# rrwick/Autocycler

Hardware: AMD Instinct MI355X
Metric: Mbp/sec through compress->unitig GFA (k=51) (higher is better)
Workload: dtype u64

## Files before the change

### autocycler_amd/_capi.py

```python
import ctypes as C
import os
from pathlib import Path

_HERE = Path(__file__).resolve().parent
LIB_PATH = _HERE / "libautocycler_hip.so"


class HipLibraryMissing(RuntimeError):
    pass


class AutocyclerError(RuntimeError):
    """The text the reference would hand to quit_with_error (misc.rs:131-137)."""


class SeqView(C.Structure):
    _fields_ = [("fwd", C.c_char_p), ("length", C.c_uint32), ("id", C.c_uint16)]


class Position(C.Structure):
    _fields_ = [("pos", C.c_uint32), ("seq_id_and_strand", C.c_uint16)]


class Link(C.Structure):
    _fields_ = [("a", C.c_int32), ("b", C.c_int32)]


class Stats(C.Structure):
    _fields_ = [("unitigs", C.c_uint32), ("links_one_way", C.c_uint64), ("total_length", C.c_uint64)]


class Timings(C.Structure):
    _fields_ = [(n, C.c_double) for n in ("h2d", "pack", "insert", "collect_sort", "degree", "segment", "minkey",
                                          "rank", "paths", "links", "seqs", "d2h", "total_device", "expand",
                                          "insert_kernel_ms")] + \
               [(n, C.c_uint64) for n in ("insert_positions", "table_capacity", "n_distinct", "n_path_entries")] + \
               [("simplify_passes", C.c_uint32), ("insert_launches", C.c_uint32), ("insert_real", C.c_uint64),
                ("analysis", C.c_double), ("finalize", C.c_double), ("n_candidates", C.c_uint32), ("n_levels", C.c_uint32),
                ("fragments", C.c_double), ("union_pack", C.c_double), ("union_insert", C.c_double),
                ("n_local_distinct", C.c_uint64), ("n_fragments", C.c_uint64), ("fragment_bytes", C.c_uint64),
                ("upload_device_ms", C.c_double), ("path_runs_copied", C.c_uint64), ("path_entries_walked", C.c_uint64), ("position_retries", C.c_uint64), ("n_candidates_owned", C.c_uint32),
                ("launches", C.c_uint32), ("readbacks", C.c_uint32), ("n_degrees_open", C.c_uint64), ("sort_retries", C.c_uint64), ("insert_rest_known", C.c_double), ("insert_rest_sampled", C.c_double), ("path_stretches", C.c_uint64),
                ("expand_sparse_sweeps", C.c_uint32), ("expand_sparse_start", C.c_uint32)]

    def as_dict(self):
        return {n: getattr(self, n) for n, _ in self._fields_}


class TrimSlice(C.Structure):
    _fields_ = [(n, C.c_uint32) for n in ("status", "begin", "end", "trimmed_length")]

    def as_dict(self):
        return {n: getattr(self, n) for n, _ in self._fields_}


class TrimResult(C.Structure):
    _fields_ = [("start_end", TrimSlice), ("hairpin", TrimSlice), ("hairpin_start_trimmed", C.c_uint32), ("hairpin_end_trimmed", C.c_uint32)]

    def as_dict(self):
        return dict(start_end=self.start_end.as_dict(), hairpin=self.hairpin.as_dict(),
                    hairpin_start_trimmed=self.hairpin_start_trimmed, hairpin_end_trimmed=self.hairpin_end_trimmed)


class TrimSummary(C.Structure):
    _fields_ = [("size", C.c_uint64), ("c_se", C.c_uint32), ("c_hp", C.c_uint32), ("chosen", C.c_uint32), ("launches", C.c_uint32),
                ("cells", C.c_uint64), ("seconds_device", C.c_double)]

    def as_dict(self):
        return {n: getattr(self, n) for n, _ in self._fields_ if n != "size"}


class AlignmentPiece(C.Structure):
    _fields_ = [("a_unitig", C.c_int32), ("a_index", C.c_uint32), ("b_unitig", C.c_int32), ("b_index", C.c_uint32)]


ALIGN_GAP, ALIGN_NONE = 0, 0xFFFFFFFF


class Bridge(C.Structure):
    _fields_ = [("start", C.c_int32), ("end", C.c_int32), ("depth", C.c_uint32), ("n_distinct", C.c_uint32), ("best_off", C.c_uint64),
                ("best_total", C.c_uint64), ("first_distinct", C.c_uint64), ("best_len", C.c_uint32), ("status", C.c_uint32),
                ("conflicting", C.c_uint32), ("culled", C.c_uint32), ("cull_rank", C.c_uint32), ("reserved", C.c_uint32)]


class ResolveSummary(C.Structure):
    _fields_ = [("size", C.c_uint64), ("jobs", C.c_uint64), ("jobs_not_launched", C.c_uint64), ("cells", C.c_uint64), ("largest_job_cells", C.c_uint64),
                ("launches", C.c_uint32), ("reserved", C.c_uint32), ("seconds_device", C.c_double)]

    def as_dict(self):
        return {n: getattr(self, n) for n, _ in self._fields_ if n not in ("size", "reserved")}


class Component(C.Structure):
    _fields_ = [("first", C.c_uint32), ("unitigs", C.c_uint32), ("length", C.c_uint64), ("links_all", C.c_uint64), ("links_one_way", C.c_uint64),
                ("open_ends", C.c_uint32), ("marked", C.c_uint32), ("circular_loop", C.c_uint8)]


class ComponentsSummary(C.Structure):
    _fields_ = [(n, C.c_uint32) for n in ("size", "unitigs", "components", "topology")] + \
               [(n, C.c_uint64) for n in ("links_all", "links_one_way", "total_length")] + \
               [("launches", C.c_uint32), ("read_backs", C.c_uint32), ("seconds_device", C.c_double)]

    def as_dict(self):
        return {n: getattr(self, n) for n, _ in self._fields_ if n != "size"}


class MergeChain(C.Structure):
    _fields_ = [("number", C.c_uint32), ("members", C.c_uint32), ("length", C.c_uint64), ("member_off", C.c_uint64), ("seq_off", C.c_uint64), ("depth", C.c_double),
                ("type", C.c_uint8), ("loop", C.c_uint8)]


class MergeSummary(C.Structure):
    _fields_ = [(n, C.c_uint32) for n in ("size", "chains", "merged_unitigs", "unitigs_after")] + [("links_after", C.c_uint64), ("bases_copied", C.c_uint64)] + \
               [("launches", C.c_uint32), ("read_backs", C.c_uint32), ("seconds_device", C.c_double), ("seconds_copy", C.c_double)]

    def as_dict(self):
        return {n: getattr(self, n) for n, _ in self._fields_ if n != "size"}


class SubsetCluster(C.Structure):
    _fields_ = [("seqs", C.c_uint32), ("unitigs", C.c_uint32), ("entries", C.c_uint64), ("links", C.c_uint64), ("length", C.c_uint64)]


class SubsetsSummary(C.Structure):
    _fields_ = [(n, C.c_uint32) for n in ("size", "clusters", "sequences_kept", "n_unitigs")] + [(n, C.c_uint64) for n in ("entries_kept", "unitigs", "links")] + \
               [("launches", C.c_uint32), ("read_backs", C.c_uint32), ("seconds_device", C.c_double)]

    def as_dict(self):
        return {n: getattr(self, n) for n, _ in self._fields_ if n != "size"}


class MergedPathsSummary(C.Structure):
    _fields_ = [("size", C.c_uint32), ("sequences", C.c_uint32), ("entries_before", C.c_uint64), ("entries_after", C.c_uint64),
                ("launches", C.c_uint32), ("read_backs", C.c_uint32), ("seconds_device", C.c_double)]

    def as_dict(self):
        return {n: getattr(self, n) for n, _ in self._fields_ if n != "size"}


class FinishedUnitig(C.Structure):
    _fields_ = [("number", C.c_uint32), ("source", C.c_uint32), ("length", C.c_uint64), ("seq_off", C.c_uint64), ("depth", C.c_double), ("type", C.c_uint8)]


class FinishedSummary(C.Structure):
    _fields_ = [(n, C.c_uint32) for n in ("size", "unitigs", "renumbered", "launches", "read_backs")] + \
               [(n, C.c_uint64) for n in ("links", "path_entries", "bases", "tie_items")] + [("seconds_device", C.c_double), ("seconds_gather", C.c_double)]

    def as_dict(self):
        return {n: getattr(self, n) for n, _ in self._fields_ if n != "size"}


class AppliedSummary(C.Structure):
    _fields_ = [(n, C.c_uint32) for n in ("size", "bridges_applied", "direct_links", "launches", "launches_components", "read_backs")] + \
               [(n, C.c_uint64) for n in ("removed_no_anchor", "removed_zero_depth", "links_in", "links_out", "bases_copied")] + \
               [("seconds_device", C.c_double), ("seconds_copy", C.c_double), ("seconds_components", C.c_double)]

    def as_dict(self):
        return {n: getattr(self, n) for n, _ in self._fields_ if n != "size"}


class CleanedSummary(C.Structure):
    _fields_ = [(n, C.c_uint32) for n in ("size", "unitigs_in", "unitigs_out", "rounds", "rounds_per_batch", "launches", "read_backs", "reserved")] + \
               [(n, C.c_uint64) for n in ("kept", "removed", "duplicated", "low_depth", "kept_dead_end", "absent", "links_in", "links_out")] + [("seconds_device", C.c_double)]

    def as_dict(self):
        return {n: getattr(self, n) for n, _ in self._fields_ if n not in ("size", "reserved")}


class TrimmedRecord(C.Structure):
    _fields_ = [("begin", C.c_uint32), ("end", C.c_uint32), ("length", C.c_uint64), ("trimmed", C.c_uint32), ("excluded", C.c_uint32)]


class TrimmedSummary(C.Structure):
    _fields_ = [("size", C.c_uint32), ("chosen", C.c_uint32), ("c_se", C.c_uint32), ("c_hp", C.c_uint32), ("sequences", C.c_uint32), ("trimmed", C.c_uint32),
                ("excluded", C.c_uint32), ("rejected", C.c_uint32), ("unitigs_in", C.c_uint32), ("unitigs_alive", C.c_uint32), ("launches", C.c_uint32),
                ("read_backs", C.c_uint32), ("median", C.c_uint64), ("mad", C.c_uint64), ("min_length", C.c_uint64), ("max_length", C.c_uint64),
                ("entries_kept", C.c_uint64), ("links", C.c_uint64), ("seconds_device", C.c_double), ("align_launches", C.c_uint32), ("reserved", C.c_uint32),
                ("align_cells", C.c_uint64), ("align_seconds_device", C.c_double)]

    def as_dict(self):
        return {name: getattr(self, name) for name, _ in self._fields_ if name not in ("size", "reserved")}


class CombinedCluster(C.Structure):
    _fields_ = [("input_index", C.c_uint32), ("unitigs", C.c_uint32), ("length", C.c_uint64), ("links", C.c_uint64), ("offset", C.c_uint64), ("max_number", C.c_uint32),
                ("topology", C.c_uint32), ("has_read_depth", C.c_uint32), ("reserved", C.c_uint32), ("read_depth", C.c_double)]


class CombinedUnitig(C.Structure):
    _fields_ = [("graph", C.c_uint32), ("index", C.c_uint32), ("number", C.c_uint32), ("length", C.c_uint32), ("depth", C.c_double), ("read_depth", C.c_double),
                ("has_read_depth", C.c_uint8), ("flags", C.c_uint8), ("type", C.c_uint8), ("reserved", C.c_uint8 * 5)]


class CombinedSummary(C.Structure):
    _fields_ = [("size", C.c_uint32), ("graphs", C.c_uint32), ("bases", C.c_uint64), ("unitigs", C.c_uint64), ("links", C.c_uint64), ("fully_resolved", C.c_uint32),
                ("with_reads", C.c_uint32), ("launches", C.c_uint32), ("read_backs", C.c_uint32), ("seconds_device", C.c_double)]

    def as_dict(self):
        d = {n: getattr(self, n) for n, _ in self._fields_ if n != "size"}
        d["fully_resolved"], d["with_reads"] = bool(d["fully_resolved"]), bool(d["with_reads"])
        return d


class ClusterNode(C.Structure):
    _fields_ = [("id", C.c_uint16), ("left", C.c_int32), ("right", C.c_int32), ("distance", C.c_double)]


class ClusterMerge(C.Structure):
    _fields_ = [("a", C.c_uint16), ("b", C.c_uint16), ("distance", C.c_double)]


class ClusterSummary(C.Structure):
    _fields_ = [("n_seqs", C.c_uint32), ("launches", C.c_uint32), ("rescans", C.c_uint64), ("compares", C.c_uint64), ("seconds", C.c_double)]

    def as_dict(self):
        return {n: getattr(self, n) for n, _ in self._fields_}


class ClusterQcRecord(C.Structure):
    _fields_ = [("node", C.c_uint16), ("container", C.c_uint16), ("size", C.c_uint32), ("assembly_count", C.c_uint32), ("fail", C.c_uint32),
                ("trusted", C.c_uint32), ("reserved", C.c_uint32), ("median_length", C.c_uint64), ("cluster_dist", C.c_double)]

    def as_dict(self):
        return {n: getattr(self, n) for n, _ in self._fields_ if n != "reserved"}


class ClusteringMetrics(C.Structure):
    _fields_ = [(n, C.c_uint32) for n in ("pass_cluster_count", "fail_cluster_count", "pass_contig_count", "fail_contig_count")] + \
               [(n, C.c_double) for n in ("pass_contig_fraction", "fail_contig_fraction", "cluster_balance_score", "cluster_tightness_score",
                                          "overall_clustering_score")]

    def as_dict(self):
        return {n: getattr(self, n) for n, _ in self._fields_}


class ClusterQcSummary(C.Structure):
    _fields_ = [(n, C.c_uint32) for n in ("n_seqs", "n_clusters", "rounds", "evaluations", "pair_batches", "launches", "readbacks", "reserved")] + \
               [(n, C.c_uint64) for n in ("alternatives", "node_pairs", "bytes_read_back")] + [("seconds", C.c_double), ("start_score", C.c_double)]

    def as_dict(self):
        return {n: getattr(self, n) for n, _ in self._fields_ if n != "reserved"}


class DepthGraph(C.Structure):
    _fields_ = [("seq_bytes", C.c_void_p), ("seq_begin", C.c_void_p), ("seq_len", C.c_void_p), ("n_unitigs", C.c_uint32),
                ("links", C.c_void_p), ("n_links", C.c_uint64)]


class DepthTotals(C.Structure):
    _fields_ = [("size", C.c_uint64)] + \
               [(n, C.c_uint64) for n in ("reads", "rejected_reads", "read_bases", "span_bases", "span_kmers", "hits", "distinct_kmers", "repeat_kmers",
                                          "table_slots")] + [("batches", C.c_uint32), ("launches", C.c_uint32), ("seconds_device", C.c_double)]

    def as_dict(self):
        return {n: getattr(self, n) for n, _ in self._fields_ if n != "size"}

ALLREDUCE_FN = C.CFUNCTYPE(C.c_int, C.c_void_p, C.c_void_p, C.c_uint64, C.c_int, C.c_int)

EXPORTS = ["ac_compress_build", "ac_compress_build_multi", "ac_multi_info_get", "ac_compress_build_device", "ac_pack_text", "ac_text_size", "ac_layout_text", "ac_kmer_count",
           "ac_stats_pre", "ac_stats_post", "ac_unitig_count", "ac_unitig", "ac_unitigs_bulk", "ac_paths_bulk", "ac_unitig_positions", "ac_links",
           "ac_path", "ac_timings_get", "ac_timings_get_sized", "ac_free", "ac_gfa_string", "ac_string_free", "ac_last_error",
           "ac_device_count", "ac_max_kmer", "ac_version", "ac_abi_version", "ac_set_host_side_device", "ac_source_hash", "ac_set_stage_timing", "ac_random_access_ceilings", "ac_random_access_ceilings_at", "ac_release_memory", "ac_end_repair_device", "ac_pairwise_distances", "ac_trim_paths", "ac_trim_path_slices", "ac_overlap_alignment", "ac_trim_max_unitigs", "ac_resolve_bridges", "ac_resolve_bridge_paths", "ac_path_distances", "ac_resolve_anchors", "ac_resolve_bridge_records", "ac_resolve_best_paths", "ac_resolve_distinct_paths", "ac_resolve_summary_get_sized", "ac_resolve_max_path", "ac_resolve_free", "ac_graph_components", "ac_components_from_links", "ac_components_records", "ac_components_of_unitig", "ac_components_members", "ac_components_unitig_flags", "ac_components_summary_get_sized", "ac_topology_name", "ac_components_free", "ac_graph_merge_plan", "ac_merge_plan_from_links", "ac_merge_chains", "ac_merge_members", "ac_merge_chain_of_unitig", "ac_merge_fixed_flags", "ac_merge_sequences", "ac_merge_links", "ac_merge_summary_get_sized", "ac_merge_free", "ac_graph_subsets", "ac_subsets_from_paths", "ac_subsets_records", "ac_subsets_unitigs", "ac_subsets_links", "ac_subsets_seqs", "ac_subsets_path_ends", "ac_subsets_dense", "ac_subsets_summary_get_sized", "ac_subsets_free", "ac_subsets_components", "ac_subsets_merge_plan", "ac_subsets_merged_paths", "ac_merged_paths_get", "ac_merged_paths_summary_get_sized", "ac_merged_paths_free", "ac_merge_finish", "ac_subsets_finish", "ac_finished_unitigs", "ac_finished_sequences", "ac_finished_new_of_old", "ac_finished_links", "ac_finished_paths", "ac_finished_summary_get_sized", "ac_finished_free", "ac_finished_gfa_string", "ac_finished_to_graph", "ac_apply_bridges", "ac_graph_resolve_apply", "ac_applied_unitigs", "ac_applied_bridge_of", "ac_applied_links", "ac_applied_bridge_sequences", "ac_applied_summary_get_sized", "ac_applied_free", "ac_applied_merge_plan", "ac_applied_finish", "ac_applied_gfa_string", "ac_resolve_graphs", "ac_clean_graph", "ac_graph_clean", "ac_cleaned_unitigs", "ac_cleaned_links", "ac_cleaned_summary_get_sized", "ac_cleaned_free", "ac_cleaned_merge_plan", "ac_cleaned_finish", "ac_cleaned_gfa_string", "ac_parse_tig_numbers", "ac_gfa_segment_types", "ac_clean_gfa", "ac_clean", "ac_trim_apply", "ac_graph_trim_apply", "ac_graph_trim", "ac_trimmed_records", "ac_trimmed_summary_get_sized", "ac_trimmed_free", "ac_trimmed_subsets", "ac_trimmed_finish", "ac_trimmed_yaml_string", "ac_trim_gfa", "ac_trim_dir", "ac_resolve_dir", "ac_combine_graphs", "ac_combine_handles", "ac_combined_clusters", "ac_combined_unitigs", "ac_combined_links", "ac_combined_summary_get_sized", "ac_combined_free", "ac_combined_gfa_string", "ac_combined_fasta_string", "ac_combined_yaml_string", "ac_combined_depth_lines", "ac_combine_gfas", "ac_combine", "ac_gfa2fasta_string", "ac_gfa2fasta", "ac_cluster_tree_build", "ac_cluster_tree_from_distances", "ac_cluster_tree_from_nodes", "ac_cluster_nodes", "ac_cluster_merges", "ac_cluster_summary_get_sized", "ac_cluster_free", "ac_cluster_max_seqs", "ac_cluster_cut", "ac_cluster_assign", "ac_cluster_containment", "ac_cluster_newick", "ac_cluster_generate", "ac_cluster_qc_nodes", "ac_cluster_qc_clusters", "ac_cluster_qc_assignment", "ac_cluster_qc_records", "ac_cluster_qc_metrics", "ac_cluster_qc_trace", "ac_cluster_qc_summary_get_sized", "ac_cluster_qc_free", "ac_cluster_min_assemblies", "ac_cluster_seq_inputs", "ac_depth_begin", "ac_depth_begin_handles", "ac_depth_add_reads", "ac_depth_add_fastq", "ac_depth_totals_get", "ac_depth_kmer_counts", "ac_depth_finish", "ac_depth_free", "ac_selftest_primitives", "ac_selftest_scan", "ac_selftest_radix", "ac_selftest_segments", "ac_selftest_sort_cmp", "ac_selftest_scan_pool", "ac_selftest_wave", "ac_selftest_fills", "ac_selftest_fill_order", "ac_selftest_readback", "ac_selftest_scalar_chain", "ac_selftest_arena", "ac_selftest_launch", "ac_selftest_atomics", "ac_selftest_side_order", "ac_selftest_event_ring", "ac_verify_graph", "ac_verify_graph_device", "ac_graph_from_gfa", "ac_graph_kmer_size", "ac_graph_seq_info", "ac_decompress_seq", "ac_decompress_device", "ac_decompress",
           "ac_shard_begin", "ac_shard_fragment_sizes", "ac_shard_fragments_export", "ac_shard_build_union", "ac_shard_fragment_packed_words", "ac_shard_fragments_export_packed", "ac_shard_build_union_packed",
           "ac_shard_unitig_count", "ac_shard_table_capacity", "ac_shard_bitmap_words", "ac_shard_bitmap_export", "ac_shard_build_novel", "ac_shard_sib_words", "ac_shard_sib_export", "ac_shard_degrees",
           "ac_shard_degree_bytes", "ac_multi_info_get_sized", "ac_shard_links_export", "ac_shard_links_import",
           "ac_shard_query_count", "ac_shard_query_key_words", "ac_shard_queries_export", "ac_shard_answer", "ac_shard_walk", "ac_shard_queries_route", "ac_shard_walk_routed", "ac_shard_local_distinct", "ac_shard_set_distinct_upper_bound", "ac_shard_distinct_count", "ac_shard_degrees_export", "ac_shard_build_graph", "ac_gfa_string_parts", "ac_shard_reduce_export", "ac_shard_reduce_import", "ac_shard_finish", "ac_shard_set_allreduce", "ac_device_copy",
           "ac_shard_path_entries", "ac_shard_paths_export", "ac_shard_free", "ac_graph_set_paths", "ac_graph_seq_count", "ac_path_counts",
           "ac_seqs_load", "ac_seqs_from_raw", "ac_seqs_count", "ac_seqs_assembly_count", "ac_seqs_views", "ac_seqs_get",
           "ac_seqs_repair_seconds", "ac_seqs_metrics_yaml", "ac_seqs_free", "ac_compress_seqs", "ac_compress_dir", "ac_compress_dir_multi"]

_libs = {}


def load_library(path=None):
    path = Path(path) if path else LIB_PATH
    key = str(path)
    if key in _libs:
        return _libs[key]
    if not path.exists():
        raise HipLibraryMissing(f"{path} not found: build the HIP extension first (make -C autocycler_amd/csrc). "
                                "There is no CPU fallback.")
    try:
        if os.environ.get("AC_NO_TORCH"):
            raise ImportError
        import torch
    except ImportError:
        pass
    lib = C.CDLL(key)
    lib.ac_last_error.restype = C.c_char_p
    lib.ac_version.restype = C.c_char_p
    lib.ac_source_hash.restype = C.c_char_p
    lib.ac_kmer_count.restype = C.c_uint64
    lib.ac_kmer_count.argtypes = [C.c_void_p]
    lib.ac_stats_pre.restype = Stats
    lib.ac_stats_pre.argtypes = [C.c_void_p]
    lib.ac_stats_post.restype = Stats
    lib.ac_stats_post.argtypes = [C.c_void_p]
    lib.ac_unitig_count.restype = C.c_uint32
    lib.ac_unitig_count.argtypes = [C.c_void_p]
    lib.ac_max_kmer.restype = C.c_uint32
    lib.ac_text_size.restype = C.c_uint64
    lib.ac_free.argtypes = [C.c_void_p]
    lib.ac_string_free.argtypes = [C.c_void_p]
    lib.ac_unitig.argtypes = [C.c_void_p, C.c_uint32, C.POINTER(C.c_void_p), C.POINTER(C.c_uint32), C.POINTER(C.c_double)]
    lib.ac_unitig_positions.argtypes = [C.c_void_p, C.c_uint32, C.c_int, C.POINTER(C.POINTER(Position)), C.POINTER(C.c_uint32)]
    lib.ac_links.argtypes = [C.c_void_p, C.POINTER(C.POINTER(Link)), C.POINTER(C.c_uint64)]
    lib.ac_path.argtypes = [C.c_void_p, C.c_uint32, C.POINTER(C.POINTER(C.c_int32)), C.POINTER(C.c_uint32)]
    lib.ac_timings_get.argtypes = [C.c_void_p, C.POINTER(Timings)]
    lib.ac_shard_unitig_count.restype = C.c_uint32
    lib.ac_shard_unitig_count.argtypes = [C.c_void_p]
    lib.ac_shard_fragment_packed_words.restype = C.c_uint64
    lib.ac_shard_fragment_packed_words.argtypes = [C.c_void_p, C.c_uint64]
    lib.ac_shard_local_distinct.restype = C.c_uint64
    lib.ac_shard_local_distinct.argtypes = [C.c_void_p]
    lib.ac_shard_set_distinct_upper_bound.argtypes = [C.c_void_p, C.c_uint64]
    lib.ac_shard_set_distinct_upper_bound.restype = None
    lib.ac_shard_distinct_count.restype = C.c_uint64
    lib.ac_shard_distinct_count.argtypes = [C.c_void_p]
    lib.ac_shard_path_entries.restype = C.c_uint64
    lib.ac_shard_path_entries.argtypes = [C.c_void_p]
    lib.ac_shard_free.argtypes = [C.c_void_p]
    for name in ("ac_shard_table_capacity", "ac_shard_bitmap_words", "ac_shard_query_count", "ac_shard_sib_words", "ac_shard_degree_bytes"):
        getattr(lib, name).restype = C.c_uint64
        getattr(lib, name).argtypes = [C.c_void_p]
    lib.ac_shard_query_key_words.restype = C.c_uint32
    lib.ac_shard_query_key_words.argtypes = [C.c_void_p]
    lib.ac_graph_seq_count.restype = C.c_uint32
    lib.ac_graph_seq_count.argtypes = [C.c_void_p]
    lib.ac_trim_max_unitigs.restype = C.c_uint32
    lib.ac_trim_max_unitigs.argtypes = []
    lib.ac_trim_paths.argtypes = [C.c_void_p, C.c_double, C.c_uint32, C.c_int, C.POINTER(TrimResult), C.POINTER(TrimSummary)]
    lib.ac_trim_path_slices.argtypes = [C.c_void_p, C.c_void_p, C.c_uint32, C.c_void_p, C.c_uint32, C.c_double, C.c_uint32, C.c_int,
                                        C.POINTER(TrimResult), C.POINTER(TrimSummary)]
    lib.ac_overlap_alignment.argtypes = [C.c_void_p, C.c_void_p, C.c_uint32, C.c_void_p, C.c_uint32, C.c_double, C.c_uint32, C.c_int, C.c_int,
                                         C.POINTER(AlignmentPiece), C.POINTER(C.c_uint32)]
    lib.ac_resolve_max_path.restype = C.c_uint32
    lib.ac_resolve_max_path.argtypes = []
    lib.ac_resolve_bridges.argtypes = [C.c_void_p, C.c_int, C.POINTER(C.c_void_p)]
    lib.ac_resolve_bridge_paths.argtypes = [C.c_void_p, C.c_void_p, C.c_uint32, C.c_void_p, C.c_void_p, C.c_uint32, C.c_int, C.POINTER(C.c_void_p)]
    lib.ac_path_distances.argtypes = [C.c_void_p, C.c_void_p, C.c_uint32, C.c_void_p, C.c_void_p, C.c_uint64, C.c_void_p, C.c_uint32, C.c_int, C.c_void_p, C.c_void_p]
    lib.ac_resolve_anchors.argtypes = [C.c_void_p, C.POINTER(C.POINTER(C.c_uint32)), C.POINTER(C.c_uint32)]
    lib.ac_resolve_bridge_records.argtypes = [C.c_void_p, C.POINTER(C.POINTER(Bridge)), C.POINTER(C.c_uint32)]
    lib.ac_resolve_best_paths.argtypes = [C.c_void_p, C.POINTER(C.POINTER(C.c_int32)), C.POINTER(C.c_uint64)]
    lib.ac_resolve_distinct_paths.argtypes = [C.c_void_p, C.POINTER(C.POINTER(C.c_int32)), C.POINTER(C.POINTER(C.c_uint64)), C.POINTER(C.POINTER(C.c_uint32)),
                                              C.POINTER(C.c_uint64)]
    lib.ac_resolve_summary_get_sized.restype = C.c_size_t
# ... 2095 lines not shown
```

### autocycler_amd/csrc/capi.cpp

```cpp
#include <algorithm>
#include <cstring>
#include <memory>

#include "capi_common.hpp"
#include "gfa_writer.hpp"

using namespace ac;
using namespace ac::abi;

static void select_device(int device, bool refresh_tuning = true) {
    if (refresh_tuning) tuning_refresh();
#ifndef AC_EMU
    int n = 0;
    hipError_t e = hipGetDeviceCount(&n);
    if (e != hipSuccess || n == 0)
        throw DeviceError("no HIP device available: the MI355X backend has no CPU fallback");
    if (device < 0 || device >= n) throw DeviceError("invalid HIP device ordinal " + std::to_string(device));
    AC_HIP_CHECK(hipSetDevice(device));
    hipDeviceProp_t prop;
    AC_HIP_CHECK(hipGetDeviceProperties(&prop, device));
    if (std::string(prop.gcnArchName).rfind("gfx950", 0) != 0)
        throw DeviceError(std::string("device is ") + prop.gcnArchName + "; this library is built for gfx950 only");
#endif
    int& arena_device = device_ctx().arena_device;
// ... 5 lines not shown
            Mailbox::get().release();
#endif
        }
        arena_device = device;
    }
}

namespace ac {
void select_device_checked(int device) { select_device(device, false); }

namespace abi __attribute__((visibility("hidden"))) {

std::string& last_error() { static thread_local std::string err; return err; }
std::mutex g_build_mutex;
int g_live_shards = 0;
std::atomic<int> g_host_side_device{0};

DeviceCall::DeviceCall(int device, Kind kind) : lock(g_build_mutex) {
    if (g_live_shards && kind != SHARD_PHASE)
        throw DeviceError(kind == SHARD_BEGIN ? "another sharded build is in flight in this process" : "a sharded build is in flight in this process");
    if (kind == ALL_DEVICES) tuning_refresh();
    else select_device(device);
}

void validate(uint32_t k, const ac_seq_view* seqs, uint32_t n_seqs) {
    if (!seqs || n_seqs == 0) throw DeviceError("no sequences found in input assemblies");
    if (k % 2 == 0) throw DeviceError("--kmer must be odd");
    if (n_seqs > 32767) throw DeviceError("no more than 32767 input sequences are allowed");
    for (uint32_t i = 0; i < n_seqs; i++) {
        if (!seqs[i].fwd) throw DeviceError("null sequence pointer");
        if (seqs[i].length < k) throw DeviceError("sequence shorter than k");
    }
}

void validate_layout(uint32_t k, uint64_t n_text, const uint64_t* off, const uint32_t* len, const uint16_t* d1, const uint16_t* d2,
                     uint32_t n_seqs) {
    if (k < 1 || k % 2 == 0) throw DeviceError("--kmer must be odd");
    if (!off || !len || !d1 || !d2) throw DeviceError("null sequence table");
    uint64_t prev_end = 0;
    for (uint32_t i = 0; i < n_seqs; i++) {
        if (len[i] < k) throw DeviceError("sequence " + std::to_string(i + 1) + " is shorter than k");
        const uint64_t plen = (uint64_t)len[i] + k - 1;
        if (off[i] != prev_end + 1) throw DeviceError("sequence table: sequence " + std::to_string(i + 1) + " does not start right behind the separator of the previous one");
        if (off[i] + plen + 1 > n_text) throw DeviceError("sequence table: sequence " + std::to_string(i + 1) + " runs past the end of the text");
        if (d1[i] > k - 1 || d2[i] > k - 1 || (uint32_t)d1[i] + d2[i] > k - 1) throw DeviceError("sequence table: more padding dots than k - 1 on sequence " + std::to_string(i + 1));
        prev_end = off[i] + plen;
    }
    if (n_seqs && prev_end + 1 != n_text) throw DeviceError("sequence table: the text does not end with the separator of the last sequence");
}

std::vector<SeqView> seq_views(const ac_seq_view* seqs, uint32_t n_seqs, std::vector<uint16_t>* seq_ids, std::vector<uint32_t>* seq_lens) {
    std::vector<SeqView> v(n_seqs);
    for (uint32_t i = 0; i < n_seqs; i++) {
        v[i] = SeqView{seqs[i].fwd, seqs[i].length};
        seq_ids->push_back(seqs[i].id);
        seq_lens->push_back(seqs[i].length);
    }
    return v;
}

void set_device_text(GraphBuilder& b, const void* d_text, uint64_t n_text, const uint64_t* seq_off, const uint32_t* seq_len,
                     const uint16_t* ids, const uint16_t* seq_d1, const uint16_t* seq_d2, uint32_t n_seqs,
                     std::vector<uint16_t>* seq_ids, std::vector<uint32_t>* seq_lens) {
    std::vector<uint64_t> off(seq_off, seq_off + n_seqs);
    std::vector<uint32_t> len(seq_len, seq_len + n_seqs);
    std::vector<uint16_t> d1(seq_d1, seq_d1 + n_seqs), d2(seq_d2, seq_d2 + n_seqs);
    seq_ids->assign(ids, ids + n_seqs);
    *seq_lens = len;
    b.set_text_device((const uint8_t*)d_text, n_text, off, len, d1, d2);
}

}
}

static void build_graph(GraphBuilder& b, uint32_t assembly_count, ac_graph* h) {
    b.build(assembly_count, &h->g);
    h->tm = b.timings();
}

template <class T> static size_t copy_sized(const T& full, T* out, size_t out_size) {
    memcpy(out, &full, std::min(out_size, sizeof full));
    return sizeof full;
}

extern "C" {

const char* ac_last_error(void) { return last_error().c_str(); }
const char* ac_version(void) {
#ifdef AC_EMU
    return "autocycler_amd 0.1 (CPU emulation, tests only)";
#else
    return "autocycler_amd 0.1 (gfx950)";
#endif
}
int ac_abi_version(void) { return AC_ABI_VERSION; }
int ac_set_host_side_device(int device) { if (device < 0) return fail("invalid HIP device ordinal"); g_host_side_device.store(device); return 0; }
void ac_set_stage_timing(int on) { set_stage_timing(on != 0); }
int ac_release_memory(void) {
    return guarded([&] {
        std::lock_guard<std::mutex> lock(g_build_mutex);
        if (g_live_shards) throw DeviceError("a sharded build is in flight in this process");
        Arena::device().release_all();
        release_multi_contexts();
        PinnedPool::get().trim();
        release_host_stager();
        scan_pool().release();
#ifndef AC_EMU
        Mailbox::get().release();
#endif
    });
}
uint32_t ac_max_kmer(void) { int m = max_supported_k(); return (uint32_t)(m % 2 ? m : m - 1); }
int ac_device_count(void) {
#ifndef AC_EMU
    int n = 0;
    if (hipGetDeviceCount(&n) != hipSuccess) return 0;
    return n;
#else
    return 0;
#endif
}

uint64_t ac_text_size(uint32_t k, const ac_seq_view* seqs, uint32_t n_seqs) {
    uint64_t n = 1;
    for (uint32_t i = 0; i < n_seqs; i++) n += (uint64_t)seqs[i].length + k - 1 + 1;
    return n;
}
int ac_layout_text(uint32_t k, const ac_seq_view* seqs, uint32_t n_seqs, uint8_t* text, uint64_t* seq_off,
                   uint16_t* seq_d1, uint16_t* seq_d2) {
    return guarded([&] {
        std::vector<SeqView> v(n_seqs);
        for (uint32_t i = 0; i < n_seqs; i++) v[i] = SeqView{seqs[i].fwd, seqs[i].length};
        std::vector<uint64_t> off; std::vector<uint32_t> len; std::vector<uint16_t> d1, d2;
        std::vector<uint8_t> t = layout_text(v, k, &off, &len, &d1, &d2);
        memcpy(text, t.data(), t.size());
        for (uint32_t i = 0; i < n_seqs; i++) { seq_off[i] = off[i]; seq_d1[i] = d1[i]; seq_d2[i] = d2[i]; }
    });
}

int ac_pack_text(const uint8_t* text, uint64_t n_text, uint64_t* bits, uint32_t* mask32, int force_scalar) {
    return guarded([&] {
        if (!text || !bits || !mask32) throw DeviceError("null pointer");
        pack_text_host(text, n_text, bits, mask32, force_scalar != 0);
    });
}

int ac_compress_build(uint32_t k, uint32_t assembly_count, const ac_seq_view* seqs, uint32_t n_seqs, int device,
                      ac_graph** out) {
    return guarded([&] {
        validate(k, seqs, n_seqs);
        DeviceCall call(device);
        auto h = std::make_unique<ac_graph>();
        const std::vector<SeqView> v = seq_views(seqs, n_seqs, &h->seq_ids, &h->seq_lens);
        GraphBuilder b(k);
        b.set_sequences_host(v);
        build_graph(b, assembly_count, h.get());
        *out = h.release();
    });
}

int ac_compress_build_multi(uint32_t k, uint32_t assembly_count, const ac_seq_view* seqs, uint32_t n_seqs, const int* devices, int n_devices,
                            ac_graph** out) {
    return guarded([&] {
        validate(k, seqs, n_seqs);
        if (!devices || n_devices < 1) throw DeviceError("ac_compress_build_multi: no devices");
        if (n_devices > 64) throw DeviceError("ac_compress_build_multi: more than 64 devices");
        DeviceCall call(-1, DeviceCall::ALL_DEVICES);
        auto h = std::make_unique<ac_graph>();
        const std::vector<SeqView> v = seq_views(seqs, n_seqs, &h->seq_ids, &h->seq_lens);
        int transport = MULTI_AUTO;
        if (const int e = tuning_multi_transport()) transport = e == 1 ? MULTI_HOST_STAGED : MULTI_RCCL;
        build_multi(k, assembly_count, v, std::vector<int>(devices, devices + n_devices), transport, &h->g, &h->tm, &h->multi);
        *out = h.release();
    });
}
int ac_multi_info_get(const ac_graph* g, ac_multi_info* o) {
    if (!g || !o) return fail("null pointer");
    const MultiStats& m = g->multi;
    memset(o, 0, sizeof *o);
    o->n_ranks = m.n_ranks; o->transport = m.transport;
    o->bytes_fragments = m.bytes_fragments; o->bytes_bitmap = m.bytes_bitmap; o->bytes_degrees = m.bytes_degrees; o->bytes_links = m.bytes_links;
    o->bytes_queries = m.bytes_queries; o->bytes_answers = m.bytes_answers; o->bytes_reduce = m.bytes_reduce;
    o->queries_total = m.queries_total; o->queries_sent_away = m.queries_sent_away;
    o->table_capacity_max = m.table_capacity_max; o->table_capacity_sum = m.table_capacity_sum;
    o->union_text_bytes = m.union_text_bytes; o->fragments = m.fragments; o->distinct = m.distinct;
    o->seconds_total = m.seconds_total; o->seconds_exchange_max = m.seconds_exchange_max;
    o->candidates_total = m.candidates_total; o->candidates_owned_max = m.candidates_owned_max;
    o->bytes_sibling = m.bytes_sibling; o->bytes_tail = m.bytes_tail; o->degrees_open = m.degrees_open; o->bytes_received_max = m.bytes_received_max;
    o->path_runs_copied = m.path_runs_copied;
    return 0;
}
size_t ac_multi_info_get_sized(const ac_graph* g, ac_multi_info* out, size_t out_size) {
    ac_multi_info t;
    if (!g || !out) { fail("null pointer"); return sizeof t; }
    ac_multi_info_get(g, &t);
    return copy_sized(t, out, out_size);
}

int ac_compress_build_device(uint32_t k, uint32_t assembly_count, const void* d_text, uint64_t n_text,
                             const uint64_t* seq_off, const uint32_t* seq_len, const uint16_t* seq_ids,
                             const uint16_t* seq_d1, const uint16_t* seq_d2, uint32_t n_seqs, int device,
                             ac_graph** out) {
    return guarded([&] {
        if (!d_text || n_seqs == 0) throw DeviceError("no sequences found in input assemblies");
        if (n_seqs > 32767) throw DeviceError("no more than 32767 input sequences are allowed");
        validate_layout(k, n_text, seq_off, seq_len, seq_d1, seq_d2, n_seqs);
        DeviceCall call(device);
        auto h = std::make_unique<ac_graph>();
        GraphBuilder b(k);
        set_device_text(b, d_text, n_text, seq_off, seq_len, seq_ids, seq_d1, seq_d2, n_seqs, &h->seq_ids, &h->seq_lens);
        build_graph(b, assembly_count, h.get());
        *out = h.release();
    });
}

uint32_t ac_graph_seq_count(const ac_graph* g) { return (uint32_t)g->seq_ids.size(); }
int ac_path_counts(const ac_graph* g, uint64_t* counts) {
    for (size_t s = 0; s + 1 < g->g.path_off.size(); s++) counts[s] = g->g.path_off[s + 1] - g->g.path_off[s];
    return 0;
}

uint32_t ac_graph_kmer_size(const ac_graph* g) { return g->g.k; }
int ac_graph_seq_info(const ac_graph* g, uint32_t i, uint16_t* id, uint32_t* length, const char** filename, const char** header) {
    if (i >= g->seq_ids.size()) return fail("sequence index out of range");
    if (id) *id = g->seq_ids[i];
    if (length) *length = g->seq_lens[i];
    if (filename) *filename = i < g->filenames.size() ? g->filenames[i].c_str() : nullptr;
    if (header) *header = i < g->headers.size() ? g->headers[i].c_str() : nullptr;
    return 0;
}

uint64_t ac_kmer_count(const ac_graph* g) { return g->g.n_kmers; }
ac_stats ac_stats_pre(const ac_graph* g) { return ac_stats{g->g.pre.unitigs, g->g.pre.links_one_way, g->g.pre.total_length}; }
ac_stats ac_stats_post(const ac_graph* g) { return ac_stats{g->g.post.unitigs, g->g.post.links_one_way, g->g.post.total_length}; }
uint32_t ac_unitig_count(const ac_graph* g) { return g->g.n_unitigs; }

int ac_unitig(const ac_graph* g, uint32_t idx, const uint8_t** seq, uint32_t* len, double* depth) {
    if (idx >= g->g.n_unitigs) return fail("unitig index out of range");
    if (!g->host_arrays) return fail("this rank kept no host arrays (sharded build, not the writing rank)");
    if (seq) *seq = (const uint8_t*)g->g.seq(idx);
    if (len) *len = g->g.seq_len[idx];
    if (depth) *depth = g->g.depth[idx];
    return 0;
}
int ac_unitig_positions(ac_graph* g, uint32_t idx, int forward, const ac_position** positions, uint32_t* n) {
    if (idx >= g->g.n_unitigs) return fail("unitig index out of range");
    return guarded([&] {
        if (!g->host_arrays || !g->host_paths) throw DeviceError("this rank kept no host arrays (sharded build, not the writing rank)");
        if (!g->positions_built) { build_positions(&g->g, g->seq_ids, g->seq_lens); g->positions_built = true; }
        auto& v = forward ? g->g.fwd_positions[idx] : g->g.rev_positions[idx];
        static_assert(sizeof(ac_position) == sizeof(Position), "layout");
        *positions = (const ac_position*)v.data();
        *n = (uint32_t)v.size();
    });
}
int ac_links(const ac_graph* g, const ac_link** links, uint64_t* n) {
    static_assert(sizeof(ac_link) == sizeof(Link), "layout");
    if (!g->host_arrays) return fail("this rank kept no host arrays (sharded build, not the writing rank)");
    *links = (const ac_link*)g->g.links;
    *n = g->g.n_links;
    return 0;
}
int ac_path(const ac_graph* g, uint32_t seq_index, const int32_t** signed_unitigs, uint32_t* n) {
    if ((size_t)seq_index + 1 >= g->g.path_off.size()) return fail("sequence index out of range");
    if (!g->host_paths) return fail("this rank kept no paths on the host (sharded build)");
    uint64_t b = g->g.path_off[seq_index], e = g->g.path_off[seq_index + 1];
    *signed_unitigs = g->g.path + b;
    *n = (uint32_t)(e - b);
    return 0;
}
int ac_unitigs_bulk(const ac_graph* g, const uint8_t** seq_bytes, const uint64_t** seq_begin, const uint32_t** seq_len, const double** depth) {
    if (!g->host_arrays) return fail("this rank kept no host arrays (sharded build, not the writing rank)");
    if (seq_bytes) *seq_bytes = (const uint8_t*)g->g.seq_block.p;
    if (seq_begin) *seq_begin = g->g.seq_begin;
    if (seq_len) *seq_len = g->g.seq_len;
    if (depth) *depth = g->g.depth;
    return 0;
}
int ac_paths_bulk(const ac_graph* g, const int32_t** path_entries, const uint64_t** path_off, uint64_t* n_entries) {
    if (!g->host_paths) return fail("this rank kept no paths on the host (sharded build)");
    if (path_entries) *path_entries = g->g.path;
    if (path_off) *path_off = g->g.path_off.data();
    if (n_entries) *n_entries = g->g.n_path;
    return 0;
}
int ac_timings_get(const ac_graph* g, ac_timings* o) {
    const BuildTimings& t = g->tm;
    o->h2d = t.h2d; o->pack = t.pack; o->insert = t.insert; o->collect_sort = t.collect_sort; o->degree = t.degree;
    o->segment = t.segment; o->minkey = t.minkey; o->rank = t.rank; o->paths = t.paths; o->links = t.links; o->seqs = t.seqs;
    o->d2h = t.d2h; o->total_device = t.total_device; o->expand = t.expand;
    o->insert_kernel_ms = t.insert_kernel_ms; o->insert_positions = t.insert_positions;
    o->table_capacity = t.table_capacity; o->n_distinct = t.n_distinct; o->n_path_entries = t.n_path_entries;
    o->simplify_passes = t.simplify_passes; o->n_candidates = t.n_candidates; o->n_levels = t.n_levels;
    o->insert_launches = t.insert_launches; o->insert_real = t.insert_real;
    o->analysis = t.analysis; o->finalize = t.finalize;
    o->fragments = t.fragments; o->union_pack = t.union_pack; o->union_insert = t.union_insert;
    o->n_local_distinct = t.n_local_distinct; o->n_fragments = t.n_fragments; o->fragment_bytes = t.fragment_bytes;
    o->upload_device_ms = t.upload_device_ms;
    o->path_runs_copied = t.path_runs_copied; o->path_entries_walked = t.path_entries_walked; o->position_retries = t.position_retries;
    o->n_candidates_owned = t.n_candidates_owned;
    o->launches = t.launches; o->readbacks = t.readbacks; o->n_degrees_open = t.n_degrees_open; o->sort_retries = t.sort_retries;
    o->insert_rest_known = t.insert_rest_known; o->insert_rest_sampled = t.insert_rest_sampled; o->path_stretches = t.path_stretches;
    o->expand_sparse_sweeps = t.expand_sparse_sweeps; o->expand_sparse_start = t.expand_sparse_start;
    return 0;
}
size_t ac_timings_get_sized(const ac_graph* g, ac_timings* out, size_t out_size) {
    ac_timings t;
    memset(&t, 0, sizeof t);
    ac_timings_get(g, &t);
    return out ? copy_sized(t, out, out_size) : sizeof t;
}
void ac_free(ac_graph* g) { delete g; }

static int gfa_parts_impl(const ac_graph* g, int parts, const char* const* filenames, const char* const* headers, char** out,
                          uint64_t* out_len) {
    return guarded([&] {
        if ((parts & 1) && !g->host_arrays) throw DeviceError("this rank kept no unitigs / links on the host (sharded build)");
        if ((parts & 2) && !g->host_paths) throw DeviceError("this rank kept no paths on the host (sharded build)");
        std::vector<SeqMeta> meta(g->seq_ids.size());
        for (size_t i = 0; i < meta.size(); i++) meta[i] = SeqMeta{g->seq_ids[i], g->seq_lens[i], filenames[i], headers[i]};
        std::string s = gfa_string(g->g, meta, parts);
        char* p = (char*)malloc(s.size() + 1);
        if (!p) throw DeviceError("out of memory");
        memcpy(p, s.data(), s.size()); p[s.size()] = 0;
        *out = p;
        if (out_len) *out_len = s.size();
    });
}
int ac_gfa_string(const ac_graph* g, const char* const* filenames, const char* const* headers, char** out, uint64_t* out_len) {
    return gfa_parts_impl(g, 3, filenames, headers, out, out_len);
}
int ac_gfa_string_parts(const ac_graph* g, int parts, const char* const* filenames, const char* const* headers, char** out,
                        uint64_t* out_len) {
    return gfa_parts_impl(g, parts, filenames, headers, out, out_len);
}
void ac_string_free(char* p) { free(p); }

}
```

### autocycler_amd/csrc/graph_build.hpp

```cpp
#pragma once
#include <cstdint>
#include <functional>
#include <string>
#include <vector>

#include "graph_types.hpp"
#include "trim_host.hpp"
#include "resolve_host.hpp"
#include "components_host.hpp"
#include "merge_host.hpp"
#include "subset_host.hpp"
#include "trim_apply_host.hpp"
#include "finish_host.hpp"
#include "apply_host.hpp"
#include "clean_host.hpp"
#include "combine_host.hpp"
#include "cluster_host.hpp"
#include "cluster_qc_host.hpp"

namespace ac {

struct SeqView {
    const uint8_t* fwd;
    uint32_t length;
};

struct BuildTimings {
    double h2d = 0, pack = 0, insert = 0, collect_sort = 0, degree = 0, segment = 0, minkey = 0, rank = 0,
           paths = 0, links = 0, seqs = 0, d2h = 0, total_device = 0;
    double expand = 0;
    double analysis = 0;
    double finalize = 0;
    double insert_kernel_ms = 0;
    uint64_t insert_positions = 0;
    uint64_t table_capacity = 0;
    uint64_t n_distinct = 0;
    uint64_t n_path_entries = 0;
    uint32_t insert_launches = 0;
    uint64_t insert_real = 0;
    uint32_t simplify_passes = 0, n_candidates = 0, n_levels = 0;
    uint32_t n_candidates_owned = 0;
    uint32_t local_hint = 0, graph_hint = 0;
    double fragments = 0;
    double union_pack = 0, union_insert = 0;
    uint64_t n_local_distinct = 0, n_fragments = 0, fragment_bytes = 0;
    double upload_device_ms = 0;
    double insert_rest_known = 0;
    uint64_t path_stretches = 0;
    uint32_t expand_sparse_sweeps = 0;
    uint32_t expand_sparse_start = 0;
    double insert_rest_sampled = 0;
    uint32_t sort_retries = 0;
    uint32_t position_retries = 0;
    uint32_t launches = 0, readbacks = 0;
    uint64_t n_degrees_open = 0;
    uint64_t path_runs_copied = 0, path_entries_walked = 0;
};

struct RepairTimings { double total = 0, scan_ms = 0; uint64_t hits = 0, matches = 0; uint32_t patterns = 0; };

class GraphBuilder {
  public:
    explicit GraphBuilder(uint32_t k);
    ~GraphBuilder();
    void set_sequences_host(const std::vector<SeqView>& seqs, bool pack_now = true);
    void repair_ends(RepairTimings* tm);
    void set_text_device(const uint8_t* d_text, uint64_t n_text, const std::vector<uint64_t>& off,
                         const std::vector<uint32_t>& len, const std::vector<uint16_t>& d1,
                         const std::vector<uint16_t>& d2);
    void build(uint32_t assembly_count_hint, FinalGraph* out);

    void shard_begin(uint32_t local_assembly_hint);
    uint64_t local_distinct_count() const;
    void set_distinct_upper_bound(uint64_t n);
    uint64_t fragment_text_bytes() const;
    uint64_t fragment_count() const;
    void fragments_export(void* d_text_out, void* d_meta_out);
    uint64_t fragment_packed_words(uint64_t union_off) const;
    void fragments_export_packed(uint64_t union_off, void* d_words_out, void* d_meta_out);
    void shard_build_union_packed(uint32_t rank, uint32_t n_shards, const void* d_staged_words, const uint64_t* first_word, const uint64_t* n_words,
                                  uint64_t n_union_text, const void* d_meta, uint64_t n_frags_total);
    void shard_build_union(uint32_t rank, uint32_t n_shards, const uint8_t* d_union_text, uint64_t n_union_text,
                           const void* d_meta, uint64_t n_frags_total);
    uint64_t bitmap_words() const;
    void bitmap_export(void* d_out);
    void shard_build_novel(const void* d_bitmap_sum);
    uint64_t sib_words() const;
    void sib_export(void* d_out);
    void shard_degrees(const void* d_sib_sum);
    uint64_t degree_bytes() const;
    uint64_t distinct_count() const;
    void degrees_export(void* d_out);
    void shard_build_graph(const void* d_kinfo_sum);
    uint32_t unitig_count() const;
    void links_export(void* d_links_i32, void* d_wlinks_i64);
    void links_import(const void* d_links_i32, const void* d_wlinks_i64);
    uint64_t query_count() const;
    uint32_t query_key_words() const;
    void queries_export(void* d_out);
    void answer_queries(const void* d_keys, uint64_t n, void* d_out);
    void shard_walk(const void* d_answers_mine);
    void queries_route(uint32_t n_shards, void* d_routed_keys, uint64_t* counts_host);
    void shard_walk_routed(const void* d_routed_answers);
    void reduce_export(int32_t* d_sum, int32_t* d_min);
    void reduce_import(const int32_t* d_sum, const int32_t* d_min);
    void set_tail_exchange(std::function<void(void*, uint64_t, int, int)> all_reduce);
    void shard_finish(FinalGraph* out, bool want_graph, bool want_paths);
    uint64_t path_entry_count() const;
    void paths_export(void* d_out);
    const BuildTimings& timings() const { return tm_; }
    void set_sequence_index_base(uint64_t n);
    static void set_upload_threads_cap(int n);
    uint64_t n_text() const;
    uint64_t n_bases() const;

    struct Impl;

  private:
    void build_union_impl(uint32_t rank, uint32_t n_shards, const uint8_t* d_union_text, const void* d_staged_words, const uint64_t* first_word,
                          const uint64_t* n_words, uint64_t n_union_text, const void* d_meta, uint64_t n_frags_total);
    void upload_packed(const std::vector<SeqView>& seqs, const std::vector<uint64_t>& off);
    Impl* impl_;
    BuildTimings tm_;
};

std::vector<uint8_t> layout_text(const std::vector<SeqView>& seqs, uint32_t k, std::vector<uint64_t>* off,
                                 std::vector<uint32_t>* len, std::vector<uint16_t>* d1, std::vector<uint16_t>* d2);

void end_repair_device(uint32_t k, uint8_t* d_text, uint64_t n_text, const std::vector<uint64_t>& off, const std::vector<uint32_t>& len,
                       std::vector<uint16_t>* d1, std::vector<uint16_t>* d2, RepairTimings* tm, bool reset_arena = true);

void pairwise_distances_device(const FinalGraph& g, uint32_t n_seqs, double* out);

struct VerifyReport {
    uint32_t failed = 0;
    uint64_t first_bad_unitig = ~0ULL, first_bad_link = ~0ULL, first_bad_path_entry = ~0ULL, first_bad_sequence = ~0ULL, first_bad_base = ~0ULL;
    uint64_t unitigs = 0, links = 0, path_entries = 0, bases_checked = 0, self_mirror_links = 0;
    double seconds = 0;
    uint32_t checks = 0;
    uint64_t first_bad_junction = ~0ULL;
};
void verify_graph_device(const FinalGraph& g, const uint8_t* d_text, uint64_t n_text, const std::vector<uint64_t>& off,
                         const std::vector<uint32_t>& len, VerifyReport* rep);

void decompress_device(const FinalGraph& g, const std::vector<uint32_t>& seq_len, uint8_t* out_host);
struct TrimDeviceStats { double seconds_device = 0; uint64_t cells = 0; uint32_t jobs = 0, launches = 0; };
void overlap_alignment_batch(const std::vector<AlignJob>& jobs, const uint32_t* weights, uint32_t max_unitigs, std::vector<AlignOut>* outs,
                             TrimDeviceStats* st);
uint32_t trim_max_unitigs();
struct ResolveDeviceStats { double seconds_device = 0; uint64_t cells = 0, jobs = 0, largest_job_cells = 0; uint32_t launches = 0; };
void path_distance_batch(const PathPool& pool, const std::vector<PathPair>& pairs, const uint32_t* weights, std::vector<uint32_t>* dist,
                         ResolveDeviceStats* st);
uint32_t resolve_max_path();
struct ClusterDeviceStats { double seconds = 0; uint64_t rescans = 0, compares = 0; uint32_t launches = 0; };
void cluster_merges_device(const double* asym, uint32_t n, std::vector<ClusterRowMerge>* merges, ClusterDeviceStats* st);
void cluster_merges_graph_device(const FinalGraph& g, uint32_t n_seqs, double* asym_out, std::vector<ClusterRowMerge>* merges, ClusterDeviceStats* st);
uint32_t cluster_max_seqs();
struct ClusterQcDeviceStats {
    double seconds = 0;
    uint32_t launches = 0, readbacks = 0, evaluations = 0, pair_batches = 0;
    uint64_t alternatives = 0, pairs_counted = 0, bytes_read_back = 0;
};
void cluster_qc_device(const double* asym, uint32_t n, const uint32_t* dfs_tip, double cutoff, const std::function<void(const ClusterQcEvaluate&)>& body,
                       ClusterQcDeviceStats* st);
void components_device(uint32_t n_unitigs, const Link* links, uint64_t n_links, const uint32_t* unitig_len, const uint8_t* alive, const uint8_t* marked,
                       ComponentsResult* out);
struct MergePlanInput {
    uint32_t n_unitigs = 0; const Link* links = nullptr; uint64_t n_links = 0; const uint32_t* unitig_len = nullptr; const uint8_t* alive = nullptr;
    const uint8_t* seed_fixed = nullptr; const int32_t* path = nullptr; uint64_t n_path = 0;
    const uint8_t* seq_bytes = nullptr; const uint64_t* seq_begin = nullptr; uint64_t seq_total = 0;
};
void merge_plan_device(const MergePlanInput& in, MergeResult* out);
struct SubsetInput {
    uint32_t n_unitigs = 0; const Link* links = nullptr; uint64_t n_links = 0; const uint32_t* unitig_len = nullptr; const uint8_t* alive = nullptr;
    const int32_t* path = nullptr; const uint64_t* path_off = nullptr; uint32_t n_clusters = 0; const SubsetPlan* plan = nullptr;
};
void subsets_device(const SubsetInput& in, SubsetResult* out);
struct MergedPathsInput {
    uint32_t n_unitigs = 0; const uint32_t* unitig_len = nullptr; const int32_t* path = nullptr; const uint64_t* path_off = nullptr;
    const SubsetPlan* plan = nullptr; size_t kept_first = 0, kept_count = 0; const MergeResult* merge = nullptr;
};
void merged_paths_device(const MergedPathsInput& in, MergedPathsResult* out);
struct TrimApplyInput {
    uint32_t n_unitigs = 0; const Link* links = nullptr; uint64_t n_links = 0; const uint32_t* unitig_len = nullptr; const uint8_t* alive = nullptr;
    const int32_t* path = nullptr; const uint64_t* path_off = nullptr; double mad = 0;
};
void trim_apply_device(const TrimApplyInput& in, TrimApplyPlan* tp, SubsetPlan* plan, SubsetResult* out);
struct FinishInput {
    uint32_t n_unitigs = 0; const Link* links = nullptr; uint64_t n_links = 0; const uint32_t* unitig_len = nullptr; const uint8_t* alive = nullptr;
    const double* depth = nullptr; const uint8_t* type = nullptr; const uint8_t* seq_bytes = nullptr; const uint64_t* seq_begin = nullptr; uint64_t seq_total = 0;
    const MergeResult* plan = nullptr; const int32_t* path = nullptr; uint64_t n_path = 0; bool renumber = false; uint64_t unitigs_after = 0;
};
void merge_finish_device(const FinishInput& in, FinishResult* out);
void apply_bridges_device(const ApplyInput& in, const ApplyPlan& plan, ApplyResult* out);
void clean_device(const CleanInput& in, CleanResult* out);
void combine_device(const CombineInput& in, CombineResult* out);
void primitives_selftest(uint64_t n, uint64_t seed, int end_bit, int key_kind);
void selftest_scan(int kind, const void* in, uint64_t n, bool in_place, int misalign_in, int misalign_out, void* out);
void selftest_radix(const uint64_t* keys, const void* vals, uint64_t n, int begin_bit, int end_bit, int val_kind, uint64_t prep_n, int prep_bits, bool prep_reuse,
                    uint64_t* keys_out, void* vals_out);
void selftest_segments(int op, const uint32_t* seg, const uint64_t* vals, uint64_t n, uint64_t n_segments, bool deferred_err, void* out, uint32_t* err_out);
void selftest_sort_cmp(int form, const uint64_t* a, const uint32_t* b, const uint32_t* vals, uint64_t n, uint64_t* a_out, uint32_t* b_out, uint32_t* vals_out);
void selftest_scan_pool(int op, uint64_t value, uint64_t* out);
void selftest_wave(int program, const uint64_t* in_u64, const int32_t* aux_i32, const uint64_t* live_mask, uint64_t* out_u64);
void selftest_fills(const uint64_t* regions, uint64_t n_regions, int trigger, int mode, uint8_t* span, uint64_t span_bytes, uint32_t* launches_out);
void selftest_fill_order(uint64_t n, int byte1, uint64_t w_lo, uint64_t w_hi, int w_val, uint64_t from2, int byte2, uint64_t upto3, int byte3, uint8_t* out);
void selftest_readback(const uint8_t* data, uint64_t n_data, int path, const uint64_t* items, uint64_t n_items, uint8_t* out, uint32_t* counters_out);
void selftest_scalar_chain(const uint64_t* values, uint64_t n, uint64_t* out, uint32_t* counters_out);
void selftest_arena(const uint64_t* ops, uint64_t n_ops, uint64_t* totals_out, uint64_t* allocs_out, const uint8_t* live, uint64_t* wrong_out);
void selftest_launch(int which, uint64_t n, uint64_t* slots_out, uint32_t* info_out);
void selftest_atomics(int op, uint64_t init, uint64_t expected, const uint64_t* operand, const uint32_t* target, uint32_t n_words, uint64_t* words_out, uint64_t* returns_out);
void selftest_side_order(int mode, int which, uint32_t seed, uint64_t n_words, uint32_t* out_words);
void selftest_event_ring(int op, const uint8_t* kinds, uint32_t n_more, uint64_t* out);

void random_access_ceilings(double* cas_gops, double* read_gops, uint64_t table_slots = (uint64_t)1 << 24);

void device_warmup(int device, uint32_t k = 0, uint64_t text_bytes_estimate = 0);

void pack_text_host(const uint8_t* text, uint64_t n_text, uint64_t* bits, uint32_t* mask32, bool force_scalar);

void release_host_stager();

int max_supported_k();
void tuning_refresh();
int tuning_multi_transport();
bool tuning_multi_fragments_as_bytes();
bool tuning_multi_tail_replicated();
void set_stage_timing(bool on);
bool stage_timing();

}
```

### autocycler_amd/csrc/graph_impl.hpp

```cpp
#pragma once
#include "graph_build.hpp"

#include <chrono>
#include <cmath>
#include <map>
#include <string>
#include <algorithm>
#include <atomic>
#include <thread>
#include <functional>
#include <condition_variable>
#include <mutex>
#include <fcntl.h>
#include <unistd.h>
#if defined(__x86_64__)
#include <immintrin.h>
#endif

#include "device_rt.hpp"

namespace ac {

static double now_s() {
    return std::chrono::duration<double>(std::chrono::steady_clock::now().time_since_epoch()).count();
}



static const int MAX_PROBES = 1 << 14;
static const int MAX_PROBES_INSERT = 1 << 10;
#ifndef AC_W_ONLY
#define AC_W_ONLY 0
#endif
extern bool g_stage_timing;

static const u32 KI_OUT_MASK = 7u, KI_IN_SHIFT = 3, KI_FIRST_T = 1u << 6, KI_FIRST_RCT = 1u << 7;

struct TextCtx {
    const u64* bits;
    const u64* mask;
    u64 n_text;
    int k;
    const u64* seq_off;
    const u32* seq_len;
    const u16* seq_d1;
    const u16* seq_d2;
    u32 n_seqs;
};

struct Table {
    u64* slots;
    u64 cap_mask;
    const u64* occ;
    u64* novel;
    u32 n_owners;
    u32 my_owner;
    u64* sflags;
    u64* full_at;
    u64* runs; u32* run_count; u64 run_row0;
};
static const u64 RUN_MIN = 128;
static const u32 RUN_ROW = 128;
AC_D void run_note(const Table& tb, u64 wave, u32& noted, u64 pj, u64 qj, bool same, u64 n) {
    if (!tb.runs || n < RUN_MIN || noted >= RUN_ROW) return;
    u64* rec = tb.runs + 3 * ((tb.run_row0 + wave) * RUN_ROW + noted);
    noted++;
    const bool with_anchor = ((tb.novel[qj >> 6] >> (qj & 63)) & 1) != 0;
    if (with_anchor) { rec[0] = pj; rec[1] = n + 1; rec[2] = qj | ((u64)(same ? 1 : 0) << 63); }
    else { rec[0] = pj + 1; rec[1] = n; rec[2] = (same ? qj + 1 : qj - 1) | ((u64)(same ? 1 : 0) << 63); }
}
AC_D void run_note_done(const Table& tb, u64 wave, u32 noted) { if (tb.runs) tb.run_count[tb.run_row0 + wave] = noted; }
AC_D void sib_note(const Table& tb, u64 s, u32 fl) { if (fl) atomic_or64(&tb.sflags[s >> 5], (u64)fl << (2 * (s & 31))); }
AC_HD u32 sib_bits(u64 v, u64 mine) {
    const u64 d = v ^ mine;
    if ((d >> TAG_MFP_SHIFT) != 0 || slot_isdot(v) || (d >> 41) == 0) return 0;
    return (((d >> TAG_X_SHIFT) & 3) == 0 ? 1u : 0u) | (((d >> TAG_Y_SHIFT) & 3) == 0 ? 2u : 0u);
}
AC_HD bool table_owns(const Table& tb, u64 home_hash) { return tb.n_owners <= 1 || (u32)((home_hash >> 40) % tb.n_owners) == tb.my_owner; }

AC_HD bool locate(const TextCtx& t, u64 p, u32* s_out, u32* f_out) {
    if (t.n_seqs == 0 || p < t.seq_off[0]) return false;
    u32 lo = 0, hi = t.n_seqs;
    while (hi - lo > 1) {
        u32 mid = lo + ((hi - lo) >> 1);
        if (t.seq_off[mid] <= p) lo = mid; else hi = mid;
    }
    u64 f = p - t.seq_off[lo];
    if (f >= (u64)t.seq_len[lo]) return false;
    *s_out = lo; *f_out = (u32)f;
    return true;
}

template <int W> AC_HD bool xkmer_at(const TextCtx& t, u64 p, XKmer<W>* x) {
    u32 s, f;
    if (!locate(t, p, &s, &f)) return false;
    int k = t.k;
    int plen = (int)t.seq_len[s] + k - 1;
    int ld = (int)t.seq_d1[s] - (int)f;
    int td = (int)f + k - (plen - (int)t.seq_d2[s]);
    x->ld = ld > 0 ? ld : 0;
    x->td = td > 0 ? td : 0;
    x->fwd = text_extract<W>(t.bits, p, k);
    return true;
}

template <int W> AC_HD int claimant_match(const TextCtx& t, u64 v, const Key<W>& ukey) {
    XKmer<W> y;
    if (!slot_isdot(v)) {
        y.fwd = text_extract<W>(t.bits, slot_pos(v), t.k);
        y.ld = 0; y.td = 0;
    } else {
        if (!xkmer_at<W>(t, slot_pos(v), &y)) return 0;
    }
    bool yf;
    Key<W> yk = xk_canonical<W>(y, t.k, &yf);
    if (!key_eq<W>(yk, ukey)) return 0;
    return yf ? 2 : 1;
}

struct FindResult { u64 pos; int claimant_flipped; bool found; };

template <int W> AC_HD FindResult table_find(const TextCtx& t, const Table& tb, const Key<W>& ukey, bool isdot) {
    const KeyPlace pl = key_place<W>(ukey, t.k, isdot, key_hash<W>(ukey));
    u64 tag = slot_make(pl.tag, isdot, 0);
    const u64 hh = pl.home;
    u64 s = hh & tb.cap_mask;
    FindResult r; r.found = false; r.pos = 0; r.claimant_flipped = 0;
    if (!table_owns(tb, hh)) return r;
    if (tb.occ && !((tb.occ[s >> 6] >> (s & 63)) & 1)) return r;
    for (int probes = 0; probes < MAX_PROBES; probes++) {
        u64 v = tb.slots[s];
        if (v == SLOT_EMPTY) return r;
        if (slot_tag_eq(v, tag)) {
            int m = claimant_match<W>(t, v, ukey);
            if (m) { r.found = true; r.pos = slot_pos(v); r.claimant_flipped = (m == 2); return r; }
        }
        s = (s + 1) & tb.cap_mask;
    }
    return r;
}

template <int W> AC_HD bool find_xk(const TextCtx& t, const Table& tb, const XKmer<W>& x, u64* pos, bool* rel_same) {
    bool flipped;
    Key<W> uk = xk_canonical<W>(x, t.k, &flipped);
    FindResult r = table_find<W>(t, tb, uk, x.ld > 0 || x.td > 0);
    if (!r.found) return false;
    *pos = r.pos;
    *rel_same = ((r.claimant_flipped != 0) == flipped);
    return true;
}

template <int W> AC_HD bool owns_xk(const TextCtx& t, const Table& tb, const XKmer<W>& x) {
    if (tb.n_owners <= 1) return true;
    bool flipped;
    Key<W> uk = xk_canonical<W>(x, t.k, &flipped);
    return table_owns(tb, key_home<W>(uk, t.k, x.ld > 0 || x.td > 0, key_hash<W>(uk)));
}

struct Novel {
    const u64* bm;
    const u32* wprefix;
};
AC_HD int popc64(u64 x) {
#ifdef AC_EMU
    return __builtin_popcountll(x);
#else
    return __popcll(x);
#endif
}
AC_HD u32 novel_rank(const Novel& nv, u64 pos) {
    u64 w = pos >> 6;
    int b = (int)(pos & 63);
    u64 below = b ? (nv.bm[w] & ((1ULL << b) - 1)) : 0;
    return nv.wprefix[w] + (u32)popc64(below);
}

static const u64 NOREF = ~0ULL;

template <int W> AC_D u64 table_insert(const TextCtx& t, const Table& tb, const Key<W>& ukey, bool isdot, bool flipped, u64 p,
                                       u32* claimed, u32* err, bool* same, bool* mine_now) {
    const KeyPlace pl = key_place<W>(ukey, t.k, isdot, key_hash<W>(ukey));
    u64 mine = slot_make(pl.tag, isdot, p);
    const u64 hh = pl.home;
    u64 s = hh & tb.cap_mask;
    *mine_now = false;
    if (!table_owns(tb, hh)) return NOREF;
    const bool note = tb.sflags != nullptr && !isdot;
    u32 my_fl = 0;
    for (int probes = 0; probes < MAX_PROBES_INSERT; probes++) {
        u64 v = tb.slots[s];
        if (v == SLOT_EMPTY) {
            u64 old = atomic_cas64(&tb.slots[s], SLOT_EMPTY, mine);
            if (old == SLOT_EMPTY) { (*claimed)++; *mine_now = true; if (note) sib_note(tb, s, my_fl); return NOREF; }
            v = old;
        }
        if (slot_tag_eq(v, mine)) {
            if (slot_pos(v) == p) { if (note) sib_note(tb, s, my_fl); return NOREF; }
            int m = claimant_match<W>(t, v, ukey);
            if (m) {
                if (note) sib_note(tb, s, my_fl);
                if (slot_pos(v) > p) {
                    u64 old = atomic_min64(&tb.slots[s], mine);
                    if (old > mine) {
                        *mine_now = true;
                        u64 q = slot_pos(old);
                        atomic_xor64(&tb.novel[q >> 6], 1ULL << (q & 63));
                    }
                    return NOREF;
                }
                *same = ((m == 2) == flipped);
                return slot_pos(v);
            }
        } else if (note) {
            const u32 fl = sib_bits(v, mine);
            if (fl) { sib_note(tb, s, fl); my_fl |= fl; }
        }
        s = (s + 1) & tb.cap_mask;
    }
    atomic_or32(err, 1u);
    if (tb.full_at) atomic_max64(tb.full_at, ~p);
    return NOREF;
}

struct alignas(16) V16 { u32 a, b, c, d; };

#include "kernels_table.inc"
#include "kernels_unitigs.inc"
#include "kernels_paths.inc"
#include "kernels_tail.inc"
#include "kernels_shard.inc"
struct PathRemapJob {
    int32_t* path = nullptr; u64 n_ent = 0;
    const int32_t* rec_val = nullptr; const u32* rec_pos = nullptr; u64 n_rec = 0;
    const u32* number = nullptr; u32 n_unitigs = 0;
    u64 ent_limit = ~0ULL;
    void* landed = nullptr; SideStream* side = nullptr;
    int dev = 0;
    std::atomic<u64> next{0}; std::atomic<int> ready{0};
    std::atomic<u32> bad{0};
    u64 ticket = 0; bool started = false;
    std::atomic<double> t_ready{0}, t_last{0};
};
void path_remap_range(int32_t* p, u64 n, const u32* number, u32 n_unitigs, std::atomic<u32>* bad);
void path_stretch_range(const PathRemapJob& j, u64 s0, u64 s1, std::atomic<u32>* bad);
bool path_remap_is_wide();
void path_remap_start(PathRemapJob& j, int threads);
void path_remap_finish(PathRemapJob& j) noexcept;
struct SeqExpandJob {
    const u64* words = nullptr; u8* out = nullptr; u64 total = 0;
    void* landed = nullptr; SideStream* side = nullptr; int dev = 0;
    std::atomic<u64> next{0}; std::atomic<int> ready{0};
    u64 ticket = 0; bool started = false;
    std::atomic<double> t_start{0}, t_ready{0}, t_last{0};
};
void seq_expand_range(const u64* words, u8* out, u64 b, u64 e);
void seq_expand_start(SeqExpandJob& j, int threads);
void seq_expand_finish(SeqExpandJob& j) noexcept;
[[maybe_unused]] static int key_words(int k) { int w = words_for_k(k); return w <= 4 ? w : (w <= 8 ? 8 : 16); }
[[maybe_unused]] static u64 next_pow2(u64 x) { u64 p = 1; while (p < x) p <<= 1; return p; }
[[maybe_unused]] static size_t arena_estimate(u64 n_text, bool owns_text) { return (size_t)n_text * (owns_text ? 8 : 7) + ((size_t)768 << 20); }
struct Knobs {
    int minkey_variant;
    int path_copy;
    u64 run_piece;
    u32 pos_cap;
    bool path_filter;
    int host_remap_mode;
    u32 remap_block;
    int minkey_prefix_bases;
    bool seed_prefix_sort;
    u32 seed_max_group;
    int seed_prefix_bits;
    u32 degree_region_cap;
    int upload_direct_mode;
    int upload_slots;
    int degree_flags;
    int table_shift;
    u64 wave_chunk_max;
    u64 insert_chunk_rest_env;
    bool host_pack;
    u32 expand_level_table;
    bool shard_path_copy;
    bool expand_rewrite_always;
    u32 expand_sparse_max, expand_sparse_list, expand_sparse_batch;
    u32 stretch_device_share;
    int seq_codes_transfer;
    int late_copies;
    bool seq_writer_plain;
    bool seq_writer_forced;
    u64 seed_radix_limit;
    bool upload_overlap;
    bool sort_checks_deferrable;
    bool shard_host_remap;
    bool shard_degree_flags;
    bool insert_adaptive;
    u64 insert_growth;
    u64 insert_waves_target;
    bool renum_two_pass;
    u32 renum_max_group;
    u32 path_chunk_env;
    long upload_threads_env;
    bool debug_arena;
    bool degree_diag;
    int multi_transport;
    int multi_fragments;
    int multi_tail;
    u64 trim_batch_bytes;
    u64 resolve_batch_bytes;
    static Knobs read() {
        Knobs k;
        k.minkey_variant = [&]() -> int { const char* e = getenv("AC_MINKEY_VARIANT"); return e ? atoi(e) : -1; }();
        k.path_copy = [&]() -> int { const char* e = getenv("AC_PATH_COPY"); return e ? (atoi(e) != 0 ? 1 : 0) : 2; }();
        k.run_piece = [&]() -> u64 { const char* e = getenv("AC_RUN_PIECE"); const long v = e ? atol(e) : 0; return v > 0 ? (u64)v : 4096; }();
        k.pos_cap = [&]() -> u32 { const char* e = getenv("AC_POS_CAP"); const long v = e ? atol(e) : 65536; return v < 0 ? 0u : (u32)std::min<long>(v, 0x3FFFFFFF); }();
        k.path_filter = [&]() -> bool { const char* e = getenv("AC_PATH_FILTER"); return e ? atoi(e) != 0 : true; }();
        k.host_remap_mode = [&]() -> int { const char* e = getenv("AC_HOST_REMAP"); return e ? (atoi(e) == 2 ? 2 : (atoi(e) != 0 ? 1 : 0)) : -1; }();
        k.remap_block = [&]() -> u32 { const char* e = getenv("AC_REMAP_BLOCK"); int v = e ? atoi(e) : 4096; v = v < 64 ? 64 : (v > 65536 ? 65536 : v); return (u32)(v & ~63); }();
        k.minkey_prefix_bases = [&]() -> int { const char* e = getenv("AC_MINKEY_PREFIX_BASES"); int v = e ? atoi(e) : 31; return v < 1 ? 1 : (v > 31 ? 31 : v); }();
        k.seed_prefix_sort = [&]() -> bool { const char* e = getenv("AC_SEED_PREFIX_SORT"); return e ? atoi(e) != 0 : true; }();
        k.seed_max_group = [&]() -> u32 { const char* e = getenv("AC_SEED_MAX_GROUP"); int v = e ? atoi(e) : 1024; return (u32)(v < 1 ? 1 : v); }();
        k.seed_prefix_bits = [&]() -> int { const char* e = getenv("AC_SEED_PREFIX_BITS"); if (!e) return 0; int v = atoi(e); return v < 1 ? 1 : (v > 64 ? 64 : v); }();
        k.degree_region_cap = [&]() -> u32 { const char* e = getenv("AC_DEGREE_REGION_CAP"); int v = e ? atoi(e) : 0; return (u32)(v < 0 ? 0 : v); }();
        k.upload_direct_mode = [&]() -> int { const char* e = getenv("AC_UPLOAD_DIRECT"); return e ? (atoi(e) != 0 ? 1 : 0) : -1; }();
        k.upload_slots = [&]() -> int { const char* e = getenv("AC_UPLOAD_SLOTS"); int v = e ? atoi(e) : 1 << 20; return v < 1 ? 1 : v; }();
        k.degree_flags = [&]() -> int { const char* e = getenv("AC_DEGREE_FLAGS"); return e ? (atoi(e) != 0 ? 1 : 0) : 1; }();
        k.table_shift = [&]() -> int { const char* e = getenv("AC_TABLE_SHIFT"); if (!e) return -1; int v = atoi(e); return v < 0 ? 0 : (v > 3 ? 3 : v); }();
        k.wave_chunk_max = [&]() -> u64 { const char* e = getenv("AC_INSERT_CHUNK"); u64 x = e ? (u64)atoll(e) : 8192; return (std::max<u64>(x, 256) + 63) & ~63ULL; }();
        k.insert_chunk_rest_env = [&]() -> u64 { const char* e = getenv("AC_INSERT_CHUNK_REST"); if (!e) return 0; return (std::max<u64>((u64)atoll(e), 256) + 63) & ~63ULL; }();
        k.host_pack = [&]() -> bool { const char* e = getenv("AC_HOST_PACK"); return e ? atoi(e) != 0 : true; }();
        k.expand_level_table = [&]() -> u32 { const char* e = getenv("AC_EXPAND_LEVEL_TABLE"); int v = e ? atoi(e) : 1024; return (u32)(v < 1 ? 1 : v); }();
        k.shard_path_copy = [&]() -> bool { const char* e = getenv("AC_SHARD_PATH_COPY"); return !(e && atoi(e) == 0); }();
        k.expand_rewrite_always = [&]() -> bool { return getenv("AC_EXPAND_REWRITE_ALWAYS") != nullptr; }();
        k.expand_sparse_max = [&]() -> u32 { const char* e = getenv("AC_EXPAND_SPARSE_MAX"); int v = e ? atoi(e) : 256; return (u32)(v < 0 ? 0 : v); }();
        k.late_copies = [&]() -> int { const char* e = getenv("AC_LATE_COPIES"); return e ? atoi(e) : 1; }();
        k.seq_codes_transfer = [&]() -> int { const char* e = getenv("AC_SEQ_CODES"); return e ? atoi(e) : 1; }();
        k.stretch_device_share = [&]() -> u32 { const char* e = getenv("AC_STRETCH_DEVICE_SHARE"); int v = e ? atoi(e) : 30; return (u32)(v < 0 ? 0 : v); }();
        k.expand_sparse_list = [&]() -> u32 { const char* e = getenv("AC_EXPAND_SPARSE_LIST"); int v = e ? atoi(e) : 0; return (u32)(v < 0 ? 0 : v); }();
        k.expand_sparse_batch = [&]() -> u32 { const char* e = getenv("AC_EXPAND_SPARSE_BATCH"); int v = e ? atoi(e) : 4096; return (u32)(v < 1 ? 1 : v); }();
        k.seq_writer_plain = [&]() -> bool { const char* e = getenv("AC_SEQ_WRITER"); return e && atoi(e) == 0; }();
        k.seq_writer_forced = [&]() -> bool { const char* e = getenv("AC_SEQ_WRITER"); return e && atoi(e) == 1; }();
        k.seed_radix_limit = [&]() -> u64 { const char* e = getenv("AC_SEED_RADIX_LIMIT"); return e ? (u64)atoll(e) : (1u << 19); }();
        k.upload_overlap = [&]() -> bool { const char* e = getenv("AC_UPLOAD_OVERLAP"); return e ? atoi(e) != 0 : true; }();
        k.sort_checks_deferrable = [&]() -> bool { const char* e = getenv("AC_SORT_CHECKS"); return !(e && atoi(e) == 1); }();
        k.shard_host_remap = [&]() -> bool { const char* e = getenv("AC_SHARD_HOST_REMAP"); return e ? atoi(e) != 0 : true; }();
        k.shard_degree_flags = [&]() -> bool { const char* e = getenv("AC_SHARD_DEGREE_FLAGS"); return e ? atoi(e) != 0 : true; }();
        k.insert_adaptive = [&]() -> bool { const char* e = getenv("AC_INSERT_ADAPT"); return e ? atoi(e) != 0 : true; }();
        k.insert_growth = [&]() -> u64 { const char* e = getenv("AC_INSERT_GROWTH"); long x = e ? atol(e) : 2; return (u64)(x < 2 ? 2 : x); }();
        k.insert_waves_target = [&]() -> u64 { const char* e = getenv("AC_INSERT_WAVES"); long x = e ? atol(e) : 16384; return (u64)(x < 1024 ? 1024 : x); }();
        k.renum_two_pass = [&]() -> bool { const char* e = getenv("AC_RENUM_TWO_PASS"); return e && atoi(e) != 0; }();
        k.renum_max_group = [&]() -> u32 { const char* e = getenv("AC_RENUM_MAX_GROUP"); int v = e ? atoi(e) : 64; return (u32)(v < 1 ? 1 : (v > 64 ? 64 : v)); }();
        k.path_chunk_env = [&]() -> u32 { const char* e = getenv("AC_PATH_CHUNK"); if (!e) return 0; int v = atoi(e); return (u32)(v < 64 ? 64 : (v > 4096 ? 4096 : v)); }();
        k.upload_threads_env = [&]() -> long { const char* e = getenv("AC_UPLOAD_THREADS"); return e ? atol(e) : 24; }();
        k.debug_arena = [&]() -> bool { return getenv("AC_DEBUG_ARENA") != nullptr; }();
        k.degree_diag = [&]() -> bool { return getenv("AC_DEGREE_DIAG") != nullptr; }();
        k.multi_transport = [&]() -> int { const char* e = getenv("AC_MULTI_TRANSPORT"); return !e ? 0 : (!strcmp(e, "host") ? 1 : (!strcmp(e, "rccl") ? 2 : 0)); }();
        k.multi_fragments = [&]() -> int { const char* e = getenv("AC_MULTI_FRAGMENTS"); return e && !strcmp(e, "bytes") ? 1 : 0; }();
        k.multi_tail = [&]() -> int { const char* e = getenv("AC_MULTI_TAIL"); return e && !strcmp(e, "replicated") ? 1 : 0; }();
        k.trim_batch_bytes = [&]() -> u64 { const char* e = getenv("AC_TRIM_BATCH_BYTES"); const long long v = e ? atoll(e) : 0; return v > 0 ? (u64)v : (u64)4 << 30; }();
        k.resolve_batch_bytes = [&]() -> u64 { const char* e = getenv("AC_RESOLVE_BATCH_BYTES"); const long long v = e ? atoll(e) : 0; return v > 0 ? (u64)v : (u64)1 << 30; }();
        return k;
    }
};
const Knobs& knobs();
void knobs_refresh();

[[maybe_unused]] static int minkey_variant() { return knobs().minkey_variant; }
[[maybe_unused]] static int path_copy() { return knobs().path_copy; }
[[maybe_unused]] static bool path_copy_pays(u64 n_text, u32 assemblies, u32 k, double r2) {
    const double A = (double)std::max<u32>(assemblies, 1);
    const double entries = (double)n_text * std::min(1.0, 2.0 * A * r2 / (double)k);
    const double saving = entries * 53e-12 * std::max(0.0, 1.0 - 2.0 / A), cost = 0.25e-3 + 0.3e-12 * (double)n_text;
    return saving > 1.5 * cost;
}
[[maybe_unused]] static u64 run_piece() { return knobs().run_piece; }
[[maybe_unused]] static u32 pos_cap() { return knobs().pos_cap; }
[[maybe_unused]] static bool path_filter() { return knobs().path_filter; }
#ifdef AC_MEASUREMENT_KNOBS
[[maybe_unused]] static int path_diag() { const char* e = getenv("AC_PATH_DIAG"); return e ? (atoi(e) & 3) : 0; }
#else
[[maybe_unused]] static int path_diag() { return 0; }
#endif
[[maybe_unused]] static u32 path_chunk(u64 n_kmers, u32 n_unitigs) {
    if (knobs().path_chunk_env) return knobs().path_chunk_env;
    const u64 want = 5 * n_kmers / std::max<u32>(n_unitigs, 1);
    u32 pc = 64;
    while (pc < 2048 && (u64)pc * 3 / 2 < want) pc *= 2;
    return pc;
}
[[maybe_unused]] static int host_remap_mode() { return knobs().host_remap_mode; }
[[maybe_unused]] static u32 remap_block() { return knobs().remap_block; }
[[maybe_unused]] static int minkey_prefix_bases() { return knobs().minkey_prefix_bases; }
[[maybe_unused]] static bool seed_prefix_sort() { return knobs().seed_prefix_sort; }
[[maybe_unused]] static u32 seed_max_group() { return knobs().seed_max_group; }
[[maybe_unused]] static int seed_prefix_bits() { return knobs().seed_prefix_bits; }
[[maybe_unused]] static u32 degree_region_cap() { return knobs().degree_region_cap; }
[[maybe_unused]] static u64 upload_chunk_bytes() { return (u64)64 << 20; }
[[maybe_unused]] static int upload_direct_mode() { return knobs().upload_direct_mode; }
[[maybe_unused]] static int upload_slots() { return knobs().upload_slots; }
[[maybe_unused]] static int degree_flags() { return knobs().degree_flags; }
[[maybe_unused]] static int table_shift() { return knobs().table_shift; }
[[maybe_unused]] static u64 wave_chunk_max() { return knobs().wave_chunk_max; }
[[maybe_unused]] static u64 wave_chunk_rest() { return 16384; }
[[maybe_unused]] static u64 insert_chunk_rest_env() { return knobs().insert_chunk_rest_env; }
static thread_local int tl_upload_threads_cap = 0;
[[maybe_unused]] static u64 upload_threads() {

    long x = knobs().upload_threads_env;
    if (tl_upload_threads_cap > 0 && x > tl_upload_threads_cap) x = tl_upload_threads_cap;
    return (u64)(x < 1 ? 1 : (x > 128 ? 128 : x));
}
[[maybe_unused]] static bool host_pack() { return knobs().host_pack; }
[[maybe_unused]] static bool insert_profile() { static const bool v = getenv("AC_INSERT_PROFILE") != nullptr; return v; }
[[maybe_unused]] static u32 expand_level_table() { return knobs().expand_level_table; }
[[maybe_unused]] static bool shard_path_copy() { return knobs().shard_path_copy; }
[[maybe_unused]] static u32 expand_sparse_max() { return knobs().expand_sparse_max; }
[[maybe_unused]] static int late_copies() { return knobs().late_copies; }
[[maybe_unused]] static int seq_codes_transfer() { return knobs().seq_codes_transfer; }
[[maybe_unused]] static u32 stretch_device_share() { return knobs().stretch_device_share; }
[[maybe_unused]] static u32 expand_sparse_list() { return knobs().expand_sparse_list; }
[[maybe_unused]] static u32 expand_sparse_batch() { return knobs().expand_sparse_batch; }
[[maybe_unused]] static bool expand_rewrite_always() { return knobs().expand_rewrite_always; }
[[maybe_unused]] static bool seq_writer_plain() { return knobs().seq_writer_plain; }
[[maybe_unused]] static bool seq_writer_forced() { return knobs().seq_writer_forced; }
[[maybe_unused]] static u64 seed_radix_limit() { return knobs().seed_radix_limit; }
[[maybe_unused]] static bool upload_overlap() { return knobs().upload_overlap; }
[[maybe_unused]] static bool sort_checks_deferrable() { return knobs().sort_checks_deferrable; }
[[maybe_unused]] static bool shard_host_remap() { return knobs().shard_host_remap; }
[[maybe_unused]] static bool shard_degree_flags() { return knobs().shard_degree_flags; }
[[maybe_unused]] static bool insert_adaptive() { return knobs().insert_adaptive; }
[[maybe_unused]] static u64 insert_growth() { return knobs().insert_growth; }
[[maybe_unused]] static u64 insert_waves_target() { return knobs().insert_waves_target; }

struct PackedText {
    const u8* d_text = nullptr;
    u64 n_text = 0, n_bases = 0;
    u32 n_seqs = 0;
    int any_dots = 0; u64 n_dotted = 0;
    DBuf<u64> seq_off; DBuf<u32> seq_len; DBuf<u16> seq_d1, seq_d2; DBuf<u8> seq_flags;
    bool has_flags = false;
    DBuf<u64> bits, mask;
    DBuf<u32> pack_bad; bool check_alphabet = false; int k = 0; u64 expected_nonbase = 0;
    u64 index_base = 0;
    PackCheck chk() const { return PackCheck{seq_off.ptr(), seq_len.ptr(), seq_d1.ptr(), seq_d2.ptr(), n_seqs, k, check_alphabet ? const_cast<u32*>(pack_bad.ptr()) : nullptr}; }
    std::vector<u64> h_off; std::vector<u32> h_len;
    void set_table(const std::vector<uint64_t>& off, const std::vector<uint32_t>& len, const std::vector<uint16_t>& d1,
                   const std::vector<uint16_t>& d2, const std::vector<uint8_t>* flags = nullptr) {
        n_seqs = (u32)off.size();
        h_off = off; h_len = len;
        seq_off.alloc(n_seqs); seq_len.alloc(n_seqs); seq_d1.alloc(n_seqs); seq_d2.alloc(n_seqs);
        copy_h2d(seq_off.ptr(), off.data(), (size_t)n_seqs * 8);
        copy_h2d(seq_len.ptr(), len.data(), (size_t)n_seqs * 4);
        copy_h2d(seq_d1.ptr(), d1.data(), (size_t)n_seqs * 2);
        copy_h2d(seq_d2.ptr(), d2.data(), (size_t)n_seqs * 2);
        has_flags = flags != nullptr;
        if (flags) { seq_flags.alloc(n_seqs); copy_h2d(seq_flags.ptr(), flags->data(), n_seqs); }
        n_bases = 0; any_dots = 0; n_dotted = 0; expected_nonbase = (u64)n_seqs + 1;
        for (u32 i = 0; i < n_seqs; i++) { n_bases += len[i]; if (d1[i] || d2[i]) { any_dots = 1; n_dotted++; } expected_nonbase += (u64)d1[i] + d2[i]; }
        stream_sync();
    }
    void alloc_table(u32 n) { n_seqs = n; h_off.clear(); h_len.clear(); seq_off.alloc(n); seq_len.alloc(n); seq_d1.alloc(n); seq_d2.alloc(n); seq_flags.alloc(n); has_flags = true; }
    void set_sums(u64 bases, u64 dotted, u64 dots) { n_bases = bases; n_dotted = dotted; any_dots = dotted ? 1 : 0; expected_nonbase = (u64)n_seqs + 1 + dots; }
    TextCtx ctx(int k) const { return TextCtx{bits.ptr(), mask.ptr(), n_text, k, seq_off.ptr(), seq_len.ptr(), seq_d1.ptr(), seq_d2.ptr(), n_seqs}; }
    bool packed = false;
    void pack_alloc(stream_t s = 0) {
        u64 n_bits_words = n_text / 32 + 24, n_mask_words = n_text / 64 + 12;
        bits.alloc(n_bits_words); mask.alloc(n_mask_words);
        const u64 groups = (n_text + 31) / 32;
        bits.fill_bytes_from(groups * 8, 0, s);
        mask.fill_bytes_from(groups * 4, 0xFF, s);
        if (check_alphabet) { pack_bad.alloc(2); pack_bad.fill_bytes(0xFF, s); }
    }
    void verify_alphabet(const u32* bad) const {
        if (!check_alphabet) return;
        if (bad[0] != 0xFFFFFFFFu) throw DeviceError("input sequence " + std::to_string(index_base + bad[0]) + " contains non-ACGT characters");
        const u64 found = (u64)(u32)(bad[1] + 1u);
        if (found != (expected_nonbase & 0xFFFFFFFFULL))
            throw DeviceError("the text does not match its sequence table: " + std::to_string(expected_nonbase) + " padding dots and separators expected, " +
                              std::to_string(found) + " non-ACGT characters found");
    }
    void pack() {
        if (packed) return;
        pack_alloc();
        launch((n_text + 31) / 32, PackFunctor{d_text, n_text, bits.ptr(), (u32*)mask.ptr(), 0, chk()});
        packed = true;
    }
};

struct GraphBuilder::Impl {
    u32 k = 0;
    DBuf<u8> text_owned;
    PackedText loc;
    PackedText uni;
    PackedText* G = &loc;
    BuildTimings* tm = nullptr;
    double t0 = 0, t_begin = 0;
    void lap(double* acc) { if (!g_stage_timing) return; stream_sync(); double t = now_s(); *acc += t - t0; t0 = t; }

    DBuf<u32> counters;
    DBuf<u64> slots; u64 cap = 0; u64 N = 0;
    DBuf<u64> bm; DBuf<u32> wprefix; DBuf<u64> npos;
    u32 U = 0;
    DBuf<u32> kinfo, head, scan, ustart, order, rank, ulen;
    DBuf<u64> ustartpos, useq_off; DBuf<u8> uorient;
    DBuf<int32_t> links; DBuf<u64> wlinks;
    DBuf<u32> depth, minpos_fwd, minpos_rev; DBuf<u64> path_off; DBuf<int32_t> ent_val; u64 n_ent = 0;
    DBuf<u64> wl_text; DBuf<u32> depth_u, minpos_fwd_u, minpos_rev_u, run_start, run_end;
    void walk_arrays();
    void walk_tables(bool filter);
    void walk_to_seed_order();
    bool walked_plain = false;
    DBuf<u8> fs0, fe0;
    u32 pos_cap_now = 0xFFFFFFFFu; bool exact_positions = false;
    bool host_remap_allowed = false;
    bool paths_in_seed_numbers = false;
    bool checked_sorts = false; DBuf<u32> sort_flags;
    bool deferred_sort_checks() const { return host_remap_allowed_build && !checked_sorts && sort_checks_deferrable(); }
    bool host_remap_allowed_build = false;
    DBuf<u8> maybe_dest; bool maybe_dest_valid = false;
    DBuf<u8> frag_text; DBuf<u64> frag_meta, frag_fpos, frag_boff; u64 frag_bytes = 0, n_frags = 0;
    u64 distinct_upper = 0;

    void begin(BuildTimings* t) {
        tm = t; t_begin = t0 = now_s();
        rt_counters() = RtCounters();
        host_remap_allowed = false;
        counters.alloc(8); counters.fill_bytes(0);
        sort_flags.alloc(2); sort_flags.fill_bytes(0);
    }
    void check_sizes(const PackedText& t) const {
        if (t.n_text >= POS_MASK) throw DeviceError("input too large for 40-bit text positions");
        if (t.n_seqs == 0 || t.n_text < (u64)k + 2) throw DeviceError("no sequences");
    }
    template <int W> void insert(const PackedText& t, u32 hint, DBuf<u64>* slots_out, u64* cap_out, u64* n_distinct_out, DBuf<u64>* bm_out, bool want_sib = false);
    DBuf<u64> sflags;
    DBuf<u64> runs; DBuf<u32> run_count; u64 run_rows = 0, run_rows_cap = 0;
    DBuf<u64> loc_bm; DBuf<u32> loc_wprefix; bool local_insert_of_shard = false;
    struct CopyPlan { bool ok = false; u64 R = 0, NW = 0, Rb = 0; DBuf<RunRec> rr; DBuf<u32> rseq; DBuf<u64> wfirst, w_begin, w_end; DBuf<u32> w_gap; } cplan;
    void occupancy_bitmap(const DBuf<u64>& sl, u64 c, DBuf<u64>* occ_out, const u64* sflags_in, u64* sib_out, stream_t s = 0);
    DBuf<u64> occ;
    DBuf<u64> sib;
    DBuf<u64> sibn; bool sib_pending = false;
    DBuf<u32> kcontrib, pend, pidx; u64 n_pending = 0, n_first = 0;
    DBuf<u64> endset, endset_bloom; u64 endset_mask = 0;
    u32 n_owners = 1, my_owner = 0;
    void* upload_done = nullptr; u64 upload_avail = 0; bool upload_pending = false;
    struct UploadJob {
#ifndef AC_EMU
        const std::vector<SeqView>* seqs = nullptr;
        std::vector<uint64_t> off;
        uint32_t k = 0; u64 n = 0, CH = 0, SUB = 0, n_chunks = 0, slot_bytes = 0; int NSLOT = 0, dev = 0;
        hipStream_t up = nullptr, pk = nullptr;
        u64* d_bits = nullptr;
        bool direct = false;
        double t_start = 0; std::atomic<u64> chunks_issued{0}; std::atomic<double> t_last{0};
        hipEvent_t fills_done = nullptr;
        std::atomic<u64> next{0}, nonbase{0}, bar_sink{0}; u64 expected_nonbase = 0;
        std::vector<std::atomic<u32>> done, slot_state, issued;
        std::vector<hipEvent_t> landed;
        std::mutex hip_mu; std::string fail; std::atomic<bool> stop{false};
        u64 ticket = 0;
        void* stager = nullptr;
        u64 next_wait = 0;
        void run();
#endif
    };
    UploadJob* job = nullptr;
    u64 upload_rest_limit(u64 pb) const;
    void need_text(u64 upto);
    void finish_upload();
    ~Impl();
    void pack_overlapped(u32 hint) {
        PackedText& pt = loc;
        if (pt.packed) return;
#ifndef AC_EMU
        const u64 p_end_all = pt.n_text - (u64)k + 1;
        const u64 first = std::max<u64>(p_end_all / std::max<u32>(hint, 1), 1u << 16);
        const u64 H = (first + (u64)k + 8192 + 4095) & ~4095ULL;
        const u64 cap_est = next_pow2(std::max<u64>(1024, pt.n_bases / std::max<u32>(hint, 1) * 3 + 4096));
        if (cap_est <= (1ULL << 25) && H + (1u << 22) < pt.n_text) {
            pt.pack_alloc();
            launch(H / 32, PackFunctor{pt.d_text, pt.n_text, pt.bits.ptr(), (u32*)pt.mask.ptr(), 0, pt.chk()});
            SideStream& side = SideStream::get();
            side.after_main();
            launch((pt.n_text + 31) / 32 - H / 32, PackFunctor{pt.d_text, pt.n_text, pt.bits.ptr(), (u32*)pt.mask.ptr(), H / 32, pt.chk()}, side.stream());
            upload_done = side.mark(); upload_avail = H; upload_pending = true;
            pt.packed = true;
            return;
        }
#endif
        pt.pack();
    }
    Table graph_table() const { return Table{const_cast<u64*>(slots.ptr()), cap - 1, occ.ptr(), nullptr, n_owners, my_owner, nullptr, nullptr, nullptr, nullptr, 0}; }
    template <int W> void fragments();
    template <int W> void table();
    void novel_list(u64 known_n);
    template <int W> void degrees();
    template <int W> void walk_queries();
    template <int W> void answer_queries(const u64* d_keys, u64 n, u64* d_out);
    DBuf<u64> qkeys; u64 n_queries = 0;
    DBuf<u32> qidx;
    DBuf<u64> qanswers;
    template <int W> void route_queries(u32 n_shards, u64* d_routed_keys, u64* counts_host);
    const u64* walk_answers = nullptr;
    template <int W> void unitigs();
    template <int W> void walk();
    template <int W> bool walk_copy_prepare(u32 PC, const Novel& nv_text);
    template <int W> void walk_copy_finish(u32 PC);
    void tail(FinalGraph* out, bool want_graph, bool want_paths);
    std::function<void(void*, uint64_t, int, int)> tail_xchg;
};

inline void GraphBuilder::Impl::occupancy_bitmap(const DBuf<u64>& sl, u64 c, DBuf<u64>* occ_out, const u64* sflags_in, u64* sib_out, stream_t s) {
    occ_out->alloc((c + 63) / 64);
#ifdef AC_EMU
    occ_out->fill_bytes(0);
#endif
    launch_full(c, MarkFunctor{sl.ptr(), occ_out->ptr(), sflags_in, sib_out}, s);
}
inline void GraphBuilder::Impl::novel_list(u64 known_n) {
    PackedText& g = *G;
    u64 n_bm_words = g.n_text / 64 + 1;
    DBuf<u32> wcnt(n_bm_words + 1);
    wprefix.alloc(n_bm_words + 1);
    launch(n_bm_words + 1, PopcFunctor{bm.ptr(), wcnt.ptr(), n_bm_words});
    exclusive_scan_u32(wcnt.ptr(), wprefix.ptr(), n_bm_words + 1);
    if (known_n) N = known_n;
    else {
        N = read_scalar(wprefix.ptr() + n_bm_words);
        if (N == 0) throw DeviceError("internal error: no k-mers in the union of the shards");
        tm->n_distinct = N;
    }
    npos.alloc(N);
    launch_wave_kernel(fill_novel_wave_kernel<0>, (n_bm_words + 255) / 256, 0, (const u64*)bm.ptr(), (const u32*)wprefix.ptr(), npos.ptr(), n_bm_words);
    kinfo.alloc(N, true);
    head.alloc(N + 1); scan.alloc(N + 1);
    head.fill_bytes_from(N * 4, 0); scan.fill_bytes_from(N * 4, 0);
    lap(&tm->collect_sort);
}

inline void GraphBuilder::Impl::walk_arrays() {
    wl_text.alloc((u64)U * 10);
    depth_u.alloc(U, true); minpos_fwd_u.alloc(U); minpos_rev_u.alloc(U);
    run_start.alloc((u64)U + 1, true); run_end.alloc((u64)U + 1, true);
}
inline void GraphBuilder::Impl::walk_tables(bool filter) {
    launch((u64)U * 10, WlinkFlagFunctor{filter ? maybe_dest.ptr() : nullptr, wlinks.ptr(), counters.ptr() + 4});
    const u32 pos_init = pos_cap_now == 0xFFFFFFFFu ? 0xFFFFFFFFu : ((pos_cap_now + 1) | POS_BOUND);
    launch((u64)U * 10, WlinkTextOrderFunctor{wlinks.ptr(), rank.ptr(), order.ptr(), uorient.ptr(), wl_text.ptr(), minpos_fwd_u.ptr(), minpos_rev_u.ptr(), pos_init});
}
inline void GraphBuilder::Impl::walk_to_seed_order() {
    depth.alloc(U); minpos_fwd.alloc(U); minpos_rev.alloc(U);
    DBuf<u32> started, ended;
    if (walked_plain) {
        started.alloc((u64)U + 1); ended.alloc((u64)U + 1);
        inclusive_scan_u32(run_start.ptr(), started.ptr(), (u64)U + 1);
        exclusive_scan_u32(run_end.ptr(), ended.ptr(), (u64)U + 1);
    }
    launch(U, WalkToSeedOrderFunctor{order.ptr(), depth_u.ptr(), walked_plain ? started.ptr() : nullptr, walked_plain ? ended.ptr() : nullptr,
                                     minpos_fwd_u.ptr(), minpos_rev_u.ptr(), depth.ptr(), minpos_fwd.ptr(), minpos_rev.ptr()});
}

template <int W> struct Stages {
    static void table(GraphBuilder::Impl& m);
    static void degrees(GraphBuilder::Impl& m);
    static void walk_queries(GraphBuilder::Impl& m);
    static void answer_queries(GraphBuilder::Impl& m, const u64* d_keys, u64 n, u64* d_out);
    static void route_queries(GraphBuilder::Impl& m, u32 n_shards, u64* d_routed_keys, u64* counts_host);
    static void unitigs(GraphBuilder::Impl& m);
    static void walk(GraphBuilder::Impl& m);
    static void fragments(GraphBuilder::Impl& m);
    static void warm();
};

void tail_warm();

#define AC_DISPATCH_W(NAME, ARGS)                                        \
    switch (key_words((int)impl_->k)) {                                  \
        case 1: Stages<1>::NAME ARGS; break;                             \
        case 2: Stages<2>::NAME ARGS; break;                             \
        case 3: Stages<3>::NAME ARGS; break;                             \
        case 4: Stages<4>::NAME ARGS; break;                             \
        case 8: Stages<8>::NAME ARGS; break;                             \
        case 16: Stages<16>::NAME ARGS; break;                           \
        default: throw DeviceError("unsupported k");                     \
    }

}
```

### autocycler_amd/csrc/graph_stages.hip

```cpp
#include "graph_impl.hpp"

namespace ac {

template <int W>
void GraphBuilder::Impl::insert(const PackedText& pt, u32 hint, DBuf<u64>* slots_out, u64* cap_out, u64* n_distinct_out, DBuf<u64>* bm_out, bool want_sib) {
    TextCtx t = pt.ctx((int)k);
    const u64 p_end_all = pt.n_text - (u64)k + 1;
    if (hint == 0) hint = 1;
    u64 est = pt.n_bases / hint;
    u64 c = next_pow2(std::max<u64>(1024, est * 3 + 4096));
    if (&pt == &uni && distinct_upper) {
        const u64 mine = distinct_upper / std::max<u32>(n_owners, 1) + distinct_upper / (8 * (u64)std::max<u32>(n_owners, 1)) + 4096;
        c = next_pow2(std::max<u64>(1024, mine * 10 / 7));
    }
    if (c > next_pow2(pt.n_bases * 2 + 1024)) c = next_pow2(pt.n_bases * 2 + 1024);
    const int shift = table_shift() >= 0 ? table_shift() : (c > (1ULL << 25) ? 0 : 1);
    c <<= shift;
    struct CapMemo { u64 n_text = 0, cap = 0; u32 k = 0; int shift = -2; u32 owners = 0; };
    static thread_local CapMemo memo[4]; static thread_local unsigned memo_next = 0;
    const u32 memo_owners = (&pt == &uni) ? n_owners : 1u;
    for (const CapMemo& m : memo)
        if (pt.n_text == m.n_text && k == m.k && m.shift == table_shift() && m.owners == memo_owners && m.cap > c) c = m.cap;
    const int copy_mode = (&pt == &loc && (want_sib || (local_insert_of_shard && shard_path_copy()))) ? path_copy() : 0;
    bool want_runs = false;
    DBuf<InsertStats> istats(257);
    DBuf<u64> sl;
    DBuf<u64> nbm(pt.n_text / 64 + 2);
    u64 n_distinct = 0;
    const Arena::Mark retry_mark = Arena::device().mark();
    std::vector<u64> phase_end;
    for (;;) {
        sl.alloc(c);
        sl.fill_bytes(0xFF);
        nbm.fill_bytes(0);
        counters.fill_bytes(0);
        istats.fill_bytes(0);
        if (want_sib) { sflags.alloc(c / 32 + 1); sflags.fill_bytes(0); }
        else sflags = DBuf<u64>();
        u32* ierr = (u32*)&istats.ptr()[256].real;
        Table tb{sl.ptr(), c - 1, nullptr, nbm.ptr(), (&pt == &uni) ? n_owners : 1u, (&pt == &uni) ? my_owner : 0u, want_sib ? sflags.ptr() : nullptr,
                 &istats.ptr()[256].claimed, nullptr, nullptr, 0};
        if (&pt == &loc) { runs = DBuf<u64>(); run_count = DBuf<u32>(); run_rows = run_rows_cap = 0; cplan = CopyPlan(); }
        phase_end.clear();
        stream_sync();
#ifndef AC_EMU
        std::vector<hipEvent_t> evs;
        flush_fills();
#endif
        u32 launches = 0;
        u64 rest_chunk = wave_chunk_rest();
        u64 first = std::max<u64>(p_end_all / hint, 1u << 16);
        u64 pb = 0;
        bool rest_at_once = false;
        while (pb < p_end_all) {
            const bool diverse = launches >= 2 && !rest_at_once && insert_adaptive();
            u64 pe = (pb == 0) ? first : pb * (diverse ? std::max<u64>(insert_growth(), 4) : insert_growth());
            if (rest_at_once || pe > p_end_all || p_end_all - pe < (1u << 16)) pe = p_end_all;
#ifndef AC_EMU
            if (upload_pending && &pt == &loc && pe + (u64)k + 8192 > upload_avail) {
                flush_fills();
                SideStream::get().consumed(upload_done);
                AC_HIP_CHECK(hipStreamWaitEvent(0, (hipEvent_t)upload_done, 0));
                upload_pending = false;
            }
            if (job && &pt == &loc) {
                if (rest_at_once) pe = std::min<u64>(pe, upload_rest_limit(pb));
                need_text(pe + (u64)k + 8192);
            }
#endif
            const u64 len = pe - pb;
            {
                u64 c = (len / (diverse ? std::max<u64>(insert_waves_target(), 65536) : insert_waves_target()) + 63) & ~63ULL;
                u32 chunk = (u32)std::min<u64>(std::max<u64>(c, 256), rest_at_once ? rest_chunk : wave_chunk_max());
                u64 n_waves = (len + chunk - 1) / chunk;
                if (want_runs && rest_at_once) {
                    if (!run_rows_cap) {
                        run_rows_cap = 2 * ((p_end_all - pb) / chunk + 1) + n_waves + 64;
                        run_rows_cap = std::min<u64>(run_rows_cap, 4 * (pt.n_text / rest_chunk + 1) + n_waves + 1024);
                        runs.alloc(3 * run_rows_cap * RUN_ROW); run_count.alloc(run_rows_cap + 1);
                        run_count.fill_bytes(0);
                    }
                    if (run_rows + n_waves <= run_rows_cap) { tb.runs = runs.ptr(); tb.run_count = run_count.ptr(); tb.run_row0 = run_rows; run_rows += n_waves; }
                    else tb.runs = nullptr;
                }
                const u64 blocks = (n_waves + 3) / 4;
#ifndef AC_EMU
                if (insert_profile()) {
                    DBuf<u64> prof(16);
                    prof.fill_bytes(0);
                    launch_wave_kernel(insert_wave_kernel<W, true>, blocks, 0, t, tb, pb, pe, chunk, istats.ptr(), ierr, prof.ptr());
                    std::vector<u64> h = to_host(prof, 16);
                    fprintf(stderr, "insert launch %u: positions %llu chunk %u waves %llu | opener %llu steps avg %.0f cy | wide %llu steps avg %.0f cy | follow %llu runs avg %.0f cy | "
                            "wave avg %.0f cy, longest %llu cy\n", launches, (unsigned long long)len, chunk, (unsigned long long)h[7],
                            (unsigned long long)h[1], h[1] ? (double)h[0] / h[1] : 0.0, (unsigned long long)h[3], h[3] ? (double)h[2] / h[3] : 0.0,
                            (unsigned long long)h[5], h[5] ? (double)h[4] / h[5] : 0.0, h[7] ? (double)h[6] / h[7] : 0.0, (unsigned long long)h[8]);
                } else {
                    hipEvent_t ea, eb;
                    AC_HIP_CHECK(hipEventCreate(&ea)); AC_HIP_CHECK(hipEventCreate(&eb));
                    evs.push_back(ea); evs.push_back(eb);
                    flush_fills();
                    AC_HIP_CHECK(hipEventRecord(ea, 0));
                    launch_wave_kernel(insert_wave_kernel<W, false>, blocks, 0, t, tb, pb, pe, chunk, istats.ptr(), ierr, (u64*)nullptr);
                    AC_HIP_CHECK(hipEventRecord(eb, 0));
                }
#else
                launch_wave_kernel(insert_wave_kernel<W, false>, blocks, 0, t, tb, pb, pe, chunk, istats.ptr(), ierr, (u64*)nullptr);
#endif
            }
            launches++;
            pb = pe;
            phase_end.push_back(pe);
            if (launches == 2 && insert_adaptive() && pb < p_end_all && (p_end_all - pb) > 4 * first) {
                u64 probe_end = p_end_all;
#ifndef AC_EMU
                if (&pt == &loc) {
                    if (job) {
                        need_text(std::min<u64>(p_end_all, pb + (1u << 20)) + (u64)k + 8192);
                        const u64 avail = job ? std::min<u64>(job->n, job->next_wait * job->CH) : pt.n_text;
                        probe_end = std::min<u64>(p_end_all, avail > (u64)k + 64 ? avail - (u64)k - 64 : 0);
                    } else if (upload_pending) probe_end = std::min<u64>(p_end_all, upload_avail > (u64)k + 64 ? upload_avail - (u64)k - 64 : 0);
                }
#endif
                if (probe_end < pb) probe_end = pb;
                DBuf<u32> probe(2);
                probe.fill_bytes(0);
                const u64 n_probe = std::min<u64>(32768, (probe_end - pb) / 4096 + 1);
                if (probe_end > pb) launch(n_probe, RestProbeFunctor<W>{t, tb, pb, probe_end, (probe_end - pb) / n_probe, probe.ptr()});
                tm->insert_rest_sampled = (double)(probe_end - pb) / (double)(p_end_all - pb);
                std::vector<InsertStats> st2(257); u32 h_probe[2] = {0, 0};
                { ReadBatch rb; rb.add(st2.data(), istats.ptr(), 257 * sizeof(InsertStats)); rb.add(h_probe, probe.ptr(), 8); rb.run(); }
                u64 claimed = 0;
                for (size_t q = 0; q < 256; q++) claimed += st2[q].claimed;
                if (st2[256].real == 0 && claimed * 4 <= first * 5) rest_at_once = true;
                const double known = h_probe[0] ? (double)h_probe[1] / (double)h_probe[0] : 1.0;
                rest_chunk = insert_chunk_rest_env() ? insert_chunk_rest_env() : (known >= 0.9 ? 16384 : known >= 0.6 ? 8192 : known >= 0.3 ? 4096 : 2048);
                tm->insert_rest_known = known;
                const double r2 = claimed > first ? (double)(claimed - first) / (double)first : 0.0;
                want_runs = rest_at_once && (copy_mode == 1 || (copy_mode == 2 && path_copy_pays(pt.n_text, hint, k, r2)));
                if (knobs().debug_arena) fprintf(stderr, "insert: second stretch %.4f new, one-launch rest %d, copying walk %d (mode %d)\n", r2, (int)rest_at_once, (int)want_runs, copy_mode);
            }
        }
#ifndef AC_EMU
        flush_fills();
        if (!evs.empty()) AC_HIP_CHECK(hipEventSynchronize(evs.back()));
        for (size_t i = 0; i + 1 < evs.size(); i += 2) {
            float ms = 0; AC_HIP_CHECK(hipEventElapsedTime(&ms, evs[i], evs[i + 1]));
            tm->insert_kernel_ms += ms;
        }
        for (hipEvent_t e : evs) (void)hipEventDestroy(e);
#endif
        tm->insert_launches += launches;
        std::vector<InsertStats> st = to_host(istats, 257);
        const bool ins_err = st[256].real != 0;
        const u64 full_at = ~st[256].claimed;
        st.pop_back();
        n_distinct = 0;
        u64 real = 0;
        for (auto& x : st) { n_distinct += x.claimed; real += x.real; }
        bool overflow = ins_err || (n_distinct * 10 > c * 7);
        if (!overflow) { tm->insert_real += real; tm->insert_positions += pt.n_text; break; }
        const u64 c_max = next_pow2(pt.n_bases * 4 + 1024);
        if (c >= c_max) throw DeviceError("k-mer table overflow");
        u64 want = c * 4;
        if (!ins_err) want = std::max(want, next_pow2(n_distinct * 2));
        else {
            u64 pb_full = 0, pe_full = p_end_all;
            for (u64 e : phase_end) { if (full_at < e) { pe_full = e; break; } pb_full = e; }
            const double done = std::sqrt((double)std::max<u64>(pb_full, pe_full / 4) * (double)pe_full);
            const double need = (double)c * 0.7 * (double)p_end_all / std::max(done, 1.0);
            want = std::max(want, next_pow2((u64)std::min(need * 2.0, 9.0e18)));
        }
        c = std::min(want, c_max);
        tm->insert_kernel_ms = 0; tm->insert_launches = 0;
        stream_sync();
        sl = DBuf<u64>(); sflags = DBuf<u64>();
        Arena::device().rewind(retry_mark);
    }
    if (n_distinct >= 0xFFFFFFF0ULL) throw DeviceError("too many distinct k-mers for 32-bit novel indices");
    {
        CapMemo* slot = nullptr;
        for (CapMemo& m : memo) if (m.n_text == pt.n_text && m.k == k && m.owners == memo_owners) slot = &m;
        if (!slot) slot = &memo[memo_next++ % 4];
        slot->n_text = pt.n_text; slot->k = k; slot->shift = table_shift(); slot->owners = memo_owners;
        slot->cap = (n_distinct * 2 > c && c * 2 <= next_pow2(pt.n_bases * 4 + 1024)) ? c * 2 : c;
    }
    *slots_out = std::move(sl);
    *cap_out = c;
    *n_distinct_out = n_distinct;
    *bm_out = std::move(nbm);
}

template <int W> void GraphBuilder::Impl::fragments() {
    DBuf<u64> lslots; DBuf<u64>& lbm = loc_bm; u64 lcap = 0, ln = 0;
    local_insert_of_shard = true;
    insert<W>(loc, tm->local_hint, &lslots, &lcap, &ln, &lbm);
    local_insert_of_shard = false;
    tm->n_local_distinct = ln;
    lap(&tm->insert);
    u64 nw = loc.n_text / 64 + 1;
    DBuf<u32> ns(nw + 1), ne(nw + 1), so(nw + 1), eo(nw + 1);
    ns.fill_bytes(0); ne.fill_bytes(0);
    launch(nw, RunEdgeCountFunctor{lbm.ptr(), nw, ns.ptr(), ne.ptr()});
    exclusive_scan_u32(ns.ptr(), so.ptr(), nw + 1);
    exclusive_scan_u32(ne.ptr(), eo.ptr(), nw + 1);
    u64 n_runs = read_scalar(so.ptr() + nw);
    if (n_runs != (u64)read_scalar(eo.ptr() + nw)) throw DeviceError("internal error: unbalanced novel runs");
    DBuf<u64> run_start(n_runs), run_end(n_runs);
    launch(nw, RunEdgeFillFunctor{lbm.ptr(), nw, so.ptr(), eo.ptr(), run_start.ptr(), run_end.ptr()});
    n_frags = n_runs + 2 * (u64)loc.n_seqs;
    DBuf<u64> blen(n_frags + 1);
    DBuf<u64>& fpos = frag_fpos; DBuf<u64>& boff = frag_boff;
    fpos.alloc(n_frags); boff.alloc(n_frags + 1);
    frag_meta.alloc(n_frags);
    launch(n_frags + 1, FragMetaFunctor{loc.ctx((int)k), run_start.ptr(), run_end.ptr(), n_runs, n_frags, fpos.ptr(), frag_meta.ptr(),
                                        blen.ptr(), counters.ptr() + 6});
    exclusive_scan_u64(blen.ptr(), boff.ptr(), n_frags + 1);
    frag_bytes = read_scalar(boff.ptr() + n_frags);
    {
        u32 frag_err = 0, pack_bad[2] = {0xFFFFFFFFu, 0xFFFFFFFFu};
        ReadBatch rb;
        rb.add(&frag_err, counters.ptr() + 6, 4);
        if (loc.check_alphabet && loc.pack_bad.size()) rb.add(pack_bad, loc.pack_bad.ptr(), 8);
        rb.run();
        if (loc.pack_bad.size()) loc.verify_alphabet(pack_bad);
        if (frag_err) throw DeviceError("internal error: novel run outside a sequence");
    }
    tm->n_fragments = n_frags; tm->fragment_bytes = frag_bytes;
    lap(&tm->fragments);
}

template <int W> void GraphBuilder::Impl::table() {
    PackedText& g = *G;
    check_sizes(g);
    const bool want_sib = k >= 3 && degree_flags() && (n_owners <= 1 || shard_degree_flags());
    insert<W>(g, tm->graph_hint, &slots, &cap, &N, &bm, want_sib);
    tm->table_capacity = cap;
    tm->n_distinct = N;
    lap(G == &loc ? &tm->insert : &tm->union_insert);
    const bool sib_by_pos = want_sib && n_owners <= 1;
    if (sib_by_pos) { sib.alloc(2 * (g.n_text / 64 + 2)); sib.fill_bytes(0); }
    else sib = DBuf<u64>();
    sibn = DBuf<u64>(); sib_pending = false;
    occupancy_bitmap(slots, cap, &occ, sib_by_pos ? sflags.ptr() : nullptr, sib_by_pos ? sib.ptr() : nullptr);
    if (n_owners <= 1) novel_list(N);
}

template <int W> void GraphBuilder::Impl::degrees() {
    PackedText& g = *G;
    Table tb = graph_table();
    Novel nv{bm.ptr(), wprefix.ptr()};
    kcontrib = DBuf<u32>(); pend = DBuf<u32>(); pidx = DBuf<u32>(); n_pending = n_first = 0;
    u32* kout = kinfo.ptr();
    const bool by_index = n_owners > 1 && sibn.size() != 0;
    const u64* sib_ptr = by_index ? sibn.ptr() : (sib.size() ? sib.ptr() : nullptr);
    EndSet es{nullptr, 0, nullptr, nullptr};
    if (sib_ptr && g.any_dots) {
        endset_mask = next_pow2(4 * (g.has_flags ? g.n_dotted : (u64)g.n_seqs) + 16) - 1;
        endset.alloc((endset_mask + 1) * W);
        endset.fill_bytes(0xFF);
        endset_bloom.alloc(2 * ENDSET_BLOOM_WORDS);
        endset_bloom.fill_bytes(0);
        es = EndSet{endset.ptr(), endset_mask, endset_bloom.ptr(), endset_bloom.ptr() + ENDSET_BLOOM_WORDS};
    }
    auto fill_end_set = [&] { if (es.keys) launch(2 * (u64)g.n_seqs, EndSetFunctor<W>{g.ctx((int)k), es}); };
    const u8* fflags = g.has_flags ? g.seq_flags.ptr() : nullptr;
    if (sib_ptr && degree_flags() == 1 && (!g.any_dots || es.keys)) {
        DBuf<u32> fslot;
        if (by_index) {
            pend.alloc(N + 1); pidx.alloc(N + 1);
            pend.fill_bytes_from(N * 4, 0);
            fslot.alloc((u64)g.n_seqs + 1);
            DBuf<u32> fcnt((u64)g.n_seqs + 1);
            fill_end_set();
            launch((u64)g.n_seqs + 1, FirstSlotCountFunctor{fflags, g.n_seqs, fcnt.ptr()});
            exclusive_scan_u32(fcnt.ptr(), fslot.ptr(), (u64)g.n_seqs + 1);
        }
        const Arena::Mark deg_mark = Arena::device().mark();
        DegWork wk;
        const u64 max_generic = std::min<u64>(N, 2 * ((u64)k - 1) * g.n_seqs);
        wk.rcap[0] = (u32)(N / DEG_REGIONS + N / (4 * DEG_REGIONS) + 64 * DEG_BATCH); wk.ocap[0] = N;
        wk.rcap[1] = (u32)(max_generic / DEG_REGIONS + 64 * DEG_BATCH); wk.ocap[1] = max_generic;
        if (degree_region_cap()) { wk.rcap[0] = std::min(wk.rcap[0], degree_region_cap()); wk.rcap[1] = std::min(wk.rcap[1], degree_region_cap()); }
        DBuf<u64> items(wk.words()); DBuf<u32> counts(DEG_LISTS * (DEG_REGIONS + 1));
        counts.fill_bytes(0);
        wk.items = items.ptr(); wk.counts = counts.ptr();
        if (!by_index) fill_end_set();
        const u64 n_thr = (((N + DEG_BATCH - 1) / DEG_BATCH) + 63) & ~63ULL;
        launch_full(n_thr, DegreeLightFunctor<W>{g.ctx((int)k), npos.ptr(), kinfo.ptr(), g.any_dots, bm.ptr(), sib_ptr, es, wk, N, n_thr, by_index ? 1 : 0,
                                                 by_index ? pend.ptr() : nullptr});
        DBuf<u32> kc_tmp;
        if (by_index) {
            exclusive_scan_u32(pend.ptr(), pidx.ptr(), N + 1);
            u32 hp[2];
            { ReadBatch rb; rb.add(&hp[0], pidx.ptr() + N, 4); rb.add(&hp[1], fslot.ptr() + g.n_seqs, 4); rb.run(); }
            n_pending = hp[0]; n_first = hp[1];
            kc_tmp.alloc(n_pending + n_first + 1); kc_tmp.fill_bytes(0);
            kout = kc_tmp.ptr();
        }
        launch((u64)DEG_LISTS * DEG_REGIONS * DEG_PROBE_THREADS, DegreeProbeFunctor<W>{g.ctx((int)k), tb, npos.ptr(), kout, g.any_dots, wk, es, by_index ? pidx.ptr() : nullptr});
#ifdef AC_EMU
        if (knobs().degree_diag) {
            u64 c0 = 0, c1 = 0;
            for (u32 r = 0; r <= DEG_REGIONS; r++) { c0 += wk.count(0)[r]; c1 += wk.count(1)[r]; }
            fprintf(stderr, "degree diag: N %llu, queued real %llu, generic %llu, left open %llu, any_dots %d\n", (unsigned long long)N,
                    (unsigned long long)c0, (unsigned long long)c1, (unsigned long long)n_pending, (int)g.any_dots);
        }
#endif
        if (by_index) launch(g.n_seqs, FirstFunctor<W>{g.ctx((int)k), tb, nv, kinfo.ptr(), fflags, fslot.ptr(), kc_tmp.ptr() + n_pending});
        items = DBuf<u64>(); counts = DBuf<u32>();
        const u32* kc_src = kc_tmp.ptr();
        kc_tmp = DBuf<u32>();
        Arena::device().rewind(deg_mark);
        if (by_index) {
            kcontrib.alloc(n_pending + n_first + 1);
            const u64 kc_bytes = (n_pending + n_first + 1) * 4;
            if (kcontrib.ptr() != kc_src) {
                const u8* dst_b = (const u8*)kcontrib.ptr(); const u8* src_b = (const u8*)kc_src;
                if (dst_b + kc_bytes <= src_b || src_b + kc_bytes <= dst_b) { Arena::keep_readable(kc_src, kc_bytes); copy_d2d(kcontrib.ptr(), kc_src, kc_bytes); }
                else {
                    const Arena::Mark bounce_mark = Arena::device().mark();
                    DBuf<u32> pad((u64)(src_b + kc_bytes - dst_b) / 4 + 1), bounce(n_pending + n_first + 1);
                    Arena::keep_readable(kc_src, kc_bytes);
                    copy_d2d(bounce.ptr(), kc_src, kc_bytes);
                    copy_d2d(kcontrib.ptr(), bounce.ptr(), kc_bytes);
                    stream_sync();
                    pad = DBuf<u32>(); bounce = DBuf<u32>();
                    Arena::device().rewind(bounce_mark);
                }
            }
            tm->n_degrees_open = n_pending;
            lap(&tm->degree);
            return;
        }
    } else {
        fill_end_set();
        launch(N, DegreeFunctor<W>{g.ctx((int)k), tb, npos.ptr(), kinfo.ptr(), g.any_dots, 0, bm.ptr(), sib.size() && n_owners <= 1 ? sib.ptr() : nullptr, es});
    }
    launch(g.n_seqs, FirstFunctor<W>{g.ctx((int)k), tb, nv, kout, fflags, nullptr, nullptr});
    lap(&tm->degree);
}

template <int W> void GraphBuilder::Impl::unitigs() {
    PackedText& g = *G;
    TextCtx t = g.ctx((int)k);
    Table tb = graph_table();
    Novel nv{bm.ptr(), wprefix.ptr()};
    launch(N, HeadFunctor{npos.ptr(), kinfo.ptr(), head.ptr(), N});
    inclusive_scan_u32(head.ptr(), scan.ptr(), N);
    U = read_scalar(scan.ptr() + (N - 1));
    ustart.alloc((u64)U + 1);
    int seed_keep = seed_prefix_bits();
    if (seed_keep <= 0) { int lg = 1; while ((1ULL << lg) < (u64)U) lg++; seed_keep = std::min(64, ((2 * lg + 8 + 7) / 8) * 8); }
    RadixScratch seed_rs; DBuf<u32> seed_big(1, true);
    if (seed_prefix_sort()) seed_rs.prepare(U, seed_keep);
    launch(N, UnitigStartFunctor{head.ptr(), scan.ptr(), ustart.ptr(), N});
    lap(&tm->segment);

    DBuf<MinVal<W>> umin(U);
    const int mk = minkey_variant() >= 0 ? minkey_variant() : ((W > 4 || (W >= 3 && N >= 32 * (u64)U)) ? 2 : 1);
    if (mk == 2) {
        const u64 n_waves = (N + 63) / 64;
        DBuf<MinPre> upre(U), wfirst(n_waves), wlast(n_waves);
        MinPreArgs a{t, npos.ptr(), scan.ptr(), N, upre.ptr(), wfirst.ptr(), wlast.ptr(), minkey_prefix_bases()};
        launch_wave_kernel(minpre_wave_kernel<W>, (N + 255) / 256, 0, a);
        launch(U, MinFinishFunctor<W>{t, npos.ptr(), ustart.ptr(), U, N, upre.ptr(), wfirst.ptr(), wlast.ptr(), umin.ptr()});
    } else if constexpr (W <= 4) {
        if (mk == 1) {
            const u64 n_waves = (N + 63) / 64;
            DBuf<MinVal<W>> wfirst(n_waves), wlast(n_waves);
            MinWaveArgs<W> a{t, npos.ptr(), scan.ptr(), N, umin.ptr(), wfirst.ptr(), wlast.ptr()};
            launch_wave_kernel(minkey_wave_kernel<W>, (N + 255) / 256, 0, a);
            launch(U, MinJoinFunctor<W>{ustart.ptr(), U, N, wfirst.ptr(), wlast.ptr(), umin.ptr()});
        } else {
            DBuf<MinVal<W>> vals(N); DBuf<u32> seg(N);
            launch(N, CKeyFunctor<W>{t, npos.ptr(), scan.ptr(), vals.ptr(), seg.ptr()});
            reduce_by_segment(seg.ptr(), vals.ptr(), N, umin.ptr(), U, MinOp<W>(), counters.ptr() + 3);
        }
    } else {
        DBuf<u32> umin_idx(U);
        segment_argmin(scan.ptr(), N, umin_idx.ptr(), U, MinIdxOp<W>{t, npos.ptr()}, counters.ptr() + 3);
        launch(U, UnitigMinFunctor<W>{t, npos.ptr(), umin_idx.ptr(), umin.ptr()});
    }
    lap(&tm->minkey);

    order.alloc(U);
    bool seeds_ordered = false;
    if (seed_prefix_sort()) {
        DBuf<u64> wkey(U);
        const int keep = seed_keep;
        DBuf<u32> by_prefix(U);
        launch(U, SeedPrefixFunctor<W>{umin.ptr(), (int)k, wkey.ptr(), keep, by_prefix.ptr()});
        sort_pairs_u64_u32(wkey, by_prefix, U, 64, 0, 64 - keep, &seed_rs);
        DBuf<u32> settled(U); DBuf<u32>& big = seed_big;
        const bool defer = deferred_sort_checks();
        launch(U, SeedTieFunctor<W>{by_prefix.ptr(), wkey.ptr(), U, umin.ptr(), settled.ptr(), seed_max_group(), defer ? sort_flags.ptr() : big.ptr()});
        if (defer || read_scalar(big.ptr()) == 0) {
            order = std::move(settled);
            DBuf<MinVal<W>> sorted(U);
            launch(U, GatherMinFunctor<W>{order.ptr(), umin.ptr(), sorted.ptr()});
            umin = std::move(sorted);
            seeds_ordered = true;
        }
    }
    if (!seeds_ordered) launch(U, IotaFunctor{order.ptr()});
    if (seeds_ordered) {
    } else if constexpr (W <= 4) {
        if ((u64)U >= seed_radix_limit() || seed_prefix_sort()) {
            DBuf<u64> wkey(U);
            for (int word = W - 1; word >= 0; word--) {
                launch(U, MinWordFunctor<W>{order.ptr(), umin.ptr(), word, wkey.ptr()});
                sort_pairs_u64_u32(wkey, order, U, 64);
            }
            DBuf<MinVal<W>> sorted(U);
            launch(U, GatherMinFunctor<W>{order.ptr(), umin.ptr(), sorted.ptr()});
            umin = std::move(sorted);
        } else {
            sort_by_key_cmp(umin, order, U, MinValLess<W>());
        }
    } else {
        sort_keys_cmp(order, U, MinValIdxLess<W>{umin.ptr()});
        DBuf<MinVal<W>> sorted(U);
        launch(U, GatherMinFunctor<W>{order.ptr(), umin.ptr(), sorted.ptr()});
        umin = std::move(sorted);
    }
    rank.alloc(U); ulen.alloc(U); ustartpos.alloc(U); useq_off.alloc((u64)U + 1); uorient.alloc(U);
    DBuf<u64> ulen64((u64)U + 1);
    launch((u64)U + 1, UnitigMetaFunctor<W>{order.ptr(), ustart.ptr(), npos.ptr(), umin.ptr(), U, N, rank.ptr(), ulen.ptr(),
                                            ulen64.ptr(), ustartpos.ptr(), uorient.ptr()});
    exclusive_scan_u64(ulen64.ptr(), useq_off.ptr(), (u64)U + 1);
    UnitigCtx uc{head.ptr(), scan.ptr(), rank.ptr(), uorient.ptr(), ustart.ptr(), ulen.ptr(), U, N};
    lap(&tm->rank);

    links.alloc((u64)U * 10); wlinks.alloc((u64)U * 10);
    DBuf<V16> ui(U);
    launch(U, WalkInfoFunctor{uc, nullptr, ui.ptr()});
    launch((u64)U * 2, LinksFunctor<W>{t, tb, nv, uc, order.ptr(), npos.ptr(), g.any_dots, links.ptr(), wlinks.ptr(), counters.ptr() + 3, ui.ptr()});
    lap(&tm->links);
}

template <int W> void GraphBuilder::Impl::walk_queries() {
    const u32 PC = path_chunk(N, U);
    u64 n_walkers = (loc.n_text + PC - 1) / PC;
    cplan = CopyPlan();
    if (run_rows && loc_bm.size() && PC <= 65535) {
        const u64 nw = loc.n_text / 64 + 1;
        DBuf<u32> wcnt(nw + 1);
        loc_wprefix.alloc(nw + 1);
        launch(nw + 1, PopcFunctor{loc_bm.ptr(), wcnt.ptr(), nw});
        exclusive_scan_u32(wcnt.ptr(), loc_wprefix.ptr(), nw + 1);
        if (walk_copy_prepare<W>(PC, Novel{loc_bm.ptr(), loc_wprefix.ptr()})) n_walkers = cplan.NW;
    }
    n_queries = n_walkers + loc.n_seqs;
    qkeys.alloc(n_queries * W);
    launch(n_queries, WalkQueryFunctor<W>{loc.ctx((int)k), PC, n_walkers, qkeys.ptr(), cplan.ok ? cplan.w_begin.ptr() : nullptr});
}
template <int W> void GraphBuilder::Impl::route_queries(u32 n_shards, u64* d_routed_keys, u64* counts_host) {
    DBuf<u64> owner64(n_queries), first(n_shards);
    qidx.alloc(n_queries);
    first.fill_bytes(0xFF);
    launch(n_queries, QueryOwnerFunctor<W>{qkeys.ptr(), (int)k, n_shards, my_owner, owner64.ptr(), qidx.ptr()});
    int bits = 1;
    while ((1u << bits) < n_shards) bits++;
    sort_pairs_u64_u32(owner64, qidx, n_queries, bits);
    launch(n_queries, OwnerBoundsFunctor{owner64.ptr(), first.ptr()});
    launch(n_queries, QueryGatherFunctor<W>{qkeys.ptr(), qidx.ptr(), d_routed_keys});
    std::vector<u64> h_first = to_host(first, n_shards);
    u64 end = n_queries;
    for (u32 o = n_shards; o-- > 0;) {
        if (h_first[o] == ~0ULL) { counts_host[o] = 0; continue; }
        counts_host[o] = end - h_first[o];
        end = h_first[o];
    }
}
template <int W> void GraphBuilder::Impl::answer_queries(const u64* d_keys, u64 n, u64* d_out) {
    launch(n, AnswerFunctor<W>{G->ctx((int)k), graph_table(), d_keys, d_out});
}

template <int W> bool GraphBuilder::Impl::walk_copy_prepare(u32 PC, const Novel& nv_text) {
    TextCtx t = loc.ctx((int)k);
    cplan = CopyPlan();
    const Arena::Mark mk = Arena::device().mark();
    DBuf<u32> rfirst(run_rows + 1);
    exclusive_scan_u32(run_count.ptr(), rfirst.ptr(), run_rows + 1);
    const u64 R0 = read_scalar(rfirst.ptr() + run_rows);
    if (R0 == 0 || R0 >= 0xFFFFFFF0ULL) { Arena::device().rewind(mk); return false; }
    DBuf<RunRec> sorted(R0);
    launch(run_rows * RUN_ROW, RunGatherFunctor{runs.ptr(), run_count.ptr(), rfirst.ptr(), sorted.ptr()});
    DBuf<u32> ok(R0 + 1), at(R0 + 1); DBuf<u64> covered(1, true); DBuf<u32> overlap(1, true);
    ok.fill_bytes(0);
    DBuf<RunRec> fixed(R0); DBuf<u32> fseq(R0);
    launch(R0, RunFilterFunctor{sorted.ptr(), fixed.ptr(), R0, nv_text, loc.n_text, ok.ptr(), covered.ptr(), t, overlap.ptr(), run_piece(), fseq.ptr()});
    exclusive_scan_u32(ok.ptr(), at.ptr(), R0 + 1);
    const u64 Rb = R0 + loc.n_text / run_piece() + 1;
    CopyPlan& c = cplan;
    c.rr.alloc(Rb); c.rseq.alloc(Rb);
    launch(R0, RunCompactFunctor{fixed.ptr(), ok.ptr(), at.ptr(), c.rr.ptr(), run_piece(), fseq.ptr(), c.rseq.ptr(), nv_text, loc.n_text});
    DBuf<u64> gw(Rb + 2);
    c.wfirst.alloc(Rb + 2);
    launch(Rb + 2, GapWalkersFunctor{c.rr.ptr(), at.ptr() + R0, loc.n_text, PC, gw.ptr()});
    exclusive_scan_u64(gw.ptr(), c.wfirst.ptr(), Rb + 2);
    u64 h_cov = 0, NW = 0; u32 h_R = 0, h_overlap = 0;
    { ReadBatch rb; rb.add(&h_cov, covered.ptr(), 8); rb.add(&h_R, at.ptr() + R0, 4); rb.add(&h_overlap, overlap.ptr(), 4); rb.add(&NW, c.wfirst.ptr() + (Rb + 1), 8); rb.run(); }
    const u64 R = h_R;
    if (knobs().debug_arena) fprintf(stderr, "path copy: %llu runs on the list, %llu pieces usable, covering %llu of %llu positions, %llu walkers\n", (unsigned long long)R0, (unsigned long long)R, (unsigned long long)h_cov, (unsigned long long)loc.n_text, (unsigned long long)NW);
    if (R == 0 || h_overlap || h_cov * 2 < loc.n_text || NW == 0 || NW >= 0xFFFFFFF0ULL) {
        cplan = CopyPlan();
        Arena::device().rewind(mk);
        return false;
    }
    c.w_begin.alloc(NW); c.w_end.alloc(NW); c.w_gap.alloc(NW);
    launch(NW, WalkerRangeFunctor{c.rr.ptr(), R, loc.n_text, PC, c.wfirst.ptr(), c.w_begin.ptr(), c.w_end.ptr(), c.w_gap.ptr()});
    c.R = R; c.NW = NW; c.Rb = Rb; c.ok = true;
    return true;
}
template <int W> void GraphBuilder::Impl::walk_copy_finish(u32 PC) {
    TextCtx t = loc.ctx((int)k), g = G->ctx((int)k);
    Table tb = graph_table();
    Novel nv{bm.ptr(), wprefix.ptr()};
    UnitigCtx uc{head.ptr(), scan.ptr(), rank.ptr(), uorient.ptr(), ustart.ptr(), ulen.ptr(), U, N};
    CopyPlan& c = cplan;
    const u64 R = c.R, NW = c.NW;
    DBuf<u64> wcount(NW + 1), woff(NW + 1);
    const u64 n_slots = ((NW + 63) / 64) * 64 * PC;
    DBuf<int32_t> stage(n_slots); DBuf<u16> stage_off(n_slots);
    DBuf<u32> seq_tid(loc.n_seqs), seq_j(loc.n_seqs);
    wcount.fill_bytes(0);
    const bool filter = maybe_dest_valid;
    walk_tables(filter);
    walked_plain = false;
    DBuf<V16> uinfo(U);
    launch(U, WalkInfoFunctor{uc, filter ? maybe_dest.ptr() : nullptr, uinfo.ptr()});
    launch(NW, PathWalkFunctor<W>{t, g, tb, nv, uc, uinfo.ptr(), wl_text.ptr(), PC, stage.ptr(), wcount.ptr(), seq_tid.ptr(), seq_j.ptr(),
                                 depth_u.ptr(), minpos_fwd_u.ptr(), minpos_rev_u.ptr(), counters.ptr() + 4, filter ? maybe_dest.ptr() : nullptr,
                                 pos_cap_now, 0, walk_answers, NW, c.w_begin.ptr(), c.w_end.ptr(), stage_off.ptr(), nullptr, nullptr});
    exclusive_scan_u64(wcount.ptr(), woff.ptr(), NW + 1);
    const u64 NE = read_scalar(woff.ptr() + NW);
    DBuf<int32_t> ent(NE); DBuf<u64> ent_pos(NE), ent_end(NE); DBuf<u8> ent_want(NE); DBuf<u32> ent_gap(NE);
    launch_full(NW, WalkCompactFunctor{stage.ptr(), stage_off.ptr(), wcount.ptr(), woff.ptr(), c.w_begin.ptr(), c.w_gap.ptr(), PC, NW, uinfo.ptr(),
                                       ent.ptr(), ent_pos.ptr(), ent_end.ptr(), ent_want.ptr(), ent_gap.ptr()});
    DBuf<u64> ra(R), rcnt(R + 1), seg(2 * R + 2), segoff(2 * R + 2); DBuf<u32> cov(NE + 1), copies(NE + 1);
    cov.fill_bytes(0);
    launch(R, RunRangeFunctor{c.rr.ptr(), ent_pos.ptr(), ent_end.ptr(), NE, ra.ptr(), rcnt.ptr(), cov.ptr()});
    launch(2 * R + 2, SegCountFunctor{c.wfirst.ptr(), woff.ptr(), rcnt.ptr(), R, seg.ptr()});
    exclusive_scan_u64(seg.ptr(), segoff.ptr(), 2 * R + 2);
    inclusive_scan_u32(cov.ptr(), copies.ptr(), NE + 1);
    n_ent = read_scalar(segoff.ptr() + (2 * R + 1));
// ... 95 lines not shown
```

### autocycler_amd/csrc/graph_tail.hip

```cpp
#include "graph_impl.hpp"

namespace ac {

[[maybe_unused]] static bool renum_two_pass() { return knobs().renum_two_pass; }
[[maybe_unused]] static u32 renum_max_group() { return knobs().renum_max_group; }
[[maybe_unused]] static void renumber_sort(DBuf<u32>& order, u32 U, const u32* len, const u64* off, const u8* seq, const u32* depth, u32* flag, bool deferred = false,
                                           RadixScratch* sc = nullptr, int len_bits = 32, bool order_is_identity = false) {
    if (U <= 1) return;
    DBuf<u32> backup(deferred && !renum_two_pass() ? 0 : U);
    if (backup.size()) copy_d2d(backup.ptr(), order.ptr(), (size_t)U * 4);
    DBuf<u64> prefix(U), key(U);
    UnitigLess less{len, off, seq, depth};
    u32 zero = 0;
    if (!renum_two_pass()) {
        if (order_is_identity) launch(U, RenumKeyPassFunctor{RenumKeyFunctor{len, off, seq, prefix.ptr()}, RenumPassFunctor{order.ptr(), len, depth, prefix.ptr(), 2, key.ptr()}});
        else {
            launch(U, RenumKeyFunctor{len, off, seq, prefix.ptr()});
            launch(U, RenumPassFunctor{order.ptr(), len, depth, prefix.ptr(), 2, key.ptr()});
        }
        sort_pairs_u64_u32(key, order, U, 32 + std::min(std::max(len_bits, 1), 32), 0, 0, sc);
        launch(U, RenumTieFunctor{order.ptr(), U, len, depth, prefix.ptr(), less, flag, 0, renum_max_group()});
#ifdef AC_EMU
        if (knobs().degree_diag) {
            u64 groups = 0, members = 0, biggest = 0, cur = 1, longest = 0;
// ... 250 lines not shown
        launch(C, LevelPredsFunctor{L, cand.ptr(), clist.ptr(), prio.ptr(), C, preds.ptr(), npred.ptr(), touch.ptr()});
        if (partitioned) {
            DBuf<u32> parent(C);
            jowner.alloc(C); owned_count.alloc(1); owned_count.fill_bytes(0);
            launch(C, UfInitFunctor{parent.ptr()});
            launch(C, UfUnionFunctor{preds.ptr(), npred.ptr(), C, parent.ptr()});
            launch(C, UfOwnerFunctor{parent.ptr(), m.n_owners, jowner.ptr()});
            launch_full((J + 63) & ~63ULL, OwnedDirtyFunctor{cand.ptr(), prio.ptr(), jowner.ptr(), m.my_owner, dirty.ptr(), owned_count.ptr(), J});
            gpre.alloc(U, true); gpost.alloc(U, true);
        }
        u32 max_level = 1;
        for (int round = 0;; round++) {
            if (round) changed.fill_bytes(0);
            for (int it = 0; it < 8; it++)
                launch(C, LevelRelaxFunctor{preds.ptr(), npred.ptr(), C, level.ptr(), changed.ptr() + it, it ? changed.ptr() + it - 1 : nullptr, changed.ptr() + 8});
            const std::vector<u32> hc = to_host(changed, 9);
            max_level = std::max(max_level, hc[8]);
            if (hc[7] == 0) break;
        }
        lkey.alloc(C);
        launch(C, LevelKeyFunctor{level.ptr(), lkey.ptr()});
        int level_bits = 1;
        while (level_bits < 32 && (max_level >> level_bits)) level_bits++;
        sort_pairs_u64_u32(lkey, clist, C, level_bits, 0, 0, &sort_lv);
        const u32 LV_TABLE = expand_level_table();
        DBuf<u32> bstart((u64)LV_TABLE + 2);
        launch(C, LevelBoundsFunctor{lkey.ptr(), C, bstart.ptr(), LV_TABLE});
        hb = to_host(bstart, (u64)LV_TABLE + 2);
        n_levels = hb[0];
        if (n_levels > LV_TABLE) {
            DBuf<u32> big((u64)n_levels + 2);
            launch(C, LevelBoundsFunctor{lkey.ptr(), C, big.ptr(), n_levels});
            hb = to_host(big, (u64)n_levels + 2);
        }
        hb.resize((size_t)n_levels + 2);
        hb[n_levels + 1] = (u32)C;
        e = ExpState{cur, ev.ptr(), pool.ptr(), pool_used.ptr(), m.minpos_fwd.ptr(), m.minpos_rev.ptr(), dirty.ptr(), cand.ptr(), L, shifted.ptr(), touch.ptr()};
    }

    void rewrite(bool last) {
        const u32 U = m.U;
        if (partitioned) launch(U, ExpFoldFunctor{e, gpre.ptr(), gpost.ptr()});
        launch((u64)U + 1, ExpLenFunctor{e, len64.ptr(), U});
        exclusive_scan_u64(len64.ptr(), noff.ptr(), (u64)U + 1);
        const bool defer_total = last && !partitioned && (seq_writer_plain() || (final_total < ((u64)16 << 20) && !seq_writer_forced()));
        if (defer_total) { write_seqs(1, &e, noff.ptr(), final_total, alt, true); final_total_pending = true; }
        else { final_total = read_scalar(noff.ptr() + U); write_seqs(1, &e, noff.ptr(), final_total, alt); }
        launch(U, ExpResetFunctor{e, noff.ptr(), coff.ptr(), clen.ptr()});
        std::swap(cur, alt);
        e.cur = cur;
        if (!last) pool_used.fill_bytes(0);
        moved_since_rewrite = 0;
    }

    void run_level(u32 lv) {
        const u64 cnt = (u64)(hb[lv + 1] - hb[lv]);
        if (cnt) launch_wave_kernel(expand_wave_kernel<16>, (cnt * 16 + 255) / 256, 0, e, (const u32*)clist.ptr(), (u64)hb[lv], cnt, (u32)pool.size(), m.counters.ptr() + 7);
    }

    void run_passes() {
        const u32 sparse_max = expand_sparse_max();
        const u32 sub_limit = (u32)(pool.size() / 2 / EXP_SUBPOOLS / 2);
        for (u32 check = 0;; check++) {
            u64* const sh_words = shifted2.ptr() + 2 * (u64)(check % SHIFT_CHECKS);
            if (check && check % SHIFT_CHECKS == 0) shifted2.fill_bytes(0);
            for (int half = 0; half < 2; half++) {
                e.shifted = sh_words + half;
                for (u32 lv = 1; lv <= n_levels; lv++) run_level(lv);
            }
            if (sparse_max) {
                launch_full((C + 63) & ~63ULL, MopCompactFunctor{clist.ptr(), lkey.ptr(), dirty.ptr(), (u64*)preds.ptr(), changed.ptr() + 9, C});
                const MopState ms{(u64*)preds.ptr(), changed.ptr() + 9, prio.ptr(), level.ptr(), sh_words, changed.ptr() + 10, sparse_max, expand_sparse_list() ? expand_sparse_list() : 8 * sparse_max, sub_limit, std::min(MOP_BATCH, expand_sparse_batch())};
                launch_wave_kernel_sized(expand_mopup_kernel<0>, 1, MOP_THREADS, 0, e, ms, (u32)pool.size(), m.counters.ptr() + 7);
            }
            u64 sh[2]; u32 used = 0; u32 mop[3] = {0, 0, 0};
            {
                std::vector<u32> pu(EXP_SUBPOOLS + 1);
                ReadBatch rb;
                rb.add(sh, sh_words, 16);
                rb.add(pu.data(), pool_used.ptr(), (EXP_SUBPOOLS + 1) * 4);
                if (sparse_max) rb.add(mop, changed.ptr() + 10, 12);
                rb.run();
                for (u32 q = 0; q < EXP_SUBPOOLS; q++) used = std::max(used, pu[q]);
                if (pu[EXP_SUBPOOLS]) used = 0xFFFFFFFFu;
            }
            moved_since_rewrite += sh[0] + sh[1];
            if (sh[0] == 0) { passes += 1; break; }
            passes += 2;
            if (sh[1] == 0) break;
            if (mop[0]) {
                passes += (int)mop[1];
                sparse_sweeps += mop[1]; sparse_start = mop[2];
                if (mop[0] == 1) break;
            }
            if (used > sub_limit || expand_rewrite_always()) rewrite(false);
        }
    }

    void merge_ranks() {
        const u32 U = m.U;
        DBuf<u8> fown((u64)U * 3); DBuf<int32_t> lens3((u64)U * 3 + 1);
        launch(U, FieldOwnerFunctor{L, cand.ptr(), prio.ptr(), jowner.ptr(), m.n_owners, fown.ptr()});
        launch(U, OwnedLensFunctor{e, fown.ptr(), gpre.ptr(), gpost.ptr(), m.my_owner, lens3.ptr()});
        const int32_t neg_passes = -(int32_t)passes;
        copy_h2d(lens3.ptr() + (u64)U * 3, &neg_passes, 4);
        stream_sync();
        m.tail_xchg(lens3.ptr(), (u64)U * 3, 1, 0);
        m.tail_xchg(lens3.ptr() + (u64)U * 3, 1, 1, 1);
        launch((u64)U + 1, Lens3SumFunctor{lens3.ptr(), len64.ptr(), U});
        exclusive_scan_u64(len64.ptr(), noff.ptr(), (u64)U + 1);
        int32_t min_neg = 0;
        {
            ReadBatch rb;
            rb.add(&final_total, noff.ptr() + U, 8);
            rb.add(&min_neg, lens3.ptr() + (u64)U * 3, 4);
            rb.add(&n_cand_owned, owned_count.ptr(), 4);
            rb.run();
        }
        passes = -min_neg;
        if (final_total > seq_alt.size()) throw DeviceError("internal error: merged sequences longer than before expand_repeats");
        const u32 per = 16;
        launch((final_total + per - 1) / per, MergeSeqFunctor{e, fown.ptr(), gpre.ptr(), gpost.ptr(), m.my_owner, lens3.ptr(), noff.ptr(), U, final_total, alt, per});
        stream_sync();
        m.tail_xchg(alt, final_total, 0, 0);
        launch(U, ExpResetFunctor{e, noff.ptr(), coff.ptr(), clen.ptr()});
        std::swap(cur, alt);
        e.cur = cur;
    }

    void send_sequences() {
        if (!want_graph) return;
        const u32 U = m.U;
        out->seq_block = PinnedPool::get().alloc(final_total + 64);
        const u64 other_late = (u64)U * 28 + n_links * sizeof(Link);
        if (seq_codes_transfer() == 2 || (seq_codes_transfer() == 1 && final_total >= ((u64)32 << 20) && final_total > 2 * other_late)) {
            const u64 nw = (final_total + 31) / 32;
            seq_words.alloc(nw); seq_bad.alloc(1); seq_bad.fill_bytes(0);
            launch(nw, SeqPack2Functor{cur, final_total, seq_words.ptr(), seq_bad.ptr()});
            seq_words_block = PinnedPool::get().alloc(nw * 8);
            side.after_main();
            copy_d2h_async(seq_words_block.p, seq_words.ptr(), nw * 8, side.stream());
            seq_job.words = (const u64*)seq_words_block.p; seq_job.out = (u8*)out->seq_block.p; seq_job.total = final_total;
            seq_job.landed = side.mark(); seq_job.side = &side;
#ifndef AC_EMU
            AC_HIP_CHECK(hipGetDevice(&seq_job.dev));
            seq_expand_start(seq_job, 12);
#endif
            seq_as_codes = true;
        } else {
            side.after_main();
            copy_d2h_async(out->seq_block.p, cur, final_total, side.stream());
        }
    }

    void finalise_records() {
        const u32 U = m.U;
        order2.alloc(U);
        copy_d2d(order2.ptr(), order1.ptr(), (size_t)U * 4);
        renumber_sort(order2, U, clen.ptr(), coff.ptr(), cur, m.depth.ptr(), defer_sorts ? m.sort_flags.ptr() + 1 : renum_flag.ptr(), defer_sorts, &sort2, len_bits);
        number_len.alloc(U); number_len_text.alloc(U); loff.alloc((u64)U + 1);
        number_only.alloc(host_numbers ? U : 0);
        meta.alloc((size_t)U * 24);
        u64* d_seq_begin = (u64*)meta.ptr();
        double* d_depth = (double*)(meta.ptr() + (size_t)U * 8);
        u32* d_seq_len = (u32*)(meta.ptr() + (size_t)U * 16);
        u32* d_seed_index = (u32*)(meta.ptr() + (size_t)U * 20);
        out->k = m.k;
        out->n_kmers = 2 * (u64)m.N;
        out->n_unitigs = U;
        late_by_host = late_copies() == 2 || (late_copies() == 1 && final_total + (u64)U * 28 + n_links * sizeof(Link) >= ((u64)256 << 20));
        launch(U, FinalMetaFunctor{order2.ptr(), coff.ptr(), clen.ptr(), m.depth.ptr(), lcnt.ptr(), number_len.ptr(), d_seq_begin, d_depth,
                                   d_seq_len, lcount.ptr(), host_numbers ? number_only.ptr() : nullptr, d_seed_index, m.order.ptr(), number_len_text.ptr(), m.uorient.ptr()});
        if (host_numbers) {
            number_block = PinnedPool::get().alloc((size_t)U * 4);
            remap_job.path = (int32_t*)out->path_block.p; remap_job.n_ent = m.n_ent;
            if (host_stretch) { remap_job.rec_val = (const int32_t*)rec_val_block.p; remap_job.rec_pos = (const u32*)rec_pos_block.p; remap_job.n_rec = n_stretch; }
            remap_job.number = (const u32*)number_block.p; remap_job.n_unitigs = U;
            remap_job.ent_limit = host_stretch ? (u64)stretch_split_wave * remap_block() : ~0ULL;
            const u32* d_number_only = number_only.ptr();
            const int remap_threads = (int)(host_stretch ? 2 * upload_threads() : upload_threads());
            late_copy([this, U, d_number_only, remap_threads]() {
                copy_d2h_async(number_block.p, d_number_only, (size_t)U * 4, side.stream());
                remap_job.landed = side.mark(); remap_job.side = &side;
#ifndef AC_EMU
                AC_HIP_CHECK(hipGetDevice(&remap_job.dev));
                path_remap_start(remap_job, remap_threads);
#endif
            });
        }
        if (want_graph) {
            out->meta_block = PinnedPool::get().alloc((size_t)U * 24);
            const u8* d_meta = meta.ptr();
            late_copy([this, U, d_meta]() { copy_d2h_async(out->meta_block.p, d_meta, (size_t)U * 24, side.stream()); });
        }
        exclusive_scan_u64(lcount.ptr(), loff.ptr(), (u64)U + 1);
        links_out.alloc(n_links);
        launch(U, LinkOutFunctor{order2.ptr(), L, number_len.ptr(), loff.ptr(), links_out.ptr()});
        if (want_graph) {
            out->links_block = PinnedPool::get().alloc(n_links * sizeof(Link));
            const Link* d_links_out = links_out.ptr();
            late_copy([this, d_links_out]() { copy_d2h_async(out->links_block.p, d_links_out, n_links * sizeof(Link), side.stream()); });
        }
    }

    void finalise_paths() {
        const u64 n_ent = m.n_ent;
        if (host_numbers) {
            const u64 RB = remap_block();
            const u64 n_waves = (n_ent + RB - 1) / RB;
            const u64 w_split = host_stretch ? std::min<u64>(stretch_split_wave, n_waves) : n_waves;
            if (w_split) launch_full(w_split * 64, RemapFunctor{m.ent_val.ptr(), number_len_text.ptr(), m.path_off.ptr(), n_seqs, n_ent, sums.ptr(), 0, (u32)RB, nullptr, false});
            if (w_split < n_waves) {
                const u64 n_chunks = 4, per_chunk = std::max<u64>((n_waves - w_split + n_chunks - 1) / n_chunks, 64);
                for (u64 w = w_split; w < n_waves; w += per_chunk) {
                    const u64 cnt = std::min<u64>(per_chunk, n_waves - w);
                    launch_full(cnt * 64, RemapFunctor{m.ent_val.ptr(), number_len_text.ptr(), m.path_off.ptr(), n_seqs, n_ent, sums.ptr(), w, (u32)RB, nullptr, true});
                    const u64 b = w * RB, e2 = std::min<u64>((w + cnt) * RB, n_ent);
                    const int32_t* d_ent = m.ent_val.ptr();
                    late_copy([this, d_ent, b, e2]() { copy_d2h_async((int32_t*)out->path_block.p + b, d_ent + b, (e2 - b) * 4, side.stream()); });
                }
            }
        } else {
            if (want_paths) out->path_block = PinnedPool::get().alloc(n_ent * 4);
            const u64 RB = remap_block();
            const u64 n_waves = (n_ent + RB - 1) / RB;
            const u64 n_chunks = n_ent * 4 >= ((u64)256 << 20) ? 8 : 4;
            const u64 per_chunk = std::max<u64>((n_waves + n_chunks - 1) / n_chunks, 64);
            int turn = 0;
            for (u64 w = 0; w < n_waves; w += per_chunk) {
                u64 cnt = std::min<u64>(per_chunk, n_waves - w);
                launch_full(cnt * 64, RemapFunctor{m.ent_val.ptr(), number_len_text.ptr(), m.path_off.ptr(), n_seqs, n_ent, sums.ptr(), w, (u32)RB, nullptr, true});
                if (want_paths) {
                    u64 b = w * RB, e2 = std::min<u64>((w + cnt) * RB, n_ent);
                    const int which = n_chunks == 8 ? (turn++ & 1) : 0;
                    side.after_main(which);
                    copy_d2h_async((int32_t*)out->path_block.p + b, m.ent_val.ptr() + b, (e2 - b) * 4, side.stream(which));
                }
            }
        }
        issue_late_copies();
        m.lap(&m.tm->finalize);
    }

    void collect_and_check() {
        const u32 U = m.U; const u64 n_ent = m.n_ent;
        PackedText& loc = m.loc;
        std::vector<u64> h_sums(n_seqs);
        out->path_off.resize((size_t)n_seqs + 1);
        std::vector<u32> errs(8);
        u32 pack_bad[2] = {0xFFFFFFFFu, 0xFFFFFFFFu};
        u32 h_sort_flags[2] = {0, 0};
        u64 n_links_check = 0, final_total_read = 0; u32 h_seq_bad = 0;
        {
            ReadBatch rb;
            rb.add(h_sums.data(), sums.ptr(), (size_t)n_seqs * 8);
            rb.add(out->path_off.data(), m.path_off.ptr(), ((size_t)n_seqs + 1) * 8);
            rb.add(errs.data(), m.counters.ptr(), 8 * 4);
            rb.add(h_sort_flags, m.sort_flags.ptr(), 8);
            rb.add(&n_links_check, loff.ptr() + U, 8);
            if (final_total_pending) rb.add(&final_total_read, noff.ptr() + U, 8);
            if (loc.check_alphabet && loc.pack_bad.size()) rb.add(pack_bad, loc.pack_bad.ptr(), 8);
            if (seq_as_codes) rb.add(&h_seq_bad, seq_bad.ptr(), 4);
            rb.run();
        }
        const double t_main_done = now_s();
        side.sync();
        const double t_copies_done = now_s();
        if (seq_as_codes) {
#ifdef AC_EMU
            for (u64 b = 0; b < final_total; b += 4096) seq_expand_range(seq_job.words, seq_job.out, b, std::min<u64>(b + 4096, final_total));
#endif
            seq_expand_finish(seq_job);
            if (seq_job.ready.load() == 3) throw DeviceError("internal error: the sequence codes did not reach the host");
            if (h_seq_bad) {
                copy_d2h_async(out->seq_block.p, cur, final_total, side.stream());
                side.sync();
            }
        }
        if (host_numbers) {
#ifdef AC_EMU
            if (host_stretch) { for (u64 b = 0; b < n_stretch; b += 7) path_stretch_range(remap_job, b, std::min<u64>(b + 7, n_stretch), &remap_job.bad); }
            else path_remap_range(remap_job.path, n_ent, remap_job.number, U, &remap_job.bad);
#endif
            path_remap_finish(remap_job);
        }
        m.tm->path_stretches = host_stretch ? n_stretch : 0;
        if (knobs().debug_arena && seq_as_codes)
            fprintf(stderr, "d2h: sequence codes: job started %.3f ms before stream 0 drained, its codes had landed %.3f ms after that start, %.1f MB written out in %.3f ms more\n",
                    (t_main_done - seq_job.t_start.load()) * 1e3, (seq_job.t_ready.load() - seq_job.t_start.load()) * 1e3, final_total / 1e6, (seq_job.t_last.load() - seq_job.t_ready.load()) * 1e3);
        if (knobs().debug_arena && host_numbers)
            fprintf(stderr, "d2h: the host's renumbering threads started %.3f ms %s stream 0 drained (their table had landed) and were done %.3f ms later\n",
                    std::fabs(remap_job.t_ready.load() - t_main_done) * 1e3, remap_job.t_ready.load() < t_main_done ? "before" : "after", (remap_job.t_last.load() - remap_job.t_ready.load()) * 1e3);
        if (knobs().debug_arena)
            fprintf(stderr, "d2h: copies landed %.3f ms after stream 0 drained, host renumbering done %.3f ms later; late results %.1f MB (sequences %.1f, unitig records %.1f, links %.1f, number table %.1f), entries %.1f MB\n",
                    (t_copies_done - t_main_done) * 1e3, (now_s() - t_copies_done) * 1e3, (final_total + (double)U * 24 + n_links * sizeof(Link) + (host_numbers ? (double)U * 4 : 0)) / 1e6,
                    final_total / 1e6, (double)U * 24 / 1e6, n_links * sizeof(Link) / 1e6, host_numbers ? (double)U * 4 / 1e6 : 0.0, n_ent * 4 / 1e6);
        if (loc.pack_bad.size()) loc.verify_alphabet(pack_bad);
        if (errs[7] & 128u) throw NeedExactPositions();
        if (h_sort_flags[0] || h_sort_flags[1]) {
            if (!m.deferred_sort_checks()) throw DeviceError("internal error: a sort flag was left set by a checked sort");
            throw NeedCheckedSorts();
        }
        if (errs[7]) throw DeviceError("internal error: expand_repeats pool overflow");
        if (n_links_check != n_links) throw DeviceError("internal error: link counts disagree");
        if (final_total_pending) { if (final_total_read > final_total) throw DeviceError("internal error: expand_repeats lengthened the sequences"); final_total = final_total_read; }
        if (errs[3] || errs[4])
            throw DeviceError("internal error: inconsistent unitig ends (codes " + std::to_string(errs[3]) + "/" + std::to_string(errs[4]) + ")");
        if (remap_job.bad.load()) throw DeviceError("internal error: path entries without a unitig");
        if (want_graph) {
            out->seq_begin = (const u64*)out->meta_block.p;
            out->depth = (const double*)((const u8*)out->meta_block.p + (size_t)U * 8);
            out->seq_len = (const u32*)((const u8*)out->meta_block.p + (size_t)U * 16);
            out->seed_index = (const u32*)((const u8*)out->meta_block.p + (size_t)U * 20);
            out->links = (const Link*)out->links_block.p;
        }
        if (want_paths) out->path = (const int32_t*)out->path_block.p;
        out->n_links = n_links;
        out->n_path = n_ent;
        u64 n_self = errs[5];
        u64 links_one_way = (n_links + n_self) / 2;
        out->pre = GraphStats{U, links_one_way, total};
        out->post = GraphStats{U, links_one_way, final_total};
        out->simplify_passes = passes;
        for (u32 s = 0; s < n_seqs; s++)
            if (h_sums[s] != (u64)loc.h_len[s])
                throw DeviceError("internal error: path length mismatch for sequence " + std::to_string(s + 1));
        m.lap(&m.tm->d2h);
        m.tm->total_device = now_s() - m.t_begin;
        m.tm->launches = rt_counters().launches; m.tm->readbacks = rt_counters().readbacks;
        if (knobs().debug_arena)
            fprintf(stderr, "arena: used %.1f MB (peak %.1f) of %.1f MB (n_text %.1f MB), %.3f s in hipMalloc / hipFree so far\n", Arena::device().total_used() / 1e6,
                    Arena::device().peak() / 1e6, Arena::device().capacity() / 1e6, loc.n_text / 1e6, Arena::device().alloc_seconds());
    }
};

}

void GraphBuilder::Impl::tail(FinalGraph* out, bool want_graph, bool want_paths) {
    TailRun run(*this, out, want_graph, want_paths);
    run.run();
}

void tail_warm() {
#ifndef AC_EMU
    hipLaunchKernelGGL((expand_wave_kernel<16>), dim3(1), dim3(256), 0, 0, ExpState{}, (const u32*)nullptr, (u64)0, (u64)0, 0u, (u32*)nullptr);
    (void)hipGetLastError();
#endif
}

}
```

### autocycler_amd/csrc/kernels_table.inc

```
struct PackCheck { const u64* seq_off; const u32* seq_len; const u16* d1; const u16* d2; u32 n_seqs; int k; u32* bad; };
AC_D void pack_check(const PackCheck& c, const u8* buf, u64 base, u32 m, u64 n_text) {
    u32 cnt = 0;
    for (u32 mm = m; mm; mm &= mm - 1) {
        const int i = ctz32(mm);
        const u64 p = base + (u64)i;
        if (p >= n_text) break;
        cnt++;
        const u8 ch = buf[i];
        if (c.n_seqs == 0 || p < c.seq_off[0]) { if (!(p == 0 && ch == '$')) atomic_min32(c.bad, 1u); continue; }
        u32 lo = 0, hi = c.n_seqs;
        while (hi - lo > 1) { const u32 mid = lo + ((hi - lo) >> 1); if (c.seq_off[mid] <= p) lo = mid; else hi = mid; }
        const u64 rel = p - c.seq_off[lo], plen = (u64)c.seq_len[lo] + (u64)c.k - 1;
        const bool ok = rel < plen ? (ch == '.' && (rel < c.d1[lo] || rel >= plen - c.d2[lo])) : (rel == plen && ch == '$');
        if (!ok) atomic_min32(c.bad, lo + 1);
    }
    if (cnt) atomic_add32(c.bad + 1, cnt);
}
struct PackFunctor {
    const u8* text; u64 n_text; u64* bits; u32* mask32; u64 first;
    PackCheck chk;
    AC_D void operator()(u64 tid) const {
        tid += first;
        u64 base = tid * 32;
        u64 w = 0; u32 m = 0;
        alignas(16) u8 buf[32];
        if (base + 32 <= n_text && ((uintptr_t)(text + base) & 15) == 0) {
            const V16* src = (const V16*)(text + base);
            *(V16*)(buf) = src[0];
            *(V16*)(buf + 16) = src[1];
        } else {
            for (int i = 0; i < 32; i++) buf[i] = (base + (u64)i < n_text) ? text[base + (u64)i] : (u8)'$';
        }
#pragma unroll
        for (int i = 0; i < 32; i++) {
            u32 ch = buf[i];
            u32 bad = !(ch == 'A' || ch == 'C' || ch == 'G' || ch == 'T');
            u32 c = bad ? 0u : (((ch >> 1) ^ (ch >> 2)) & 3u);
            w |= (u64)c << (62 - 2 * i);
            m |= bad << i;
        }
        bits[tid] = w; mask32[tid] = m;
        if (m && chk.bad) pack_check(chk, buf, base, m, n_text);
    }
};

struct MaskTableFunctor {
    const u64* seq_off; const u32* seq_len; const u16* d1; const u16* d2; u32 n_seqs; int k; u64 n_text; u64* mask;
    AC_D void set_range(u64 a, u64 b) const {
        while (a < b) {
            const int lo = (int)(a & 63);
            const u64 n = (b - a < (u64)(64 - lo)) ? b - a : (u64)(64 - lo);
            const u64 m = (n == 64 ? ~0ULL : ((1ULL << n) - 1)) << lo;
            atomic_or64(&mask[a >> 6], m);
            a += n;
        }
    }
    AC_D void operator()(u64 s) const {
        if (s == n_seqs) { set_range(n_text, (n_text + 63) & ~63ULL); return; }
        const u64 off = seq_off[s], plen = (u64)seq_len[s] + (u64)k - 1;
        set_range(off - 1, off + d1[s]);
        set_range(off + plen - d2[s], off + plen + 1);
    }
};

struct InsertStats { u64 real; u64 claimed; };
template <int W> AC_D u64 insert_one(const TextCtx& t, const Table& tb, u64 p, u32* claimed, u32* err, bool* same, bool* mine_now) {
    const int k = t.k;
    if (text_mask_count(t.mask, p, k) == 0) {
        Key<W> fwd = text_extract<W>(t.bits, p, k);
        Key<W> rc = key_rc<W>(fwd, k);
        bool flipped = key_lt<W>(rc, fwd);
        Key<W> uk = flipped ? rc : fwd;
        uk.w[0] |= (u64)255 << 56;
        return table_insert<W>(t, tb, uk, false, flipped, p, claimed, err, same, mine_now);
    }
    *mine_now = false;
    XKmer<W> x;
    if (xkmer_at<W>(t, p, &x)) {
        bool flipped, sm;
        Key<W> uk = xk_canonical<W>(x, k, &flipped);
        table_insert<W>(t, tb, uk, true, flipped, p, claimed, err, &sm, mine_now);
    }
    return NOREF;
}
AC_HD int wave_match(const TextCtx& t, u64 a, u64 b, bool same, u64 off, u64 maxlen, const u64* nov = nullptr, u64 q0 = 0, bool* by_nov = nullptr, u64 nov_from = ~0ULL) {
    if (by_nov) *by_nov = false;
    if (off >= maxlen) return 0;
    int m;
    if (same) m = match_word_fwd(t.bits, t.mask, a + off, b + off);
    else if (off > b) return 0;
    else m = match_word_rev(t.bits, t.mask, a + off, b - off);
    if (nov && m > 0 && (same ? q0 + off < nov_from : (q0 >= off + 31 ? q0 - off - 31 < nov_from : true))) {
        const u32 firsts = same ? mask_word(nov, q0 + off) : (q0 >= off ? mask_word_rev(nov, q0 - off) : 0u);
        const int lim = ctz32(~firsts);
        if (lim < m) { m = lim; if (by_nov) *by_nov = true; }
    }
    return m;
}
static const u64 LONG_RUN = 256;
AC_D u64 wave_follow(const TextCtx& t, u64 pj, u64 qj, bool sj, u64 c1, int lane, const u64* nov, bool* again, u64 nov_from) {
    const u64 maxlen = c1 - 1 - pj;
    const u64 a = pj + (u64)t.k, b = sj ? qj + (u64)t.k : qj - 1;
    const u64 q0 = sj ? qj + 1 : qj - 1;
    u64 n = 0;
    *again = false;
    while (n < maxlen) {
        bool by_nov;
        int tmatch = wave_match(t, a, b, sj, n + 32 * (u64)lane, maxlen, nov, q0, &by_nov, nov_from);
        const u64 bal = wv::ballot(tmatch < 32);
        if (bal == 0) { n += 2048; continue; }
        const int f = ctz64(bal);
        n += 32 * (u64)f + (u64)wv::shfl(tmatch, f);
        *again = wv::shfl((int)by_nov, f) != 0;
        break;
    }
    return n > maxlen ? maxlen : n;
}
template <int W, bool PROF>
AC_KERNEL void __launch_bounds__(256) AC_WAVES_PER_EU(W <= 4 ? 8 : 1, 8)
insert_wave_kernel(TextCtx t, Table tb, u64 p_begin, u64 p_end, u32 chunk, InsertStats* stats, u32* err, u64* prof) {
    const int lane = wv::lane();
    u64 cy_open = 0, cy_wide = 0, cy_follow = 0, n_open = 0, n_wide = 0, n_follow = 0, t_wave = 0;
    if (PROF) t_wave = (u64)clock64();
    const u64 wave = ((u64)wv::bid() * 256 + wv::tid()) >> 6;
    const u64 c0 = p_begin + wave * (u64)chunk;
    if (c0 >= p_end) return;
    const u64 c1 = (c0 + chunk < p_end) ? c0 + chunk : p_end;
    u32 claimed = 0, real = 0, noted = 0;
    u64 p = c0;
    bool opener = true;
    while (p < c1) {
        if (wv::uniform((int)*(volatile const u32*)err)) break;
        if (opener) {
            u64 q = NOREF; bool same = false, mine = false;
            u64 t0 = 0;
            if (PROF) t0 = (u64)clock64();
            if (lane == 0) {
                real++;
                q = insert_one<W>(t, tb, p, &claimed, err, &same, &mine);
                if (mine) atomic_xor64(&tb.novel[p >> 6], 1ULL << (p & 63));
            }
            q = (u64)wv::shfl64((unsigned long long)q, 0);
            if (PROF) { u64 t1 = (u64)clock64(); cy_open += t1 - t0; n_open++; t0 = t1; }
            if (q != NOREF) {
                const bool s0 = wv::shfl((int)same, 0) != 0;
                bool again;
                const u64 n = wave_follow(t, p, q, s0, c1, lane, tb.runs ? tb.novel : nullptr, &again, p_begin);
                if (PROF) { cy_follow += (u64)clock64() - t0; n_follow++; }
                if (lane == 0) run_note(tb, wave, noted, p, q, s0, n);
                p += 1 + n;
                opener = n >= LONG_RUN || again;
            } else {
                p += 1;
                opener = false;
            }
            continue;
        }
        const u64 pi = p + (u64)lane;
        u64 q = NOREF; bool same = false, mine = false;
        u64 t0 = 0;
        if (PROF) t0 = (u64)clock64();
        if (pi < c1) { real++; q = insert_one<W>(t, tb, pi, &claimed, err, &same, &mine); }
        const u64 mine_mask = wv::ballot(mine);
        if (mine_mask) {
            const int sh = (int)(p & 63);
            if (lane == 0) atomic_xor64(&tb.novel[p >> 6], mine_mask << sh);
            if (lane == 1 && sh && (mine_mask >> (64 - sh))) atomic_xor64(&tb.novel[(p >> 6) + 1], mine_mask >> (64 - sh));
        }
        const u64 hits = wv::ballot(q != NOREF);
        if (PROF) { u64 t1 = (u64)clock64(); cy_wide += t1 - t0; n_wide++; t0 = t1; }
        u64 next = p + 64;
        if (hits) {
            const int jl = 63 - clz64(hits);
            const u64 qj = (u64)wv::shfl64((unsigned long long)q, jl);
            const bool sj = wv::shfl((int)same, jl) != 0;
            const u64 pj = p + (u64)jl;
            bool again;
            const u64 n = wave_follow(t, pj, qj, sj, c1, lane, tb.runs ? tb.novel : nullptr, &again, p_begin);
            if (PROF) { cy_follow += (u64)clock64() - t0; n_follow++; }
            if (lane == 0) run_note(tb, wave, noted, pj, qj, sj, n);
            if (pj + 1 + n > next) next = pj + 1 + n;
            opener = n >= LONG_RUN || (again && pj + 1 + n >= p + 64);
        }
        p = next;
    }
    if (PROF && lane == 0) {
        atomic_add64(prof + 0, cy_open); atomic_add64(prof + 1, n_open); atomic_add64(prof + 2, cy_wide); atomic_add64(prof + 3, n_wide);
        atomic_add64(prof + 4, cy_follow); atomic_add64(prof + 5, n_follow); atomic_add64(prof + 6, (u64)clock64() - t_wave); atomic_add64(prof + 7, 1);
        atomic_max64(prof + 8, (u64)clock64() - t_wave);
    }
    for (int o = 32; o; o >>= 1) { real += (u32)wv::shfl_xor((int)real, o); claimed += (u32)wv::shfl_xor((int)claimed, o); }
    if (lane == 0) {
        InsertStats* st = stats + (wave & 255);
        atomic_add64(&st->real, (u64)real);
        if (claimed) atomic_add64(&st->claimed, (u64)claimed);
        run_note_done(tb, wave, noted);
    }
}
template <int W> struct RestProbeFunctor {
    TextCtx t; Table tb; u64 pb, pe, stride; u32* out;
    AC_D void operator()(u64 i) const {
        const u64 p = pb + i * stride + (((i + 1) * 0x9E3779B97F4A7C15ULL >> 24) % (stride ? stride : 1));
        if (p >= pe || text_mask_count(t.mask, p, t.k) != 0) return;
        Key<W> fwd = text_extract<W>(t.bits, p, t.k);
        Key<W> rc = key_rc<W>(fwd, t.k);
        Key<W> uk = key_lt<W>(rc, fwd) ? rc : fwd;
        uk.w[0] |= (u64)255 << 56;
        if (!table_owns(tb, key_place<W>(uk, t.k, false, key_hash<W>(uk)).home)) return;
        atomic_add32(out, 1u);
        if (table_find<W>(t, tb, uk, false).found) atomic_add32(out + 1, 1u);
    }
};
struct MarkFunctor {
    const u64* slots; u64* occ; const u64* sflags; u64* sib;
    AC_D void operator()(u64 s, bool valid) const {
        u64 v = valid ? slots[s] : SLOT_EMPTY;
        bool full = v != SLOT_EMPTY;
        u64 b = wv::ballot(full);
        if ((s & 63) == 0 && valid) occ[s >> 6] = b;
        if (!sflags || !full) return;
        const u64 fl = (sflags[s >> 5] >> (2 * (s & 31))) & 3;
        const u64 p = slot_pos(v);
        if (fl) atomic_or64(&sib[p >> 5], fl << (2 * (p & 31)));
    }
};
struct PopcFunctor {
    const u64* bm; u32* cnt; u64 n;
    AC_HD void operator()(u64 w) const { cnt[w] = w < n ? (u32)popc64(bm[w]) : 0u; }
};
template <int UNUSED> AC_KERNEL void __launch_bounds__(256) fill_novel_wave_kernel(const u64* bm, const u32* wprefix, u64* npos, u64 n_words) {
    const u64 w = (u64)wv::bid() * 256 + wv::tid();
    const int lane = wv::lane();
    const u64 w0 = w - (u64)lane;
    if (w0 >= n_words) return;
    const u64 x = w < n_words ? bm[w] : 0;
    const u32 start = w < n_words ? wprefix[w] : 0;
    const u32 cnt = (u32)popc64(x);
    const u32 base = (u32)wv::shfl((int)start, 0);
    const u32 rel = w < n_words ? start - base : 0xFFFFFFFFu;
    const u64 lastv = n_words - w0 - 1;
    const u32 total = (u32)wv::shfl((int)(rel + cnt), lastv > 63 ? 63 : (int)lastv);
    const u32 xlo = (u32)x, xhi = (u32)(x >> 32);
    for (u32 t0 = 0; t0 < total; t0 += 64) {
        const u32 t = t0 + (u32)lane;
        int lo = 0;
#pragma unroll
        for (int step = 32; step; step >>= 1) {
            const int cand = lo + step;
            const u32 v = (u32)wv::shfl((int)rel, cand & 63);
            if (cand < 64 && v <= t) lo = cand;
        }
        const u32 r0 = (u32)wv::shfl((int)rel, lo);
        u64 v = (u64)(u32)wv::shfl((int)xlo, lo) | ((u64)(u32)wv::shfl((int)xhi, lo) << 32);
        if (t >= total) continue;
        u32 r = t - r0, pos = 0;
#pragma unroll
        for (int sh = 32; sh; sh >>= 1) {
            const u32 c = (u32)popc64(v & ((1ULL << sh) - 1));
            if (r >= c) { r -= c; v >>= sh; pos += (u32)sh; }
        }
        npos[(u64)base + t] = (w0 + (u64)lo) * 64 + pos;
    }
}
```

### include/autocycler_hip.h

```cpp
#ifndef AUTOCYCLER_HIP_H
#define AUTOCYCLER_HIP_H

#include <stddef.h>
#include <stdint.h>

#ifdef __cplusplus
extern "C" {
#endif

typedef struct ac_graph ac_graph;

typedef struct {
    const uint8_t* fwd;
    uint32_t length;
    uint16_t id;
} ac_seq_view;

typedef struct { uint32_t pos; uint16_t seq_id_and_strand; } ac_position;
typedef struct { int32_t a; int32_t b; } ac_link;
typedef struct { uint32_t unitigs; uint64_t links_one_way; uint64_t total_length; } ac_stats;

typedef struct {
    double h2d, pack, insert, collect_sort, degree, segment, minkey, rank, paths, links, seqs, d2h;
    double total_device;
    double expand;
    double insert_kernel_ms;
    uint64_t insert_positions;
    uint64_t table_capacity, n_distinct, n_path_entries;
    uint32_t simplify_passes;
    uint32_t insert_launches;
    uint64_t insert_real;
    double analysis;
    double finalize;
    uint32_t n_candidates;
    uint32_t n_levels;
    double fragments;
    double union_pack, union_insert;
    uint64_t n_local_distinct, n_fragments, fragment_bytes;
    double upload_device_ms;
    uint64_t path_runs_copied, path_entries_walked;
    uint64_t position_retries;
    uint32_t n_candidates_owned;
    uint32_t launches;
    uint32_t readbacks;
    uint64_t n_degrees_open;
    uint64_t sort_retries;
    double insert_rest_known;
    double insert_rest_sampled;
    uint64_t path_stretches;
    uint32_t expand_sparse_sweeps;
    uint32_t expand_sparse_start;
} ac_timings;

int ac_compress_build(uint32_t k, uint32_t assembly_count, const ac_seq_view* seqs, uint32_t n_seqs, int device,
                      ac_graph** out);

int ac_compress_build_multi(uint32_t k, uint32_t assembly_count, const ac_seq_view* seqs, uint32_t n_seqs, const int* devices,
                            int n_devices, ac_graph** out);
typedef struct {
    uint32_t n_ranks; int transport;
    uint64_t bytes_fragments, bytes_bitmap, bytes_degrees, bytes_links, bytes_queries, bytes_answers, bytes_reduce;
    uint64_t queries_total, queries_sent_away;
    uint64_t table_capacity_max, table_capacity_sum;
    uint64_t union_text_bytes, fragments, distinct;
    double seconds_total, seconds_exchange_max;
    uint64_t candidates_total, candidates_owned_max;
    uint64_t bytes_sibling;
    uint64_t bytes_tail;
    uint64_t degrees_open;
    uint64_t bytes_received_max;
    uint64_t path_runs_copied;
} ac_multi_info;
int ac_multi_info_get(const ac_graph*, ac_multi_info* out);
size_t ac_multi_info_get_sized(const ac_graph*, ac_multi_info* out, size_t out_size);

typedef struct {
    uint32_t failed;
    uint64_t first_bad_unitig, first_bad_link, first_bad_path_entry, first_bad_sequence, first_bad_base;
    uint64_t unitigs, links, path_entries, bases_checked, self_mirror_links;
    double seconds;
    uint32_t checks;
    uint64_t first_bad_junction;
} ac_verify_report;
int ac_verify_graph(const ac_graph* graph, const ac_seq_view* seqs, uint32_t n_seqs, int device, ac_verify_report* report);
int ac_verify_graph_device(const ac_graph* graph, const void* d_text, uint64_t n_text, const uint64_t* seq_off, const uint32_t* seq_len,
                           uint32_t n_seqs, int device, ac_verify_report* report);

int ac_decompress_device(const ac_graph*, int device, uint8_t* out, uint64_t out_bytes);

int ac_selftest_primitives(int device, uint64_t n, uint64_t seed, int end_bit, int key_kind);

int ac_selftest_scan(int device, int kind, const void* in, uint64_t n, int in_place, int misalign_in, int misalign_out, void* out);
int ac_selftest_radix(int device, const uint64_t* keys, const void* vals, uint64_t n, int begin_bit, int end_bit, int val_kind, uint64_t prep_n, int prep_bits,
                      int prep_reuse, uint64_t* keys_out, void* vals_out);
int ac_selftest_segments(int device, int op, const uint32_t* seg, const uint64_t* vals, uint64_t n, uint64_t n_segments, int deferred_err, void* out, uint32_t* err_out);
int ac_selftest_sort_cmp(int device, int form, const uint64_t* key_a, const uint32_t* key_b, const uint32_t* vals, uint64_t n, uint64_t* key_a_out, uint32_t* key_b_out,
                         uint32_t* vals_out);
int ac_selftest_scan_pool(int device, int op, uint64_t value, uint64_t* out);
int ac_selftest_wave(int device, int program, const uint64_t* in_u64, const int32_t* aux_i32, const uint64_t* live_mask, uint64_t* out_u64);

int ac_selftest_fills(int device, const uint64_t* regions, uint64_t n_regions, int trigger, int mode, uint8_t* span, uint64_t span_bytes, uint32_t* launches_out);
int ac_selftest_fill_order(int device, uint64_t n, int byte1, uint64_t w_lo, uint64_t w_hi, int w_val, uint64_t from2, int byte2, uint64_t upto3, int byte3, uint8_t* out);
int ac_selftest_readback(int device, const uint8_t* data, uint64_t n_data, int path, const uint64_t* items, uint64_t n_items, uint8_t* out, uint32_t* counters_out);
int ac_selftest_scalar_chain(int device, const uint64_t* values, uint64_t n, uint64_t* out, uint32_t* counters_out);
int ac_selftest_arena(int device, const uint64_t* ops, uint64_t n_ops, uint64_t* totals_out, uint64_t* allocs_out, const uint8_t* live, uint64_t* wrong_out);
int ac_selftest_launch(int device, int which, uint64_t n, uint64_t* slots_out, uint32_t* info_out);
int ac_selftest_atomics(int device, int op, uint64_t init, uint64_t expected, const uint64_t* operand, const uint32_t* target, uint32_t n_words, uint64_t* words_out,
                        uint64_t* returns_out);
int ac_selftest_side_order(int device, int mode, int which, uint32_t seed, uint64_t n_words, uint32_t* out_words);
int ac_selftest_event_ring(int device, int op, const uint8_t* kinds, uint32_t n_more, uint64_t* out);

int ac_pack_text(const uint8_t* text, uint64_t n_text, uint64_t* bits, uint32_t* mask32, int force_scalar);

int ac_compress_build_device(uint32_t k, uint32_t assembly_count, const void* d_text, uint64_t n_text,
                             const uint64_t* seq_off, const uint32_t* seq_len, const uint16_t* seq_ids,
                             const uint16_t* seq_d1, const uint16_t* seq_d2, uint32_t n_seqs, int device,
                             ac_graph** out);

typedef struct ac_shard ac_shard;
int ac_shard_begin(uint32_t k, uint32_t local_assembly_count, const void* d_text, uint64_t n_text, const uint64_t* seq_off,
                   const uint32_t* seq_len, const uint16_t* seq_ids, const uint16_t* seq_d1, const uint16_t* seq_d2,
                   uint32_t n_seqs, int device, ac_shard** out);
int ac_shard_fragment_sizes(const ac_shard*, uint64_t* text_bytes, uint64_t* n_fragments);
int ac_shard_fragments_export(ac_shard*, void* d_text_out , void* d_meta_out );
uint64_t ac_shard_fragment_packed_words(const ac_shard*, uint64_t union_off);
int ac_shard_fragments_export_packed(ac_shard*, uint64_t union_off, void* d_words_u64, void* d_meta_out );
int ac_shard_build_union_packed(ac_shard*, uint32_t rank, uint32_t n_shards, const void* d_staged_words_u64, const uint64_t* first_word,
                                const uint64_t* n_words, uint64_t n_union_text, const void* d_meta, uint64_t n_fragments_total);
uint64_t ac_shard_local_distinct(const ac_shard*);
void ac_shard_set_distinct_upper_bound(ac_shard*, uint64_t n);
int ac_shard_build_union(ac_shard*, uint32_t rank, uint32_t n_shards, const void* d_union_text, uint64_t n_union_text,
                         const void* d_meta, uint64_t n_fragments_total);
uint64_t ac_shard_table_capacity(const ac_shard*);
uint64_t ac_shard_bitmap_words(const ac_shard*);
int ac_shard_bitmap_export(ac_shard*, void* d_out_u64);
int ac_shard_build_novel(ac_shard*, const void* d_bitmap_sum_u64 );
uint64_t ac_shard_distinct_count(const ac_shard*);
uint64_t ac_shard_sib_words(const ac_shard*);
int ac_shard_sib_export(ac_shard*, void* d_out_u64 );
int ac_shard_degrees(ac_shard*, const void* d_sib_sum_u64);
uint64_t ac_shard_degree_bytes(const ac_shard*);
int ac_shard_degrees_export(ac_shard*, void* d_out_u8 );
int ac_shard_build_graph(ac_shard*, const void* d_degrees_sum_u8 );
uint32_t ac_shard_unitig_count(const ac_shard*);
int ac_shard_links_export(ac_shard*, void* d_links_i32 , void* d_wlinks_i64 );
int ac_shard_links_import(ac_shard*, const void* d_links_sum_i32 , const void* d_wlinks_sum_i64 );
uint64_t ac_shard_query_count(const ac_shard*);
uint32_t ac_shard_query_key_words(const ac_shard*);
int ac_shard_queries_export(ac_shard*, void* d_out_u64 );
int ac_shard_answer(ac_shard*, const void* d_keys_u64, uint64_t n_queries, void* d_out_u64 );
int ac_shard_walk(ac_shard*, const void* d_answers_u64 );
int ac_shard_queries_route(ac_shard*, uint32_t n_shards, void* d_routed_keys_u64 ,
                           uint64_t* counts );
int ac_shard_walk_routed(ac_shard*, const void* d_routed_answers_u64 );
int ac_shard_reduce_export(ac_shard*, void* d_sum_i32 , void* d_min_i32 );
int ac_shard_reduce_import(ac_shard*, const void* d_sum_i32, const void* d_min_i32);
typedef int (*ac_allreduce_fn)(void* user, void* d_buf, uint64_t count, int dtype, int op);
int ac_shard_set_allreduce(ac_shard*, ac_allreduce_fn fn, void* user);
int ac_device_copy(void* dst, const void* src, uint64_t bytes, int device);
int ac_shard_finish(ac_shard*, int want, ac_graph** out);
uint64_t ac_shard_path_entries(const ac_shard*);
int ac_shard_paths_export(ac_shard*, void* d_out_i32 );
void ac_shard_free(ac_shard*);
int ac_graph_set_paths(ac_graph*, uint32_t n_seqs_total, const uint16_t* seq_ids, const uint32_t* seq_lens,
                       const uint64_t* path_counts, const void* d_path_i32, int device);
uint32_t ac_graph_seq_count(const ac_graph*);
int ac_path_counts(const ac_graph*, uint64_t* counts );

int ac_end_repair_device(uint32_t k, void* d_text, uint64_t n_text, const uint64_t* seq_off, const uint32_t* seq_len,
                         uint16_t* seq_d1, uint16_t* seq_d2, uint32_t n_seqs, int device, double* seconds, uint64_t* n_matches);

int ac_pairwise_distances(const ac_graph*, int device, double* out);

typedef struct { uint32_t status, begin, end, trimmed_length; } ac_trim_slice;
typedef struct { ac_trim_slice start_end, hairpin; uint32_t hairpin_start_trimmed, hairpin_end_trimmed; } ac_trim_result;
typedef struct {
    uint64_t size;
    uint32_t c_se, c_hp;
    uint32_t chosen;
    uint32_t launches;
    uint64_t cells;
    double seconds_device;
} ac_trim_summary;
int ac_trim_paths(const ac_graph*, double min_identity, uint32_t max_unitigs, int device, ac_trim_result* out ,
                  ac_trim_summary* summary );
int ac_trim_path_slices(const int32_t* path_entries, const uint64_t* path_off, uint32_t n_seqs, const uint32_t* weights, uint32_t n_weights,
                        double min_identity, uint32_t max_unitigs, int device, ac_trim_result* out, ac_trim_summary* summary);
#define AC_ALIGN_GAP 0
#define AC_ALIGN_NONE 0xFFFFFFFFu
typedef struct { int32_t a_unitig; uint32_t a_index; int32_t b_unitig; uint32_t b_index; } ac_alignment_piece;
int ac_overlap_alignment(const int32_t* a, const int32_t* b, uint32_t n, const uint32_t* weights, uint32_t n_weights, double min_identity,
                         uint32_t max_unitigs, int skip_diagonal, int device, ac_alignment_piece* pieces, uint32_t* n_pieces);
uint32_t ac_trim_max_unitigs(void);

typedef struct ac_resolve ac_resolve;
typedef struct {
    int32_t start, end;
    uint32_t depth;
    uint32_t n_distinct;
    uint64_t best_off;
    uint64_t best_total;
    uint64_t first_distinct;
    uint32_t best_len, status;
    uint32_t conflicting, culled;
    uint32_t cull_rank, reserved;
} ac_bridge;
typedef struct {
    uint64_t size;
    uint64_t jobs;
    uint64_t jobs_not_launched;
    uint64_t cells;
    uint64_t largest_job_cells;
    uint32_t launches, reserved;
    double seconds_device;
} ac_resolve_summary;
int ac_resolve_bridges(const ac_graph*, int device, ac_resolve** out);
int ac_resolve_bridge_paths(const int32_t* path_entries, const uint64_t* path_off, uint32_t n_seqs, const uint32_t* consensus_weight,
                            const uint32_t* weights, uint32_t n_weights, int device, ac_resolve** out);
int ac_resolve_anchors(const ac_resolve*, const uint32_t** anchors , uint32_t* n);
int ac_resolve_bridge_records(const ac_resolve*, const ac_bridge** bridges, uint32_t* n);
int ac_resolve_best_paths(const ac_resolve*, const int32_t** entries, uint64_t* n_entries );
int ac_resolve_distinct_paths(const ac_resolve*, const int32_t** entries, const uint64_t** path_off, const uint32_t** multiplicity, uint64_t* n_paths);
size_t ac_resolve_summary_get_sized(const ac_resolve*, ac_resolve_summary* out, size_t out_size);
void ac_resolve_free(ac_resolve*);
int ac_path_distances(const int32_t* entries, const uint64_t* path_off, uint32_t n_paths, const uint32_t* pair_a, const uint32_t* pair_b,
                      uint64_t n_pairs, const uint32_t* weights, uint32_t n_weights, int device, uint32_t* dist, uint8_t* status);
uint32_t ac_resolve_max_path(void);

typedef struct ac_components ac_components;
typedef struct {
    uint32_t first;
    uint32_t unitigs;
    uint64_t length;
    uint64_t links_all;
    uint64_t links_one_way;
    uint32_t open_ends;
    uint32_t marked;
    uint8_t  circular_loop;
} ac_component;
typedef struct {
    uint32_t size;
    uint32_t unitigs, components, topology;
    uint64_t links_all, links_one_way, total_length;
    uint32_t launches, read_backs;
    double seconds_device;
} ac_components_summary;
enum { AC_TOPOLOGY_EMPTY, AC_TOPOLOGY_FRAGMENTED, AC_TOPOLOGY_LINEAR_OPEN_OPEN, AC_TOPOLOGY_CIRCULAR,
       AC_TOPOLOGY_LINEAR_HAIRPIN_HAIRPIN, AC_TOPOLOGY_LINEAR_OPEN_HAIRPIN, AC_TOPOLOGY_OTHER };
int ac_graph_components(const ac_graph*, const uint8_t* marked , int device, ac_components** out);
int ac_components_from_links(uint32_t n_unitigs, const ac_link* links, uint64_t n_links,
                             const uint32_t* unitig_len , const uint8_t* alive ,
                             const uint8_t* marked , int device, ac_components** out);
int ac_components_records(const ac_components*, const ac_component** records, uint32_t* n);
int ac_components_of_unitig(const ac_components*, const uint32_t** component );
int ac_components_members(const ac_components*, const uint64_t** off , const uint32_t** members );
int ac_components_unitig_flags(const ac_components*, const uint8_t** flags);
size_t ac_components_summary_get_sized(const ac_components*, ac_components_summary* out, size_t out_size);
const char* ac_topology_name(uint32_t topology);
void ac_components_free(ac_components*);

typedef struct ac_merge ac_merge;
typedef struct {
    uint32_t number;
    uint32_t members;
    uint64_t length;
    uint64_t member_off;
    uint64_t seq_off;
    double   depth;
    uint8_t  type;
    uint8_t  loop;
} ac_merge_chain;
typedef struct {
    uint32_t size;
    uint32_t chains, merged_unitigs, unitigs_after;
    uint64_t links_after, bases_copied;
    uint32_t launches, read_backs;
    double seconds_device;
    double seconds_copy;
} ac_merge_summary;
enum { AC_UNITIG_OTHER, AC_UNITIG_ANCHOR, AC_UNITIG_CONSENTIG, AC_UNITIG_BRIDGE };
int ac_graph_merge_plan(const ac_graph*, int use_paths, int with_sequences, int device, ac_merge** out);
int ac_merge_plan_from_links(uint32_t n_unitigs, const ac_link* links, uint64_t n_links, const uint32_t* unitig_len,
        const uint8_t* alive , const int32_t* path_ends , uint32_t n_seqs,
        const double* depth , const uint32_t* fwd_positions, const uint32_t* rev_positions ,
        const uint8_t* type ,
        const uint8_t* seq_bytes, const uint64_t* seq_begin , int device, ac_merge** out);
int ac_merge_chains(const ac_merge*, const ac_merge_chain** chains, uint32_t* n);
int ac_merge_members(const ac_merge*, const int32_t** members , uint64_t* n);
int ac_merge_chain_of_unitig(const ac_merge*, const uint32_t** chain );
int ac_merge_fixed_flags(const ac_merge*, const uint8_t** flags );
int ac_merge_sequences(const ac_merge*, const uint8_t** bytes, uint64_t* n );
int ac_merge_links(const ac_merge*, const ac_link** links, uint64_t* n);
size_t ac_merge_summary_get_sized(const ac_merge*, ac_merge_summary* out, size_t out_size);
void ac_merge_free(ac_merge*);

typedef struct ac_subsets ac_subsets;
typedef struct ac_merged_paths ac_merged_paths;
typedef struct {
    uint32_t seqs;
    uint32_t unitigs;
    uint64_t entries;
    uint64_t links;
    uint64_t length;
} ac_subset_cluster;
typedef struct {
    uint32_t size;
    uint32_t clusters, sequences_kept, n_unitigs;
    uint64_t entries_kept, unitigs, links;
    uint32_t launches, read_backs;
    double seconds_device;
} ac_subsets_summary;
int ac_graph_subsets(const ac_graph*, const uint16_t* cluster_of_seq , uint32_t n_clusters, int device, ac_subsets** out);
int ac_subsets_from_paths(uint32_t n_unitigs, const ac_link* links, uint64_t n_links, const uint32_t* unitig_len, const uint8_t* alive ,
                          const int32_t* path_entries, const uint64_t* path_off , uint32_t n_seqs, const uint16_t* cluster_of_seq,
                          uint32_t n_clusters, int device, ac_subsets** out);
int ac_subsets_records(const ac_subsets*, const ac_subset_cluster** records, uint32_t* n_clusters);
int ac_subsets_unitigs(const ac_subsets*, const uint64_t** off, const uint32_t** unitigs, const uint32_t** fwd_positions, const uint32_t** rev_positions);
int ac_subsets_links(const ac_subsets*, const uint64_t** off, const ac_link** links);
int ac_subsets_seqs(const ac_subsets*, const uint64_t** off, const uint32_t** seq_index);
int ac_subsets_path_ends(const ac_subsets*, const uint64_t** off , const int32_t** path_ends);
int ac_subsets_dense(const ac_subsets*, uint32_t cluster, uint8_t* alive, uint32_t* fwd_positions, uint32_t* rev_positions, double* depth);
size_t ac_subsets_summary_get_sized(const ac_subsets*, ac_subsets_summary* out, size_t out_size);
void ac_subsets_free(ac_subsets*);
int ac_subsets_components(const ac_subsets*, uint32_t cluster, const uint8_t* marked , int device, ac_components** out);
int ac_subsets_merge_plan(const ac_subsets*, uint32_t cluster, const uint8_t* seq_bytes, const uint64_t* seq_begin, int with_sequences, int device,
                          ac_merge** out);
typedef struct {
    uint32_t size;
    uint32_t sequences;
    uint64_t entries_before, entries_after;
    uint32_t launches, read_backs;
    double seconds_device;
} ac_merged_paths_summary;
int ac_subsets_merged_paths(const ac_subsets*, uint32_t cluster, const ac_merge* plan, int device, ac_merged_paths** out);
int ac_merged_paths_get(const ac_merged_paths*, const uint32_t** seq_index, uint32_t* n_seqs, const uint64_t** path_off ,
                        const int32_t** entries);
size_t ac_merged_paths_summary_get_sized(const ac_merged_paths*, ac_merged_paths_summary* out, size_t out_size);
void ac_merged_paths_free(ac_merged_paths*);

typedef struct ac_finished ac_finished;
typedef struct {
    uint32_t number;
    uint32_t source;
    uint64_t length;
    uint64_t seq_off;
    double   depth;
    uint8_t  type;
} ac_finished_unitig;
typedef struct {
    uint32_t size;
    uint32_t unitigs, renumbered;
    uint32_t launches, read_backs;
    uint64_t links, path_entries, bases;
    uint64_t tie_items;
// ... 349 lines not shown
```

Baseline: 85660.

## Build novel k-mer list and occupancy bitmap incrementally during insert phases

While the hash-table insert runs in several phases, each finished range of the novel bitmap is popcounted, scanned and filled into the novel position list right away, with a carry passed between pieces. The occupancy bitmap is also set by atomic OR at slot-claim time, so the full table sweep is replaced by a lighter pass that only moves sibling flags. This aims to remove the separate full passes after insert, at the cost of extra atomics in the insert hot path, more arena memory, and a device-side count check for consistency. It is gated by a knob whose default enables it only for job builds with small tables.

```diff
diff --git a/autocycler_amd/_capi.py b/autocycler_amd/_capi.py
--- a/autocycler_amd/_capi.py
+++ b/autocycler_amd/_capi.py
@@ -41,7 +41,7 @@
                 ("n_local_distinct", C.c_uint64), ("n_fragments", C.c_uint64), ("fragment_bytes", C.c_uint64),
                 ("upload_device_ms", C.c_double), ("path_runs_copied", C.c_uint64), ("path_entries_walked", C.c_uint64), ("position_retries", C.c_uint64), ("n_candidates_owned", C.c_uint32),
                 ("launches", C.c_uint32), ("readbacks", C.c_uint32), ("n_degrees_open", C.c_uint64), ("sort_retries", C.c_uint64), ("insert_rest_known", C.c_double), ("insert_rest_sampled", C.c_double), ("path_stretches", C.c_uint64),
-                ("expand_sparse_sweeps", C.c_uint32), ("expand_sparse_start", C.c_uint32)]
+                ("expand_sparse_sweeps", C.c_uint32), ("expand_sparse_start", C.c_uint32), ("novel_words_early", C.c_uint64)]
 
     def as_dict(self):
         return {n: getattr(self, n) for n, _ in self._fields_}
diff --git a/autocycler_amd/csrc/capi.cpp b/autocycler_amd/csrc/capi.cpp
--- a/autocycler_amd/csrc/capi.cpp
+++ b/autocycler_amd/csrc/capi.cpp
@@ -331,6 +331,7 @@
     o->launches = t.launches; o->readbacks = t.readbacks; o->n_degrees_open = t.n_degrees_open; o->sort_retries = t.sort_retries;
     o->insert_rest_known = t.insert_rest_known; o->insert_rest_sampled = t.insert_rest_sampled; o->path_stretches = t.path_stretches;
     o->expand_sparse_sweeps = t.expand_sparse_sweeps; o->expand_sparse_start = t.expand_sparse_start;
+    o->novel_words_early = t.novel_words_early;
     return 0;
 }
 size_t ac_timings_get_sized(const ac_graph* g, ac_timings* out, size_t out_size) {
diff --git a/autocycler_amd/csrc/graph_build.hpp b/autocycler_amd/csrc/graph_build.hpp
--- a/autocycler_amd/csrc/graph_build.hpp
+++ b/autocycler_amd/csrc/graph_build.hpp
@@ -54,6 +54,7 @@
     uint32_t position_retries = 0;
     uint32_t launches = 0, readbacks = 0;
     uint64_t n_degrees_open = 0;
+    uint64_t novel_words_early = 0;
     uint64_t path_runs_copied = 0, path_entries_walked = 0;
 };
 
diff --git a/autocycler_amd/csrc/graph_impl.hpp b/autocycler_amd/csrc/graph_impl.hpp
--- a/autocycler_amd/csrc/graph_impl.hpp
+++ b/autocycler_amd/csrc/graph_impl.hpp
@@ -58,6 +58,7 @@
     u64* sflags;
     u64* full_at;
     u64* runs; u32* run_count; u64 run_row0;
+    u64* occ_set;
 };
 static const u64 RUN_MIN = 128;
 static const u32 RUN_ROW = 128;
@@ -191,7 +192,12 @@
         u64 v = tb.slots[s];
         if (v == SLOT_EMPTY) {
             u64 old = atomic_cas64(&tb.slots[s], SLOT_EMPTY, mine);
-            if (old == SLOT_EMPTY) { (*claimed)++; *mine_now = true; if (note) sib_note(tb, s, my_fl); return NOREF; }
+            if (old == SLOT_EMPTY) {
+                (*claimed)++; *mine_now = true;
+                if (tb.occ_set) atomic_or64(&tb.occ_set[s >> 6], 1ULL << (s & 63));
+                if (note) sib_note(tb, s, my_fl);
+                return NOREF;
+            }
             v = old;
         }
         if (slot_tag_eq(v, mine)) {
@@ -258,7 +264,10 @@
 void seq_expand_finish(SeqExpandJob& j) noexcept;
 [[maybe_unused]] static int key_words(int k) { int w = words_for_k(k); return w <= 4 ? w : (w <= 8 ? 8 : 16); }
 [[maybe_unused]] static u64 next_pow2(u64 x) { u64 p = 1; while (p < x) p <<= 1; return p; }
-[[maybe_unused]] static size_t arena_estimate(u64 n_text, bool owns_text) { return (size_t)n_text * (owns_text ? 8 : 7) + ((size_t)768 << 20); }
+static const u64 NOVEL_EARLY_MAX_CAP = 1ULL << 26;
+[[maybe_unused]] static size_t arena_estimate(u64 n_text, bool owns_text) {
+    return (size_t)n_text * (owns_text ? 8 : 7) + ((size_t)768 << 20) + (size_t)std::min<u64>(n_text, NOVEL_EARLY_MAX_CAP * 7 / 10) * 8;
+}
 struct Knobs {
     int minkey_variant;
     int path_copy;
@@ -307,6 +316,7 @@
     int multi_tail;
     u64 trim_batch_bytes;
     u64 resolve_batch_bytes;
+    int novel_early;
     static Knobs read() {
         Knobs k;
         k.minkey_variant = [&]() -> int { const char* e = getenv("AC_MINKEY_VARIANT"); return e ? atoi(e) : -1; }();
@@ -358,6 +368,7 @@
         k.multi_tail = [&]() -> int { const char* e = getenv("AC_MULTI_TAIL"); return e && !strcmp(e, "replicated") ? 1 : 0; }();
         k.trim_batch_bytes = [&]() -> u64 { const char* e = getenv("AC_TRIM_BATCH_BYTES"); const long long v = e ? atoll(e) : 0; return v > 0 ? (u64)v : (u64)4 << 30; }();
         k.resolve_batch_bytes = [&]() -> u64 { const char* e = getenv("AC_RESOLVE_BATCH_BYTES"); const long long v = e ? atoll(e) : 0; return v > 0 ? (u64)v : (u64)1 << 30; }();
+        k.novel_early = [&]() -> int { const char* e = getenv("AC_NOVEL_EARLY"); return e ? (atoi(e) != 0 ? 1 : 0) : -1; }();
         return k;
     }
 };
@@ -427,6 +438,7 @@
 [[maybe_unused]] static bool sort_checks_deferrable() { return knobs().sort_checks_deferrable; }
 [[maybe_unused]] static bool shard_host_remap() { return knobs().shard_host_remap; }
 [[maybe_unused]] static bool shard_degree_flags() { return knobs().shard_degree_flags; }
+[[maybe_unused]] static int novel_early() { return knobs().novel_early; }
 [[maybe_unused]] static bool insert_adaptive() { return knobs().insert_adaptive; }
 [[maybe_unused]] static u64 insert_growth() { return knobs().insert_growth; }
 [[maybe_unused]] static u64 insert_waves_target() { return knobs().insert_waves_target; }
@@ -499,6 +511,10 @@
     DBuf<u32> counters;
     DBuf<u64> slots; u64 cap = 0; u64 N = 0;
     DBuf<u64> bm; DBuf<u32> wprefix; DBuf<u64> npos;
+    DBuf<u32> novel_cnt, novel_carry; u64 novel_w_done = 0; u32 novel_pieces = 0; bool novel_listed = false;
+    void novel_counts(const u64* bits, u64 w0, u64 w1);
+    void novel_fill(const u64* bits, u64 w0, u64 w1, u64 npos_cap);
+    void novel_piece(const u64* bits, u64 w1, u64 npos_cap) { novel_counts(bits, novel_w_done, w1); novel_fill(bits, novel_w_done, w1, npos_cap); }
     u32 U = 0;
     DBuf<u32> kinfo, head, scan, ustart, order, rank, ulen;
     DBuf<u64> ustartpos, useq_off; DBuf<u8> uorient;
@@ -531,12 +547,13 @@
         if (t.n_text >= POS_MASK) throw DeviceError("input too large for 40-bit text positions");
         if (t.n_seqs == 0 || t.n_text < (u64)k + 2) throw DeviceError("no sequences");
     }
-    template <int W> void insert(const PackedText& t, u32 hint, DBuf<u64>* slots_out, u64* cap_out, u64* n_distinct_out, DBuf<u64>* bm_out, bool want_sib = false);
+    template <int W> void insert(const PackedText& t, u32 hint, DBuf<u64>* slots_out, u64* cap_out, u64* n_distinct_out, DBuf<u64>* bm_out, bool want_sib = false, DBuf<u64>* occ_out = nullptr);
     DBuf<u64> sflags;
     DBuf<u64> runs; DBuf<u32> run_count; u64 run_rows = 0, run_rows_cap = 0;
     DBuf<u64> loc_bm; DBuf<u32> loc_wprefix; bool local_insert_of_shard = false;
     struct CopyPlan { bool ok = false; u64 R = 0, NW = 0, Rb = 0; DBuf<RunRec> rr; DBuf<u32> rseq; DBuf<u64> wfirst, w_begin, w_end; DBuf<u32> w_gap; } cplan;
     void occupancy_bitmap(const DBuf<u64>& sl, u64 c, DBuf<u64>* occ_out, const u64* sflags_in, u64* sib_out, stream_t s = 0);
+    void move_sibling_bits(const DBuf<u64>& sl, u64 c, const u64* sflags_in, u64* sib_out, stream_t s = 0);
     DBuf<u64> occ;
     DBuf<u64> sib;
     DBuf<u64> sibn; bool sib_pending = false;
@@ -590,7 +607,7 @@
 #endif
         pt.pack();
     }
-    Table graph_table() const { return Table{const_cast<u64*>(slots.ptr()), cap - 1, occ.ptr(), nullptr, n_owners, my_owner, nullptr, nullptr, nullptr, nullptr, 0}; }
+    Table graph_table() const { return Table{const_cast<u64*>(slots.ptr()), cap - 1, occ.ptr(), nullptr, n_owners, my_owner, nullptr, nullptr, nullptr, nullptr, 0, nullptr}; }
     template <int W> void fragments();
     template <int W> void table();
     void novel_list(u64 known_n);
@@ -617,21 +634,40 @@
 #endif
     launch_full(c, MarkFunctor{sl.ptr(), occ_out->ptr(), sflags_in, sib_out}, s);
 }
+inline void GraphBuilder::Impl::move_sibling_bits(const DBuf<u64>& sl, u64 c, const u64* sflags_in, u64* sib_out, stream_t s) {
+    if (!sflags_in) return;
+    launch(c / 32, SibMoveFunctor{sl.ptr(), sflags_in, sib_out}, s);
+}
+inline void GraphBuilder::Impl::novel_counts(const u64* bits, u64 w0, u64 w1) {
+    launch(w1 - w0 + 1, PopcFunctor{bits + w0, novel_cnt.ptr() + w0, w1 - w0});
+    exclusive_scan_u32(novel_cnt.ptr() + w0, wprefix.ptr() + w0, w1 - w0 + 1);
+}
+inline void GraphBuilder::Impl::novel_fill(const u64* bits, u64 w0, u64 w1, u64 npos_cap) {
+    const u32* carry_in = novel_pieces ? novel_carry.ptr() + (novel_pieces & 1) : nullptr;
+    u32* carry_out = novel_carry.size() ? novel_carry.ptr() + ((novel_pieces + 1) & 1) : nullptr;
+    launch_wave_kernel(fill_novel_wave_kernel<0>, (w1 - w0 + 1 + 255) / 256, 0, bits, wprefix.ptr(), npos.ptr(), w0, w1, carry_in, carry_out, npos_cap);
+    novel_pieces++; novel_w_done = w1;
+}
 inline void GraphBuilder::Impl::novel_list(u64 known_n) {
     PackedText& g = *G;
     u64 n_bm_words = g.n_text / 64 + 1;
-    DBuf<u32> wcnt(n_bm_words + 1);
-    wprefix.alloc(n_bm_words + 1);
-    launch(n_bm_words + 1, PopcFunctor{bm.ptr(), wcnt.ptr(), n_bm_words});
-    exclusive_scan_u32(wcnt.ptr(), wprefix.ptr(), n_bm_words + 1);
-    if (known_n) N = known_n;
+    if (known_n && novel_listed) N = known_n;
     else {
-        N = read_scalar(wprefix.ptr() + n_bm_words);
-        if (N == 0) throw DeviceError("internal error: no k-mers in the union of the shards");
-        tm->n_distinct = N;
-    }
-    npos.alloc(N);
-    launch_wave_kernel(fill_novel_wave_kernel<0>, (n_bm_words + 255) / 256, 0, (const u64*)bm.ptr(), (const u32*)wprefix.ptr(), npos.ptr(), n_bm_words);
+        novel_cnt.alloc(n_bm_words + 1);
+        wprefix.alloc(n_bm_words + 1);
+        novel_carry = DBuf<u32>(); novel_w_done = 0; novel_pieces = 0;
+        novel_counts(bm.ptr(), 0, n_bm_words);
+        if (known_n) N = known_n;
+        else {
+            N = read_scalar(wprefix.ptr() + n_bm_words);
+            if (N == 0) throw DeviceError("internal error: no k-mers in the union of the shards");
+            tm->n_distinct = N;
+        }
+        npos.alloc(N);
+        novel_fill(bm.ptr(), 0, n_bm_words, N);
+    }
+    if (known_n) launch(1, CountCheckFunctor{wprefix.ptr() + n_bm_words, (u32)known_n, counters.ptr() + 2, 1u});
+    novel_listed = false;
     kinfo.alloc(N, true);
     head.alloc(N + 1); scan.alloc(N + 1);
     head.fill_bytes_from(N * 4, 0); scan.fill_bytes_from(N * 4, 0);
diff --git a/autocycler_amd/csrc/graph_stages.hip b/autocycler_amd/csrc/graph_stages.hip
--- a/autocycler_amd/csrc/graph_stages.hip
+++ b/autocycler_amd/csrc/graph_stages.hip
@@ -3,7 +3,7 @@
 namespace ac {
 
 template <int W>
-void GraphBuilder::Impl::insert(const PackedText& pt, u32 hint, DBuf<u64>* slots_out, u64* cap_out, u64* n_distinct_out, DBuf<u64>* bm_out, bool want_sib) {
+void GraphBuilder::Impl::insert(const PackedText& pt, u32 hint, DBuf<u64>* slots_out, u64* cap_out, u64* n_distinct_out, DBuf<u64>* bm_out, bool want_sib, DBuf<u64>* occ_out) {
     TextCtx t = pt.ctx((int)k);
     const u64 p_end_all = pt.n_text - (u64)k + 1;
     if (hint == 0) hint = 1;
@@ -24,9 +24,12 @@
     const int copy_mode = (&pt == &loc && (want_sib || (local_insert_of_shard && shard_path_copy()))) ? path_copy() : 0;
     bool want_runs = false;
     DBuf<InsertStats> istats(257);
-    DBuf<u64> sl;
+    DBuf<u64> sl, occ_set;
     DBuf<u64> nbm(pt.n_text / 64 + 2);
     u64 n_distinct = 0;
+    const bool list_here = occ_out && &pt == &loc && n_owners <= 1;
+    const u64 n_bm_words = pt.n_text / 64 + 1;
+    novel_listed = false;
     const Arena::Mark retry_mark = Arena::device().mark();
     std::vector<u64> phase_end;
     for (;;) {
@@ -37,9 +40,18 @@
         istats.fill_bytes(0);
         if (want_sib) { sflags.alloc(c / 32 + 1); sflags.fill_bytes(0); }
         else sflags = DBuf<u64>();
+        const bool early = list_here && novel_early() != 0 && (novel_early() == 1 || (job != nullptr && c <= NOVEL_EARLY_MAX_CAP));
+        const u64 npos_cap = std::min<u64>(p_end_all, c * 7 / 10) + 1;
+        if (early) {
+            novel_cnt.alloc(n_bm_words + 1); wprefix.alloc(n_bm_words + 1); novel_carry.alloc(2); npos.alloc(npos_cap);
+            novel_w_done = 0; novel_pieces = 0;
+        }
+        if (early) { occ_set.alloc((c + 63) / 64); occ_set.fill_bytes(0); }
+        else occ_set = DBuf<u64>();
+        u64 words_early = 0;
         u32* ierr = (u32*)&istats.ptr()[256].real;
         Table tb{sl.ptr(), c - 1, nullptr, nbm.ptr(), (&pt == &uni) ? n_owners : 1u, (&pt == &uni) ? my_owner : 0u, want_sib ? sflags.ptr() : nullptr,
-                 &istats.ptr()[256].claimed, nullptr, nullptr, 0};
+                 &istats.ptr()[256].claimed, nullptr, nullptr, 0, early ? occ_set.ptr() : nullptr};
         if (&pt == &loc) { runs = DBuf<u64>(); run_count = DBuf<u32>(); run_rows = run_rows_cap = 0; cplan = CopyPlan(); }
         phase_end.clear();
         stream_sync();
@@ -110,6 +122,12 @@
             launches++;
             pb = pe;
             phase_end.push_back(pe);
+            if (early) {
+                const bool last = pe == p_end_all;
+                const u64 w1 = last ? n_bm_words : pe / 64;
+                if (!last) words_early = w1;
+                if (w1 > novel_w_done) novel_piece(nbm.ptr(), w1, npos_cap);
+            }
             if (launches == 2 && insert_adaptive() && pb < p_end_all && (p_end_all - pb) > 4 * first) {
                 u64 probe_end = p_end_all;
 #ifndef AC_EMU
@@ -158,7 +176,11 @@
         u64 real = 0;
         for (auto& x : st) { n_distinct += x.claimed; real += x.real; }
         bool overflow = ins_err || (n_distinct * 10 > c * 7);
-        if (!overflow) { tm->insert_real += real; tm->insert_positions += pt.n_text; break; }
+        if (!overflow) {
+            tm->insert_real += real; tm->insert_positions += pt.n_text;
+            if (early) { novel_listed = true; tm->novel_words_early = words_early; }
+            break;
+        }
         const u64 c_max = next_pow2(pt.n_bases * 4 + 1024);
         if (c >= c_max) throw DeviceError("k-mer table overflow");
         u64 want = c * 4;
@@ -173,7 +195,8 @@
         c = std::min(want, c_max);
         tm->insert_kernel_ms = 0; tm->insert_launches = 0;
         stream_sync();
-        sl = DBuf<u64>(); sflags = DBuf<u64>();
+        sl = DBuf<u64>(); sflags = DBuf<u64>(); occ_set = DBuf<u64>();
+        novel_cnt = DBuf<u32>(); wprefix = DBuf<u32>(); novel_carry = DBuf<u32>(); npos = DBuf<u64>(); novel_w_done = 0; novel_pieces = 0;
         Arena::device().rewind(retry_mark);
     }
     if (n_distinct >= 0xFFFFFFF0ULL) throw DeviceError("too many distinct k-mers for 32-bit novel indices");
@@ -188,6 +211,7 @@
     *cap_out = c;
     *n_distinct_out = n_distinct;
     *bm_out = std::move(nbm);
+    if (occ_out) *occ_out = std::move(occ_set);
 }
 
 template <int W> void GraphBuilder::Impl::fragments() {
@@ -233,15 +257,17 @@
     PackedText& g = *G;
     check_sizes(g);
     const bool want_sib = k >= 3 && degree_flags() && (n_owners <= 1 || shard_degree_flags());
-    insert<W>(g, tm->graph_hint, &slots, &cap, &N, &bm, want_sib);
-    tm->table_capacity = cap;
-    tm->n_distinct = N;
-    lap(G == &loc ? &tm->insert : &tm->union_insert);
     const bool sib_by_pos = want_sib && n_owners <= 1;
     if (sib_by_pos) { sib.alloc(2 * (g.n_text / 64 + 2)); sib.fill_bytes(0); }
     else sib = DBuf<u64>();
     sibn = DBuf<u64>(); sib_pending = false;
-    occupancy_bitmap(slots, cap, &occ, sib_by_pos ? sflags.ptr() : nullptr, sib_by_pos ? sib.ptr() : nullptr);
+    occ = DBuf<u64>();
+    insert<W>(g, tm->graph_hint, &slots, &cap, &N, &bm, want_sib, &occ);
+    tm->table_capacity = cap;
+    tm->n_distinct = N;
+    lap(G == &loc ? &tm->insert : &tm->union_insert);
+    if (occ.size()) move_sibling_bits(slots, cap, sib_by_pos ? sflags.ptr() : nullptr, sib_by_pos ? sib.ptr() : nullptr);
+    else occupancy_bitmap(slots, cap, &occ, sib_by_pos ? sflags.ptr() : nullptr, sib_by_pos ? sib.ptr() : nullptr);
     if (n_owners <= 1) novel_list(N);
 }
 
diff --git a/autocycler_amd/csrc/graph_tail.hip b/autocycler_amd/csrc/graph_tail.hip
--- a/autocycler_amd/csrc/graph_tail.hip
+++ b/autocycler_amd/csrc/graph_tail.hip
@@ -576,6 +576,7 @@
             throw NeedCheckedSorts();
         }
         if (errs[7]) throw DeviceError("internal error: expand_repeats pool overflow");
+        if (errs[2]) throw DeviceError("internal error: the novel list does not hold the k-mers the insert claimed");
         if (n_links_check != n_links) throw DeviceError("internal error: link counts disagree");
         if (final_total_pending) { if (final_total_read > final_total) throw DeviceError("internal error: expand_repeats lengthened the sequences"); final_total = final_total_read; }
         if (errs[3] || errs[4])
diff --git a/autocycler_amd/csrc/kernels_table.inc b/autocycler_amd/csrc/kernels_table.inc
--- a/autocycler_amd/csrc/kernels_table.inc
+++ b/autocycler_amd/csrc/kernels_table.inc
@@ -224,17 +224,41 @@
         if (fl) atomic_or64(&sib[p >> 5], fl << (2 * (p & 31)));
     }
 };
+struct SibMoveFunctor {
+    const u64* slots; const u64* sflags; u64* sib;
+    AC_D void operator()(u64 w) const {
+        u64 x = sflags[w];
+        while (x) {
+            const int f = ctz64(x) >> 1;
+            const u64 fl = (x >> (2 * f)) & 3;
+            x &= ~(3ULL << (2 * f));
+            const u64 v = slots[w * 32 + (u64)f];
+            if (v == SLOT_EMPTY) continue;
+            const u64 p = slot_pos(v);
+            atomic_or64(&sib[p >> 5], fl << (2 * (p & 31)));
+        }
+    }
+};
 struct PopcFunctor {
     const u64* bm; u32* cnt; u64 n;
     AC_HD void operator()(u64 w) const { cnt[w] = w < n ? (u32)popc64(bm[w]) : 0u; }
 };
-template <int UNUSED> AC_KERNEL void __launch_bounds__(256) fill_novel_wave_kernel(const u64* bm, const u32* wprefix, u64* npos, u64 n_words) {
-    const u64 w = (u64)wv::bid() * 256 + wv::tid();
+template <int UNUSED> AC_KERNEL void __launch_bounds__(256)
+fill_novel_wave_kernel(const u64* bm, u32* wprefix, u64* npos, u64 w_first, u64 w_end, const u32* carry_in, u32* carry_out, u64 npos_cap) {
+    const u64 w = w_first + (u64)wv::bid() * 256 + wv::tid();
     const int lane = wv::lane();
     const u64 w0 = w - (u64)lane;
-    if (w0 >= n_words) return;
+    if (w0 > w_end) return;
+    const u64 n_words = w_end;
     const u64 x = w < n_words ? bm[w] : 0;
-    const u32 start = w < n_words ? wprefix[w] : 0;
+    u32 start = 0;
+    if (w <= w_end) {
+        start = wprefix[w];
+        if (carry_in) { start += *carry_in; wprefix[w] = start; }
+        if (w == w_end && carry_out) *carry_out = start;
+    }
+    if (w0 >= w_end) return;
+    if (w >= n_words) start = 0;
     const u32 cnt = (u32)popc64(x);
     const u32 base = (u32)wv::shfl((int)start, 0);
     const u32 rel = w < n_words ? start - base : 0xFFFFFFFFu;
@@ -259,6 +283,6 @@
             const u32 c = (u32)popc64(v & ((1ULL << sh) - 1));
             if (r >= c) { r -= c; v >>= sh; pos += (u32)sh; }
         }
-        npos[(u64)base + t] = (w0 + (u64)lo) * 64 + pos;
-    }
-}
+        if ((u64)base + t < npos_cap) npos[(u64)base + t] = (w0 + (u64)lo) * 64 + pos;
+    }
+}
diff --git a/include/autocycler_hip.h b/include/autocycler_hip.h
--- a/include/autocycler_hip.h
+++ b/include/autocycler_hip.h
@@ -50,6 +50,7 @@
     uint64_t path_stretches;
     uint32_t expand_sparse_sweeps;
     uint32_t expand_sparse_start;
+    uint64_t novel_words_early;
 } ac_timings;
 
 int ac_compress_build(uint32_t k, uint32_t assembly_count, const ac_seq_view* seqs, uint32_t n_seqs, int device,
```

After: 82170. 4.1% lower.
